# Pixie8888/R3DFSSeg

Hardware: AMD Instinct MI355X
Metric: episodes/sec S3DIS 2-way 5-shot 2048-pt (MPTI+attention, train step: forward+backward+grad all-reduce+Adam) (higher is better)
Workload: dtype f32 (index-free GEMMs -- self-attention, 1x1 convolutions, weight gradients, the EdgeConv backward's edge GEMMs -- as bf16x3 split products on the bf16 MFMA with fp32 accumulate; every index-deciding result: fp32)

## Files before the change

include/r3d.h:

```cpp
#ifndef R3D_H
#define R3D_H
#include <stdint.h>

#ifdef __cplusplus
extern "C" {
#endif

const char* r3d_last_error_string(void);
int r3d_abi_version(void);
int r3d_debug_poison_lds(unsigned pattern, unsigned* sink , void* stream);
int r3d_debug_set_cg_spmv_lds_min_blocks(int min_blocks);
int r3d_set_matrix_arith(int mode);
int r3d_get_matrix_arith(void);
int r3d_debug_set_gemm_bx3(int mask);

int r3d_cm_to_pm(const float* in , int B, int C, int N, float* out , long ld, void* stream);
int r3d_pm_to_cm(const float* in , long ld, int B, int C, int N, float* out , void* stream);
int r3d_pm_to_cm_pitched(const float* in, long ld, int B, int C, int N, float* out , long pitch, void* stream);
long r3d_cm_pitch(int N);
int r3d_copy_cols(const float* src, long ld_src, float* dst, long ld_dst, long M, int C, void* stream);

int r3d_sqnorm(const float* x, long ldx, long rows, int C, float* out, void* stream);
long r3d_knn_norm_ws_words(int B, int N);
int r3d_knn_topk(const float* x, long ldx, const float* x_cm, int B, int N, int C, int k, int mode,
                 const int32_t* n_valid_dev, float* norm_ws, float* cm_ws, int32_t* idx_out, float* score_out,
                 int32_t* status, void* stream);
long r3d_knn_ws_words(int B, int N, int C, int k, int flags);
int r3d_knn_topk_batched(const float* x, long ldx, const float* x_cm, int B, int N, int C, int k, int mode,
                         const int32_t* n_valid_dev, int n_valid_stride, float* ws, long ws_words, int32_t* idx_out,
                         float* score_out, int32_t* status, void* stream);
int r3d_debug_set_knn_bf16_threshold(int on);
int r3d_debug_set_knn_bf16_filter(int on);
int r3d_set_wpack_in_capture(int on);

int r3d_pointwise_conv(const float* X, long ldx, const float* W , long M, int K, int Co,
                       const float* scale, const float* shift, int act, float* Out, long ldo, void* stream);

int r3d_edgeconv_fwd(const float* PQ, const int32_t* idx, const float* W2, const float* s2, const float* t2,
                     float* out, long ldo, int B, int N, int K, int32_t* argmax_out, void* stream);

long r3d_attention_ws_words(int B, int N);
int r3d_attention_fwd(const float* qkv, long ld, int B, int N, float* out, long ldo, float* lse_out, float* ws,
                      void* stream);

int r3d_head_desc_words(void);
int r3d_head_max_k(void);
int r3d_fps_sample_count_table(int k, int n_max, int32_t* out, void* stream);
long r3d_head_proto_ws_words(int n_way, int k_shot, int N);
int r3d_head_proto_ws_offsets(int n_way, int k_shot, int N, long* out6 );
#define R3D_HEAD_FPS_ONE_LAUNCH 1
int r3d_head_prototypes(const int32_t* support_y , const int32_t* shot_keep ,
                        const float* feat , long ldf, const float* featT ,
                        const float* qfeat , long ldq, int n_way, int k_shot, int N, int D,
                        int n_query_pts, int k, float* nodes, long ldn, float* node_labels ,
                        int32_t* desc, int32_t* assign_out , int32_t* cluster_count ,
                        int32_t* ws, long ws_words, int flags, void* stream);

int r3d_head_prototypes_batched(int n_ep, int fps_group, const int32_t* support_y, long sy_stride, const int32_t* shot_keep,
                                long keep_stride, const float* feat, long ldf, long feat_ep_rows, const float* qfeat, long ldq,
                                long qfeat_ep_rows, int n_way, int k_shot, int N, int D, int n_query_pts, int k, float* nodes,
                                long ldn, long nodes_ep_rows, float* node_labels, int32_t* desc, long desc_stride,
                                int32_t* assign_out, long assign_stride, int32_t* cluster_count, long ccount_stride,
                                int32_t* ws, long ws_words, long ws_stride, int flags, void* stream);

long r3d_lp_ws_words(int n_cap, int kp1);
int r3d_lp_ws_offsets(int n_cap, int kp1, long* out6);
int r3d_label_propagate(const float* nodes, long ldn, int D, const int32_t* nbr, int kp1, const float* Y,
                        const int32_t* n_dev, const int32_t* n_proto_dev, int n_cap, float sigma, float alpha,
                        int max_iter, float tol, float* Z, int32_t* ws, long ws_words, int32_t* stats_out, void* stream);

int r3d_label_propagate_batched(int n_ep, const float* nodes, long ldn, int D, const int32_t* nbr, int kp1, const float* Y,
                                const int32_t* n_dev, const int32_t* n_proto_dev, long desc_stride, int n_cap, float sigma,
                                float alpha, int max_iter, float tol, float* Z, int32_t* ws, long ws_words, long ws_stride,
                                int32_t* stats_out, long stats_stride, void* stream);
long r3d_graph_weights_verify_words(int n_cap, int kp1);
int r3d_graph_weights_verify(int n_ep, const float* nodes, long ldn, int D, const int32_t* n_dev, long desc_stride, int n_cap,
                             int kp1, float sigma, int32_t* ws, long ws_words, long ws_stride, float* scratch,
                             int32_t* mismatch_out, void* stream);

int r3d_label_propagate_solve_batched(int n_ep, const float* Y, const int32_t* n_dev, long desc_stride, int n_cap, int kp1,
                                      float alpha, int max_iter, float tol, float* Z, int32_t* ws, long ws_words,
                                      long ws_stride, int32_t* stats_out, long stats_stride, void* stream);

int r3d_graph_set_lp_budget(void* graph, void* graph_exec, int budget, int* n_cg);

int r3d_query_logits_ce(const float* Z, const int32_t* n_proto_dev, int n_q, int N, int n_classes,
                        const int64_t* labels , float* logits ,
                        float* loss_out , int32_t* pred_out , void* stream);

int r3d_query_logits_ce_batched(int n_ep, const float* Z, long z_ep_rows, const int32_t* n_proto_dev, long desc_stride, int n_q,
                                int N, int n_classes, const int64_t* labels, float* logits, float* loss_out, int32_t* pred_out,
                                void* stream);

int r3d_pointwise_conv_acc(const float* X, long ldx, const float* W, long M, int K, int Co, const float* scale,
                           const float* shift, int act, float* Out, long ldo, void* stream);
long r3d_pointwise_conv_stats_ws_words(long M, int Co);
int r3d_pointwise_conv_stats(const float* X, long ldx, const float* W, long M, int K, int Co, float* Out, long ldo,
                             float* sums_out , float* ws, void* stream);
int r3d_pointwise_conv_stats2(const float* X, long ldx, const float* W, long M, int K, int Co, float* Out, long ldo,
                              long M_first, float* sums_a , float* sums_b , float* ws, void* stream);
int r3d_pointwise_conv_stats_seg(const float* X, long ldx, const float* W, long M, int K, int Co, float* Out, long ldo,
                                 long rows_a, long rows_b, float* sums_out, float* ws, void* stream);
int r3d_colreduce(const float* part , int chunks, int C, float* sums_out , void* stream);
int r3d_colreduce_seg(const float* part, int count_a, int count_b, int n_seg, int C, float* sums_out , void* stream);
long r3d_colstats_ws_words(long M, int C);
int r3d_colstats(const float* X, long ldx, const float* DY, long lddy, long M, int C, int mode, const float* scale,
                 const float* shift, const float* mean, const float* invstd, int act, float* sums_out ,
                 float* ws, void* stream);
int r3d_bn_fold(const float* sums, double count, int C, const float* gamma, const float* beta, float eps,
                float momentum, float* running_mean , float* running_var , float* mean, float* invstd,
                float* scale, float* shift, float* rec , const int32_t* rec_index_dev , long rec_stride,
                void* stream);
long r3d_colstats_seg_ws_words(long M, int C, long rows_a, long rows_b);
int r3d_colstats_seg(const float* X, long ldx, const float* DY, long lddy, long M, int C, long rows_a, long rows_b, int mode,
                     const float* scale, const float* shift, const float* mean, const float* invstd, long bn_stride, int act,
                     float* sums_out , float* ws, void* stream);
int r3d_bn_fold_seg(const float* sums , int n_seg, double count_a, double count_b, int C, const float* gamma,
                    const float* beta, float eps, float momentum, float* running_mean , float* running_var ,
                    float* mean, float* invstd, float* scale, float* shift, long bn_stride, float* rec ,
                    const int32_t* rec_index_dev , long rec_stride, void* stream);
int r3d_affine_act_seg(const float* Z, long ldz, long M, int C, long rows_a, long rows_b, const float* scale, const float* shift,
                       long bn_stride, int act, float* Y, long ldy, void* stream);
int r3d_bn_bwd_apply_seg(const float* Z, long ldz, const float* DY, long lddy, long M, int C, long rows_a, long rows_b,
                         const float* scale, const float* shift, const float* mean, const float* invstd, long bn_stride, int act,
                         const float* sums , double count_a, double count_b, float* DZ, long lddz, void* stream);
int r3d_bn_running_update(const float* rec, int n_records, long rec_stride, int C, float momentum,
                          const float* bias , float* running_mean,
                          float* running_var, void* stream);
int r3d_affine_act(const float* Z, long ldz, long M, int C, const float* scale, const float* shift, int act, float* Y,
                   long ldy, void* stream);
int r3d_bn_bwd_apply(const float* Z, long ldz, const float* DY, long lddy, long M, int C, const float* scale,
                     const float* shift, const float* mean, const float* invstd, int act, const float* sums,
                     double count, float* DZ, long lddz, void* stream);
long r3d_gemm_tn_ws_words(long M, int Ca, int Cb);
int r3d_gemm_tn(const float* A, long lda, const float* B, long ldb, long M, int Ca, int Cb, float alpha, float* out,
                int accumulate, float* ws, void* stream);
int r3d_add_cols(const float* src, long ld_src, float* dst, long ld_dst, long M, int C, void* stream);

long r3d_edgeconv_train_ws_words(int B, int N);
int r3d_edge_stats1(const float* PQ, const int32_t* idx, int B, int N, int K, int clouds_a, int clouds_b,
                    float* sums_out , float* esum , float* ws,
                    void* stream);
int r3d_edgeconv_train_fwd_minmax(const float* PQ, const int32_t* idx, const float* s1, const float* t1, long bn_stride,
                                  const float* W2, int B, int N, int K, int clouds_a, int clouds_b, float* zmax, float* zmin,
                                  int32_t* argmax, int32_t* argmin, float* sums_out , float* ws, void* stream);
int r3d_edge_select(float* zmax , const float* zmin, int32_t* argmax ,
                    const int32_t* argmin, const float* s2, const float* t2, long bn_stride, long M, long rows_a, long rows_b,
                    float* out, long ldo, void* stream);
long r3d_edge_reverse_ws_words(int B, int N, int K);
int r3d_edge_reverse(const int32_t* idx, int B, int N, int K, int32_t* rev_ws, long ws_words, void* stream);
int r3d_edgeconv_bwd(const float* PQ, const int32_t* idx, const float* s1, const float* t1, const float* mean1,
                     const float* invstd1, const float* W2, const float* s2, const float* t2, const float* mean2,
                     const float* invstd2, long bn_stride, const float* bn2_sums, const float* dout, long lddo,
                     const int32_t* argmax, const float* zwin , const float* esum , int B, int N, int K,
                     int clouds_a, int clouds_b, float* DY1 , float* BE ,
                     const int32_t* rev_ws , float* dW2, float* bn1_sums, float* dPQ,
                     float* ws, void* stream);

int r3d_attention_fwd_train(const float* qkv, long ld, int B, int N, float* out, long ldo, float* lse_out, float p_drop,
                            unsigned seed, const unsigned* seed_dev, float* ws , void* stream);
int r3d_attention_bwd(const float* qkv, long ld, int B, int N, const float* O, long ldo, const float* dO, long lddo,
                      const float* lse, float p_drop, unsigned seed, const unsigned* seed_dev, float q_scale, float* dqkv,
                      long ldd, float* ws , void* stream);
int r3d_attention_bwd_ws(const float* qkv, long ld, int B, int N, const float* O, long ldo, const float* dO, long lddo,
                         const float* lse, float p_drop, unsigned seed, const unsigned* seed_dev, float q_scale,
                         float* dqkv, long ldd, float* ws, int ws_holds_packed_qkv, void* stream);

long r3d_attention_ws_words_ep(int B, int N, int seed_group);
int r3d_attention_fwd_train_ep(const float* qkv, long ld, int B, int N, float* out, long ldo, float* lse_out, float p_drop,
                               unsigned seed, const unsigned* seed_dev, int seed_group, float* ws, void* stream);
int r3d_attention_bwd_ep(const float* qkv, long ld, int B, int N, const float* O, long ldo, const float* dO, long lddo,
                         const float* lse, float p_drop, unsigned seed, const unsigned* seed_dev, int seed_group, float q_scale,
                         float* dqkv, long ldd, float* ws, int ws_holds_packed_qkv, void* stream);

long r3d_attention_ws_words_ep_d(int B, int N, int seed_group, int D);
int r3d_attention_fwd_train_ep_d(const float* qkv, long ld, int B, int N, float* out, long ldo, float* lse_out, float p_drop,
                                 unsigned seed, const unsigned* seed_dev, int seed_group, int D, float* ws, void* stream);
int r3d_attention_bwd_ep_d(const float* qkv, long ld, int B, int N, const float* O, long ldo, const float* dO, long lddo,
                           const float* lse, float p_drop, unsigned seed, const unsigned* seed_dev, int seed_group, int D,
                           float q_scale, float* dqkv, long ldd, float* ws, int ws_holds_packed_qkv, void* stream);

int r3d_ce_grad(const float* Z, const int32_t* n_proto_dev, int n_cap, int n_query_pts, int n_classes,
                const int64_t* labels, const float* gscale_dev, float* G, void* stream);
int r3d_label_propagate_bwd(const float* nodes, long ldn, int D, int kp1, const float* Z, const float* G,
                            const int32_t* n_dev, int n_cap, float sigma, float alpha, int max_iter, float tol, float* lam,
                            float* dnodes, long ldd, int32_t* ws, long ws_words, int32_t* stats_out, void* stream);
int r3d_head_prototypes_bwd(const float* dnodes, long ldd, int n_way, int k_shot, int N, int D, int n_query_pts,
                            const int32_t* desc, const int32_t* assign, const int32_t* cluster_count, const int32_t* ws,
                            float* dsfeat, long lds_, float* dqfeat, long ldq, void* stream);

int r3d_ce_grad_batched(int n_ep, const float* Z, const int32_t* n_proto_dev, long desc_stride, int n_cap, int n_query_pts,
                        int n_classes, const int64_t* labels, const float* gscale_dev, float* G, void* stream);
int r3d_label_propagate_bwd_batched(int n_ep, const float* nodes, long ldn, int D, int kp1, const float* Z, const float* G,
                                    const int32_t* n_dev, long desc_stride, int n_cap, float sigma, float alpha, int max_iter,
                                    float tol, float* lam, float* dnodes, long ldd, int32_t* ws, long ws_words, long ws_stride,
                                    int32_t* stats_out, long stats_stride, void* stream);
int r3d_head_prototypes_bwd_batched(int n_ep, const float* dnodes, long ldd, long nodes_ep_rows, int n_way, int k_shot, int N,
                                    int D, int n_query_pts, const int32_t* desc, long desc_stride, const int32_t* assign,
                                    long assign_stride, const int32_t* cluster_count, long ccount_stride, const int32_t* ws,
                                    long ws_stride, float* dsfeat, long lds_, long dsfeat_ep_rows, float* dqfeat, long ldq,
                                    long dqfeat_ep_rows, void* stream);

long r3d_contrast_ws_words(int n_way, int k_shot, int N);
int r3d_contrast_fwd(const float* feat, long ldf, int D, const int32_t* support_y, const int32_t* support_flag, int n_way,
                     int k_shot, int N, const float* W, const float* bias, float temp, float* loss_out, float* ws,
                     long ws_words, void* stream);
int r3d_contrast_bwd(int D, int n_way, int k_shot, int N, const float* gscale_dev, float* dfeat, long ldd, float* dW,
                     float* db, float* ws, void* stream);
int r3d_contrast_fwd_batched(int n_ep, const float* feat, long ldf, long feat_ep_rows, int D, const int32_t* support_y,
                             const int32_t* support_flag, int n_way, int k_shot, int N, const float* W, const float* bias,
                             float temp, float* loss_out, float* ws, long ws_words, long ws_stride, void* stream);
int r3d_contrast_bwd_batched(int n_ep, int D, int n_way, int k_shot, int N, const float* gscale_dev, float* dfeat, long ldd,
                             long dfeat_ep_rows, float* dW, float* db, float* ws, long ws_stride, void* stream);
int r3d_train_metrics_batched(int n_ep, const int32_t* pred, const int64_t* query_y, const int64_t* gt_query_y, int n_query_pts,
                              const float* Z, long z_ep_rows, const int32_t* desc, long desc_stride, const int32_t* proto_ws,
                              long pws_stride, const int32_t* assign, long assign_stride, const int32_t* gt_support_y, int n_way,
                              int k_shot, int N, float* out4 , void* stream);
int r3d_train_metrics(const int32_t* pred, const int64_t* query_y, const int64_t* gt_query_y, int n_query_pts, const float* Z,
                      const int32_t* desc, const int32_t* proto_ws, const int32_t* assign, const int32_t* gt_support_y,
                      int n_way, int k_shot, int N, float* out4, void* stream);

long r3d_clean_ws_words(int n_way, int k_shot);
int r3d_clean_shot_detect(const float* feat , long ldf, int D, const float* support_x ,
                          int Cin, const int32_t* support_y, int n_way, int k_shot, int N, int32_t* shot_keep,
                          float* dbg_cos_sum , int32_t* ws, void* stream);

int r3d_clean_shot_detect_batched(int n_ep, const float* feat, long ldf, long feat_ep_rows, int D, const float* support_x,
                                  int Cin, const int32_t* support_y, int n_way, int k_shot, int N, int32_t* shot_keep,
                                  float* dbg_cos_sum, int32_t* ws, long ws_stride, void* stream);

int r3d_protonet_head(const float* sfeat, long ldf, const float* qfeat, long ldq, int D, const int32_t* support_y,
                      int n_way, int k_shot, int N, int n_query_pts, int method, float scaler, float* Z, float* ws,
                      void* stream);

long r3d_protonet_head_ws_words(int n_ep, int n_way, int k_shot);
int r3d_protonet_head_batched(int n_ep, const float* sfeat, long ldf, const float* qfeat, long ldq, long feat_ep_rows, int D,
                              const int32_t* support_y, int n_way, int k_shot, int N, int n_query_pts, int method,
                              float scaler, float* Z, float* ws, long ws_words, void* stream);
int r3d_count_correct_batched(int n_ep, const int32_t* pred, const int64_t* labels, long n_pts, int32_t* correct,
                              void* stream);

long r3d_protonet_head_train_ws_words(int n_ep, int n_way, int k_shot, int N, int n_query_pts, int D);
int r3d_protonet_head_train_fwd(int n_ep, const float* sfeat, long ldf, const float* qfeat, long ldq, long feat_ep_rows, int D,
                                const int32_t* support_y, int n_way, int k_shot, int N, int n_query_pts, int method,
                                float scaler, float* Z, float* ws, long ws_words, void* stream);
int r3d_protonet_head_bwd(int n_ep, const float* qfeat, long ldq, long feat_ep_rows, int D, const int32_t* support_y, int n_way,
                          int k_shot, int N, int n_query_pts, int method, float scaler, const float* dZ, float* dsfeat,
                          long ldds, float* dqfeat, long lddq, long dfeat_ep_rows, float* ws, long ws_words, void* stream);

int r3d_miou_accumulate(const int32_t* pred, const int64_t* gt, long n, const int32_t* lut, int n_lut, int n_classes,
                        uint64_t* hist, void* stream);

#ifdef __cplusplus
}
#endif
#endif
```

r3dfsseg_amd/_lib.py:

```python
import ctypes
import os
import re

_HERE = os.path.dirname(os.path.abspath(__file__))
LIB_PATH = os.environ.get("R3D_LIB") or os.path.join(_HERE, "libr3d_hip.so")
HEADER_PATH = os.path.join(os.path.dirname(_HERE), "include", "r3d.h")

c_f = ctypes.c_void_p
c_i = ctypes.c_int
c_l = ctypes.c_long
c_fl = ctypes.c_float
c_d = ctypes.c_double
c_u = ctypes.c_uint

_SIGS = {
    "r3d_last_error_string": (ctypes.c_char_p, []),
    "r3d_abi_version": (c_i, []),
    "r3d_cm_to_pm": (c_i, [c_f, c_i, c_i, c_i, c_f, c_l, c_f]),
    "r3d_pm_to_cm": (c_i, [c_f, c_l, c_i, c_i, c_i, c_f, c_f]),
    "r3d_pm_to_cm_pitched": (c_i, [c_f, c_l, c_i, c_i, c_i, c_f, c_l, c_f]),
    "r3d_cm_pitch": (c_l, [c_i]),
    "r3d_copy_cols": (c_i, [c_f, c_l, c_f, c_l, c_l, c_i, c_f]),
    "r3d_sqnorm": (c_i, [c_f, c_l, c_l, c_i, c_f, c_f]),
    "r3d_knn_topk": (c_i, [c_f, c_l, c_f, c_i, c_i, c_i, c_i, c_i, c_f, c_f, c_f, c_f, c_f, c_f, c_f]),
    "r3d_pointwise_conv": (c_i, [c_f, c_l, c_f, c_l, c_i, c_i, c_f, c_f, c_i, c_f, c_l, c_f]),
    "r3d_edgeconv_fwd": (c_i, [c_f, c_f, c_f, c_f, c_f, c_f, c_l, c_i, c_i, c_i, c_f, c_f]),
    "r3d_attention_ws_words": (c_l, [c_i, c_i]),
    "r3d_knn_norm_ws_words": (c_l, [c_i, c_i]),
    "r3d_attention_fwd": (c_i, [c_f, c_l, c_i, c_i, c_f, c_l, c_f, c_f, c_f]),
    "r3d_head_desc_words": (c_i, []),
    "r3d_debug_poison_lds": (c_i, [c_u, c_f, c_f]),
    "r3d_debug_set_cg_spmv_lds_min_blocks": (c_i, [c_i]),
    "r3d_debug_set_gemm_bx3": (c_i, [c_i]),
    "r3d_set_matrix_arith": (c_i, [c_i]),
    "r3d_get_matrix_arith": (c_i, []),
    "r3d_head_max_k": (c_i, []),
    "r3d_fps_sample_count_table": (c_i, [c_i, c_i, c_f, c_f]),
    "r3d_head_proto_ws_words": (c_l, [c_i, c_i, c_i]),
    "r3d_head_proto_ws_offsets": (c_i, [c_i, c_i, c_i, ctypes.POINTER(c_l)]),
    "r3d_head_prototypes": (c_i, [c_f, c_f, c_f, c_l, c_f, c_f, c_l, c_i, c_i, c_i, c_i, c_i, c_i, c_f, c_l,
                                  c_f, c_f, c_f, c_f, c_f, c_l, c_i, c_f]),
    "r3d_lp_ws_words": (c_l, [c_i, c_i]),
    "r3d_lp_ws_offsets": (c_i, [c_i, c_i, ctypes.POINTER(c_l)]),
    "r3d_label_propagate": (c_i, [c_f, c_l, c_i, c_f, c_i, c_f, c_f, c_f, c_i, c_fl, c_fl, c_i, c_fl, c_f, c_f,
                                  c_l, c_f, c_f]),
    "r3d_graph_set_lp_budget": (c_i, [c_f, c_f, c_i, ctypes.POINTER(c_i)]),
    "r3d_pointwise_conv_acc": (c_i, [c_f, c_l, c_f, c_l, c_i, c_i, c_f, c_f, c_i, c_f, c_l, c_f]),
    "r3d_edgeconv_train_fwd_minmax": (c_i, [c_f, c_f, c_f, c_f, c_l, c_f, c_i, c_i, c_i, c_i, c_i, c_f, c_f, c_f, c_f, c_f, c_f, c_f]),
    "r3d_edge_select": (c_i, [c_f, c_f, c_f, c_f, c_f, c_f, c_l, c_l, c_l, c_l, c_f, c_l, c_f]),
    "r3d_pointwise_conv_stats_ws_words": (c_l, [c_l, c_i]),
    "r3d_pointwise_conv_stats": (c_i, [c_f, c_l, c_f, c_l, c_i, c_i, c_f, c_l, c_f, c_f, c_f]),
    "r3d_pointwise_conv_stats2": (c_i, [c_f, c_l, c_f, c_l, c_i, c_i, c_f, c_l, c_l, c_f, c_f, c_f, c_f]),
    "r3d_colreduce": (c_i, [c_f, c_i, c_i, c_f, c_f]),
    "r3d_colstats_ws_words": (c_l, [c_l, c_i]),
    "r3d_colstats": (c_i, [c_f, c_l, c_f, c_l, c_l, c_i, c_i, c_f, c_f, c_f, c_f, c_i, c_f, c_f, c_f]),
    "r3d_bn_fold": (c_i, [c_f, c_d, c_i, c_f, c_f, c_fl, c_fl, c_f, c_f, c_f, c_f, c_f, c_f, c_f, c_f, c_l, c_f]),
    "r3d_bn_running_update": (c_i, [c_f, c_i, c_l, c_i, c_fl, c_f, c_f, c_f, c_f]),
    "r3d_affine_act": (c_i, [c_f, c_l, c_l, c_i, c_f, c_f, c_i, c_f, c_l, c_f]),
    "r3d_bn_bwd_apply": (c_i, [c_f, c_l, c_f, c_l, c_l, c_i, c_f, c_f, c_f, c_f, c_i, c_f, c_d, c_f, c_l, c_f]),
    "r3d_gemm_tn_ws_words": (c_l, [c_l, c_i, c_i]),
    "r3d_gemm_tn": (c_i, [c_f, c_l, c_f, c_l, c_l, c_i, c_i, c_fl, c_f, c_i, c_f, c_f]),
    "r3d_add_cols": (c_i, [c_f, c_l, c_f, c_l, c_l, c_i, c_f]),
    "r3d_edgeconv_train_ws_words": (c_l, [c_i, c_i]),
    "r3d_edge_stats1": (c_i, [c_f, c_f, c_i, c_i, c_i, c_i, c_i, c_f, c_f, c_f, c_f]),
    "r3d_edge_reverse_ws_words": (c_l, [c_i, c_i, c_i]),
    "r3d_edge_reverse": (c_i, [c_f, c_i, c_i, c_i, c_f, c_l, c_f]),
    "r3d_edgeconv_bwd": (c_i, [c_f] * 11 + [c_l, c_f, c_f, c_l, c_f, c_f, c_f, c_i, c_i, c_i, c_i, c_i, c_f, c_f, c_f, c_f, c_f, c_f, c_f, c_f]),
    "r3d_attention_fwd_train": (c_i, [c_f, c_l, c_i, c_i, c_f, c_l, c_f, c_fl, c_u, c_f, c_f, c_f]),
    "r3d_attention_bwd": (c_i, [c_f, c_l, c_i, c_i, c_f, c_l, c_f, c_l, c_f, c_fl, c_u, c_f, c_fl, c_f, c_l, c_f, c_f]),
    "r3d_attention_bwd_ws": (c_i, [c_f, c_l, c_i, c_i, c_f, c_l, c_f, c_l, c_f, c_fl, c_u, c_f, c_fl, c_f, c_l, c_f, c_i, c_f]),
    "r3d_ce_grad": (c_i, [c_f, c_f, c_i, c_i, c_i, c_f, c_f, c_f, c_f]),
    "r3d_label_propagate_bwd": (c_i, [c_f, c_l, c_i, c_i, c_f, c_f, c_f, c_i, c_fl, c_fl, c_i, c_fl, c_f, c_f, c_l, c_f, c_l, c_f, c_f]),
    "r3d_head_prototypes_bwd": (c_i, [c_f, c_l, c_i, c_i, c_i, c_i, c_i, c_f, c_f, c_f, c_f, c_f, c_l, c_f, c_l, c_f]),
    "r3d_contrast_ws_words": (c_l, [c_i, c_i, c_i]),
    "r3d_contrast_fwd": (c_i, [c_f, c_l, c_i, c_f, c_f, c_i, c_i, c_i, c_f, c_f, c_fl, c_f, c_f, c_l, c_f]),
    "r3d_contrast_bwd": (c_i, [c_i, c_i, c_i, c_i, c_f, c_f, c_l, c_f, c_f, c_f, c_f]),
    "r3d_train_metrics": (c_i, [c_f, c_f, c_f, c_i, c_f, c_f, c_f, c_f, c_f, c_i, c_i, c_i, c_f, c_f]),
    "r3d_clean_ws_words": (c_l, [c_i, c_i]),
    "r3d_clean_shot_detect": (c_i, [c_f, c_l, c_i, c_f, c_i, c_f, c_i, c_i, c_i, c_f, c_f, c_f, c_f]),
    "r3d_protonet_head": (c_i, [c_f, c_l, c_f, c_l, c_i, c_f, c_i, c_i, c_i, c_i, c_i, c_fl, c_f, c_f, c_f]),
    "r3d_protonet_head_ws_words": (c_l, [c_i, c_i, c_i]),
    "r3d_protonet_head_batched": (c_i, [c_i, c_f, c_l, c_f, c_l, c_l, c_i, c_f, c_i, c_i, c_i, c_i, c_i, c_fl, c_f, c_f, c_l, c_f]),
    "r3d_count_correct_batched": (c_i, [c_i, c_f, c_f, c_l, c_f, c_f]),
    "r3d_protonet_head_train_ws_words": (c_l, [c_i, c_i, c_i, c_i, c_i, c_i]),
    "r3d_protonet_head_train_fwd": (c_i, [c_i, c_f, c_l, c_f, c_l, c_l, c_i, c_f, c_i, c_i, c_i, c_i, c_i, c_fl, c_f, c_f, c_l, c_f]),
    "r3d_protonet_head_bwd": (c_i, [c_i, c_f, c_l, c_l, c_i, c_f, c_i, c_i, c_i, c_i, c_i, c_fl, c_f, c_f, c_l, c_f, c_l, c_l, c_f,
                                    c_l, c_f]),
    "r3d_miou_accumulate": (c_i, [c_f, c_f, c_l, c_f, c_i, c_i, c_f, c_f]),
    "r3d_query_logits_ce": (c_i, [c_f, c_f, c_i, c_i, c_i, c_f, c_f, c_f, c_f, c_f]),
    "r3d_knn_topk_batched": (c_i, [c_f, c_l, c_f, c_i, c_i, c_i, c_i, c_i, c_f, c_i, c_f, c_l, c_f, c_f, c_f, c_f]),
    "r3d_knn_ws_words": (c_l, [c_i, c_i, c_i, c_i, c_i]),
    "r3d_debug_set_knn_bf16_threshold": (c_i, [c_i]),
    "r3d_debug_set_knn_bf16_filter": (c_i, [c_i]),
    "r3d_set_wpack_in_capture": (c_i, [c_i]),
    "r3d_pointwise_conv_stats_seg": (c_i, [c_f, c_l, c_f, c_l, c_i, c_i, c_f, c_l, c_l, c_l, c_f, c_f, c_f]),
    "r3d_colreduce_seg": (c_i, [c_f, c_i, c_i, c_i, c_i, c_f, c_f]),
    "r3d_colstats_seg_ws_words": (c_l, [c_l, c_i, c_l, c_l]),
    "r3d_colstats_seg": (c_i, [c_f, c_l, c_f, c_l, c_l, c_i, c_l, c_l, c_i, c_f, c_f, c_f, c_f, c_l, c_i, c_f, c_f, c_f]),
    "r3d_bn_fold_seg": (c_i, [c_f, c_i, c_d, c_d, c_i, c_f, c_f, c_fl, c_fl, c_f, c_f, c_f, c_f, c_f, c_f, c_l, c_f, c_f, c_l, c_f]),
    "r3d_affine_act_seg": (c_i, [c_f, c_l, c_l, c_i, c_l, c_l, c_f, c_f, c_l, c_i, c_f, c_l, c_f]),
    "r3d_bn_bwd_apply_seg": (c_i, [c_f, c_l, c_f, c_l, c_l, c_i, c_l, c_l, c_f, c_f, c_f, c_f, c_l, c_i, c_f, c_d, c_d, c_f, c_l, c_f]),
    "r3d_attention_ws_words_ep": (c_l, [c_i, c_i, c_i]),
    "r3d_attention_fwd_train_ep": (c_i, [c_f, c_l, c_i, c_i, c_f, c_l, c_f, c_fl, c_u, c_f, c_i, c_f, c_f]),
    "r3d_attention_bwd_ep": (c_i, [c_f, c_l, c_i, c_i, c_f, c_l, c_f, c_l, c_f, c_fl, c_u, c_f, c_i, c_fl, c_f, c_l, c_f, c_i, c_f]),
    "r3d_attention_ws_words_ep_d": (c_l, [c_i, c_i, c_i, c_i]),
    "r3d_attention_fwd_train_ep_d": (c_i, [c_f, c_l, c_i, c_i, c_f, c_l, c_f, c_fl, c_u, c_f, c_i, c_i, c_f, c_f]),
    "r3d_attention_bwd_ep_d": (c_i, [c_f, c_l, c_i, c_i, c_f, c_l, c_f, c_l, c_f, c_fl, c_u, c_f, c_i, c_i, c_fl, c_f, c_l, c_f, c_i,
                                     c_f]),
    "r3d_head_prototypes_batched": (c_i, [c_i, c_i, c_f, c_l, c_f, c_l, c_f, c_l, c_l, c_f, c_l, c_l, c_i, c_i, c_i, c_i, c_i, c_i,
                                          c_f, c_l, c_l, c_f, c_f, c_l, c_f, c_l, c_f, c_l, c_f, c_l, c_l, c_i, c_f]),
    "r3d_head_prototypes_bwd_batched": (c_i, [c_i, c_f, c_l, c_l, c_i, c_i, c_i, c_i, c_i, c_f, c_l, c_f, c_l, c_f, c_l, c_f, c_l,
                                              c_f, c_l, c_l, c_f, c_l, c_l, c_f]),
    "r3d_graph_weights_verify_words": (c_l, [c_i, c_i]),
    "r3d_graph_weights_verify": (c_i, [c_i, c_f, c_l, c_i, c_f, c_l, c_i, c_i, c_fl, c_f, c_l, c_l, c_f, c_f, c_f]),
    "r3d_label_propagate_solve_batched": (c_i, [c_i, c_f, c_f, c_l, c_i, c_i, c_fl, c_i, c_fl, c_f, c_f, c_l, c_l, c_f, c_l, c_f]),
    "r3d_label_propagate_batched": (c_i, [c_i, c_f, c_l, c_i, c_f, c_i, c_f, c_f, c_f, c_l, c_i, c_fl, c_fl, c_i, c_fl, c_f, c_f,
                                          c_l, c_l, c_f, c_l, c_f]),
    "r3d_label_propagate_bwd_batched": (c_i, [c_i, c_f, c_l, c_i, c_i, c_f, c_f, c_f, c_l, c_i, c_fl, c_fl, c_i, c_fl, c_f, c_f,
                                              c_l, c_f, c_l, c_l, c_f, c_l, c_f]),
    "r3d_ce_grad_batched": (c_i, [c_i, c_f, c_f, c_l, c_i, c_i, c_i, c_f, c_f, c_f, c_f]),
    "r3d_query_logits_ce_batched": (c_i, [c_i, c_f, c_l, c_f, c_l, c_i, c_i, c_i, c_f, c_f, c_f, c_f, c_f]),
    "r3d_contrast_fwd_batched": (c_i, [c_i, c_f, c_l, c_l, c_i, c_f, c_f, c_i, c_i, c_i, c_f, c_f, c_fl, c_f, c_f, c_l, c_l, c_f]),
    "r3d_contrast_bwd_batched": (c_i, [c_i, c_i, c_i, c_i, c_i, c_f, c_f, c_l, c_l, c_f, c_f, c_f, c_l, c_f]),
    "r3d_train_metrics_batched": (c_i, [c_i, c_f, c_f, c_f, c_i, c_f, c_l, c_f, c_l, c_f, c_l, c_f, c_l, c_f, c_i, c_i, c_i, c_f, c_f]),
    "r3d_clean_shot_detect_batched": (c_i, [c_i, c_f, c_l, c_l, c_i, c_f, c_i, c_f, c_i, c_i, c_i, c_f, c_f, c_f, c_l, c_f]),
}

_lib = None


def header_symbols():
    txt = open(HEADER_PATH).read()
    txt = re.sub(r"/\*.*?\*/", "", txt, flags=re.S)
    return sorted(set(re.findall(r"\b(r3d_[a-z0-9_]+)\s*\(", txt)))


ABI_VERSION = 5


def load():
    global _lib
    if _lib is not None:
        return _lib
    import torch
    if not os.path.exists(LIB_PATH):
        raise RuntimeError(
            "r3dfsseg_amd: %s not found -- build it with `python -m r3dfsseg_amd.build` "
            "(hipcc, gfx950). There is no CPU fallback." % LIB_PATH)
    cdll = ctypes.CDLL(LIB_PATH)
    lib = _Bound()
    lib._cdll = cdll
    for name, (res, args) in _SIGS.items():
        try:
            fn = getattr(cdll, name)
        except AttributeError:
            raise RuntimeError("r3dfsseg_amd: symbol %s missing from %s" % (name, LIB_PATH))
        fn.restype = res
        fn.argtypes = args
        setattr(lib, name, fn)
    if lib.r3d_abi_version() != ABI_VERSION:
        raise RuntimeError("r3dfsseg_amd: %s has C ABI version %d, this package binds version %d -- rebuild it "
                           "(`python -m r3dfsseg_amd.build --force`)" % (LIB_PATH, lib.r3d_abi_version(), ABI_VERSION))
    _lib = lib
    mode = os.environ.get("R3D_MATRIX_ARITH")
    if mode is not None:
        if mode not in ("fp32", "bf16x3"):
            raise RuntimeError("R3D_MATRIX_ARITH=%r: expected fp32 or bf16x3" % mode)
        check(lib.r3d_set_matrix_arith(1 if mode == "bf16x3" else 0))
    mask = os.environ.get("R3D_GEMM_BX3")
    if mask is not None:
        check(lib.r3d_debug_set_gemm_bx3(int(mask)))
    return lib


class _Bound:
    """The bound entry points as plain attributes (one per symbol of include/r3d.h)."""


_call_log = None


def record_calls(on):
    lib = load()
    for name in _SIGS:
        raw = getattr(lib._cdll, name)
        if not on:
            setattr(lib, name, raw)
            continue

        def wrapper(*args, _raw=raw):
            rc = _raw(*args)
            if _call_log is not None:
                _call_log.append((_raw, args))
            return rc
        setattr(lib, name, wrapper)


def check(rc):
    if rc != 0:
        raise RuntimeError("r3d: " + load().r3d_last_error_string().decode())
```

r3dfsseg_amd/csrc/common.h:

```cpp
#pragma once
#include <hip/hip_runtime.h>
#include <stdint.h>
#include <stdio.h>

#define R3D_OK 0
#define R3D_ERR_ARG 1
#define R3D_ERR_LAUNCH 2
#define R3D_ERR_UNSUPPORTED 3

void r3d_set_error(const char* fmt, ...);

#define R3D_REQUIRE(cond, ...)          \
  do {                                  \
    if (!(cond)) {                      \
      r3d_set_error(__VA_ARGS__);       \
      return R3D_ERR_ARG;               \
    }                                   \
  } while (0)

#define R3D_LAUNCH_CHECK(name)                                              \
  do {                                                                      \
    hipError_t e_ = hipGetLastError();                                      \
    if (e_ != hipSuccess) {                                                 \
      r3d_set_error("%s: launch failed: %s", name, hipGetErrorString(e_));  \
      return R3D_ERR_LAUNCH;                                                \
    }                                                                       \
  } while (0)

typedef float f32x16 __attribute__((ext_vector_type(16)));
typedef float f32x4 __attribute__((ext_vector_type(4)));

#define R3D_WAVE 64

static __device__ __forceinline__ int r3d_lane() { return threadIdx.x & 63; }

static __device__ __forceinline__ int r3d_acc_row(int r, int lane) {
  return (r & 3) + 8 * (r >> 2) + 4 * (lane >> 5);
}

static __device__ __forceinline__ float r3d_readlane_f(float v, int src) {
  return __int_as_float(__builtin_amdgcn_readlane(__float_as_int(v), src));
}

static __device__ __forceinline__ float r3d_sum8_dpp(float v) {
  int x = __float_as_int(v);
  v += __int_as_float(__builtin_amdgcn_mov_dpp(x, 0xB1, 0xF, 0xF, true));
  x = __float_as_int(v);
  v += __int_as_float(__builtin_amdgcn_mov_dpp(x, 0x4E, 0xF, 0xF, true));
  x = __float_as_int(v);
  v += __int_as_float(__builtin_amdgcn_mov_dpp(x, 0x141, 0xF, 0xF, true));
  return v;
}

static __device__ __forceinline__ int r3d_wave_incl_scan(int v) {
  v += __builtin_amdgcn_update_dpp(0, v, 0x111, 0xF, 0xF, true);
  v += __builtin_amdgcn_update_dpp(0, v, 0x112, 0xF, 0xF, true);
  v += __builtin_amdgcn_update_dpp(0, v, 0x114, 0xF, 0xF, true);
  v += __builtin_amdgcn_update_dpp(0, v, 0x118, 0xF, 0xF, true);
  v += __builtin_amdgcn_update_dpp(0, v, 0x142, 0xA, 0xF, false);
  v += __builtin_amdgcn_update_dpp(0, v, 0x143, 0xC, 0xF, false);
  return v;
}

static __device__ __forceinline__ float r3d_wave_sum(float v) {
#pragma unroll
  for (int o = 32; o > 0; o >>= 1) v += __shfl_xor(v, o);
  return v;
}
static __device__ __forceinline__ float r3d_wave_max(float v) {
#pragma unroll
  for (int o = 32; o > 0; o >>= 1) v = fmaxf(v, __shfl_xor(v, o));
  return v;
}

static __device__ __forceinline__ float r3d_keep(float v, bool keep) {
  return __uint_as_float(__float_as_uint(v) & (keep ? 0xffffffffu : 0u));
}

typedef unsigned r3d_u32x4 __attribute__((ext_vector_type(4)));
typedef __bf16 r3d_bf16x8 __attribute__((ext_vector_type(8)));
extern int g_r3d_matrix_arith;

static __device__ __forceinline__ void r3d_bx3_split2(float x0, float x1, unsigned& h, unsigned& m, unsigned& l) {
  const unsigned u0 = __float_as_uint(x0), u1 = __float_as_uint(x1);
  const float r0 = x0 - __uint_as_float(u0 & 0xffff0000u), r1 = x1 - __uint_as_float(u1 & 0xffff0000u);
  const unsigned v0 = __float_as_uint(r0), v1 = __float_as_uint(r1);
  const float t0 = r0 - __uint_as_float(v0 & 0xffff0000u), t1 = r1 - __uint_as_float(v1 & 0xffff0000u);
  h = __builtin_amdgcn_perm(u1, u0, 0x07060302u);
  m = __builtin_amdgcn_perm(v1, v0, 0x07060302u);
  l = __builtin_amdgcn_perm(__float_as_uint(t1), __float_as_uint(t0), 0x07060302u);
}
struct r3d_bx3 {
  r3d_u32x4 h, m, l;
};
static __device__ __forceinline__ r3d_bx3 r3d_bx3_split8(const float* x) {
  r3d_bx3 f;
#pragma unroll
  for (int i = 0; i < 4; ++i) {
    unsigned h, m, l;
    r3d_bx3_split2(x[2 * i], x[2 * i + 1], h, m, l);
    f.h[i] = h; f.m[i] = m; f.l[i] = l;
  }
  return f;
}
static __device__ __forceinline__ f32x16 r3d_mfma_bf16(r3d_u32x4 a, r3d_u32x4 b, f32x16 c) {
#if defined(ATT_ABL) && (ATT_ABL & 4)
  c[0] += __uint_as_float(a[0] ^ b[1]);
  return c;
#endif
  return __builtin_amdgcn_mfma_f32_32x32x16_bf16(__builtin_bit_cast(r3d_bf16x8, a), __builtin_bit_cast(r3d_bf16x8, b), c, 0,
                                                 0, 0);
}
static __device__ __forceinline__ f32x16 r3d_bx3_mma(const r3d_bx3& a, const r3d_bx3& b, f32x16 c) {
  c = r3d_mfma_bf16(a.l, b.h, c);
  c = r3d_mfma_bf16(a.h, b.l, c);
  c = r3d_mfma_bf16(a.m, b.m, c);
  c = r3d_mfma_bf16(a.m, b.h, c);
  c = r3d_mfma_bf16(a.h, b.m, c);
  c = r3d_mfma_bf16(a.h, b.h, c);
  return c;
}

extern int g_r3d_gemm_bx3;

static inline int r3d_cdiv(long a, long b) { return (int)((a + b - 1) / b); }

static __device__ __forceinline__ int r3d_xcd_swizzle(int id, int n) {
  const int q = n >> 3, r = n & 7, x = id & 7;
  return (x < r ? x * (q + 1) : r * (q + 1) + (x - r) * q) + (id >> 3);
}

struct r3d_segmap {
  long a, b;
  __host__ __device__ bool odd(int seg) const { return b > 0 && (seg & 1); }
  __host__ __device__ long seg_rows(int seg) const { return odd(seg) ? b : a; }
  __host__ __device__ long seg_row0(int seg) const {
    return b > 0 ? (long)(seg >> 1) * (a + b) + (odd(seg) ? a : 0) : (long)seg * a;
  }
  __host__ __device__ int seg_of_row(long r) const {
    if (b == 0) return (int)(r / a);
    const long p = r / (a + b);
    return (int)(2 * p + ((r - p * (a + b)) >= a ? 1 : 0));
  }
  __device__ int seg_of_row32(int r) const {
    const int A = (int)a, B = (int)b;
    if (B == 0) return r / A;
    const int p = r / (A + B);
    return 2 * p + ((r - p * (A + B)) >= A ? 1 : 0);
  }
  __host__ __device__ int n_seg(long total) const { return (int)(b > 0 ? 2 * (total / (a + b)) : total / a); }
  __host__ __device__ bool covers(long total) const {
    return a > 0 && b >= 0 && total > 0 && total < 0x7fffffffL && total % (a + b) == 0;
  }
};

static __global__ void r3d_fill_words_kernel(unsigned* __restrict__ p, unsigned v, long n) {
  for (long i = (long)blockIdx.x * blockDim.x + threadIdx.x; i < n; i += (long)gridDim.x * blockDim.x) p[i] = v;
}
static __global__ void r3d_copy_words_kernel(unsigned* __restrict__ dst, const unsigned* __restrict__ src, long n) {
  for (long i = (long)blockIdx.x * blockDim.x + threadIdx.x; i < n; i += (long)gridDim.x * blockDim.x) dst[i] = src[i];
}
static __global__ void r3d_fill_words_ep_kernel(unsigned* __restrict__ p, unsigned v, long n, long stride_words) {
  p += (long)blockIdx.y * stride_words;
  for (long i = (long)blockIdx.x * blockDim.x + threadIdx.x; i < n; i += (long)gridDim.x * blockDim.x) p[i] = v;
}
static inline void r3d_fill_words_ep(void* p, unsigned v, long n_words, int n_ep, long stride_words, hipStream_t st) {
  const int g = (int)(n_words < 256L * 2048 ? (n_words + 255) / 256 : 2048);
  hipLaunchKernelGGL(r3d_fill_words_ep_kernel, dim3(g > 0 ? g : 1, n_ep), dim3(256), 0, st, (unsigned*)p, v, n_words, stride_words);
}
static inline void r3d_zero_words(void* p, long n_words, hipStream_t st) {
  const int g = (int)(n_words < 256L * 2048 ? (n_words + 255) / 256 : 2048);
  hipLaunchKernelGGL(r3d_fill_words_kernel, dim3(g > 0 ? g : 1), dim3(256), 0, st, (unsigned*)p, 0u, n_words);
}
static inline void r3d_copy_words(void* dst, const void* src, long n_words, hipStream_t st) {
  const int g = (int)(n_words < 256L * 2048 ? (n_words + 255) / 256 : 2048);
  hipLaunchKernelGGL(r3d_copy_words_kernel, dim3(g > 0 ? g : 1), dim3(256), 0, st, (unsigned*)dst, (const unsigned*)src,
                     n_words);
}
```

r3dfsseg_amd/csrc/edgeconv_train.hip:

```cpp
#include <stdlib.h>
#include "edge_tile.h"

#define ET_LD 65
#define ET_MAXBLK 1024
#define EC_CHUNK 32

static __device__ __forceinline__ float lrelu(float v) { return v > 0.f ? v : 0.2f * v; }

struct EcGeom {
  int N, cpc;
  __host__ __device__ static EcGeom make(int N) { return EcGeom{N, (N + EC_CHUNK - 1) / EC_CHUNK}; }
  __device__ void range(int chunk, int& cloud, int& p0, int& p1) const {
    cloud = __builtin_amdgcn_readfirstlane(chunk / cpc);
    p0 = __builtin_amdgcn_readfirstlane(cloud * N + (chunk - cloud * cpc) * EC_CHUNK);
    p1 = __builtin_amdgcn_readfirstlane(min(p0 + EC_CHUNK, (cloud + 1) * N));
  }
};
static __device__ __forceinline__ int ec_seg(const r3d_segmap& cs, int cloud) {
  return __builtin_amdgcn_readfirstlane(cs.seg_of_row32(cloud));
}

template <int RT>
__global__ __launch_bounds__(256) void r3d_edge_stats1_kernel(const float* __restrict__ PQ, const int* __restrict__ idx,
                                                              EcGeom gm, int n_chunks, float* __restrict__ part,
// ... 343 lines not shown
  for (int o = 32; o > 0; o >>= 1) my_below += __shfl_xor(my_below, o);
  if (lane == 0) atomicAdd(&below_s, my_below);
  __syncthreads();
  if (tid < RV_RANGE) {
    const int v = tid < nr ? cnt[tid] : 0;
    int x = v;
#pragma unroll
    for (int o = 1; o < 64; o <<= 1) {
      const int y = __shfl_up(x, o);
      if (lane >= o) x += y;
    }
    if (lane == 63) wsum[w] = x;
    cur[tid] = x - v;
  }
  __syncthreads();
  if (tid < RV_RANGE) {
    int wb = 0;
    for (int q = 0; q < w; ++q) wb += wsum[q];
    off[tid] = cur[tid] + wb;
  }
  if (tid == 0) {
    int t = 0;
    for (int q = 0; q < RV_RANGE / 64; ++q) t += wsum[q];
    off[RV_RANGE] = t;
  }
  __syncthreads();
  const long seg0 = gbase + below_s;
  if (tid < nr) rev_ptr[(long)cloud * N + r0 + tid] = (int)(seg0 + off[tid]);
  if (cloud == n_clouds - 1 && r0 + nr == N && tid == 0) rev_ptr[(long)n_clouds * N] = (int)((long)n_clouds * E);
  int a = 0;
  while (a < nr) {
    if (tid == 0) {
      int b = nr;
      if (off[nr] - off[a] > RV_CAP) {
        int lo = a, hi = nr;
        while (lo < hi) {
          const int mid = (lo + hi + 1) >> 1;
          if (off[mid] - off[a] <= RV_CAP) lo = mid; else hi = mid - 1;
        }
        b = lo;
      }
      b_s = b;
    }
    __syncthreads();
    const int b = b_s;
    if (b == a) {
      long outp = seg0 + off[a];
      for (long e0 = 0; e0 < E; e0 += 1024) {
        const long e = e0 + tid;
        const bool hit = e < E && min(max(lst[min(e, E - 1)], 0), N - 1) - r0 == a;
        const unsigned long long m = __ballot(hit);
        if (lane == 0) wsum[w] = __popcll(m);
        __syncthreads();
        int before = 0, total = 0;
        for (int q = 0; q < 16; ++q) { before += q < w ? wsum[q] : 0; total += wsum[q]; }
        if (hit) rev[outp + before + __popcll(m & ((1ull << lane) - 1ull))] = (int)(gbase + e);
        outp += total;
        __syncthreads();
      }
      a += 1;
      continue;
    }
    if (tid < RV_RANGE) cur[tid] = (tid >= a && tid < b) ? off[tid] - off[a] : 0;
    __syncthreads();
    for (long e0 = tid; e0 < E; e0 += 8 * 1024) {
      int jv[8];
#pragma unroll
      for (int u = 0; u < 8; ++u) jv[u] = lst[min(e0 + 1024 * u, E - 1)];
#pragma unroll
      for (int u = 0; u < 8; ++u) {
        const int j = min(max(jv[u], 0), N - 1) - r0;
        if (e0 + 1024 * u < E && j >= a && j < b)
          buf[atomicAdd(&cur[j], 1)] = (int)(e0 + 1024 * u);
      }
    }
    __syncthreads();
    for (int j = a + w; j < b; j += 16) {
      const int s0 = off[j] - off[a], c = cnt[j];
      const long out0 = seg0 + off[j];
      for (int m0 = 0; m0 < c; m0 += 64) {
        const int mine = m0 + lane < c ? buf[s0 + m0 + lane] : 0x7fffffff;
        int rank = 0;
        for (int t0 = 0; t0 < c; t0 += 16) {
          int ov[16];
#pragma unroll
          for (int t = 0; t < 16; ++t) ov[t] = buf[s0 + min(t0 + t, c - 1)];
#pragma unroll
          for (int t = 0; t < 16; ++t) rank += (t0 + t < c && ov[t] < mine) ? 1 : 0;
        }
        if (m0 + lane < c) rev[out0 + rank] = (int)(gbase + mine);
      }
    }
    __syncthreads();
    a = b;
  }
}

#define RO_WAVES 8
__global__ __launch_bounds__(64 * RO_WAVES) void r3d_edge_reverse_ordered_kernel(const int* __restrict__ idx, int N, int K,
                                                                                 int n_clouds, int* __restrict__ rev_ptr,
                                                                                 int* __restrict__ rev) {
  extern __shared__ int ro_hist[];
  __shared__ int ro_wsum[RO_WAVES];
  const int tid = threadIdx.x, lane = tid & 63, w = __builtin_amdgcn_readfirstlane(tid >> 6);
  const int cloud = blockIdx.x;
  const int E = N * K;
  const long gbase = (long)cloud * E;
  const int* lst = idx + gbase;
  const int per = ((E + RO_WAVES - 1) / RO_WAVES + 63) & ~63;
  const int e_beg = min(w * per, E), e_end = min(e_beg + per, E);
  int* mine = ro_hist + w * N;
  for (int i = tid; i < RO_WAVES * N; i += 64 * RO_WAVES) ro_hist[i] = 0;
  __syncthreads();
  for (int e0 = e_beg + lane; e0 < e_end; e0 += 8 * 64) {
    int jv[8];
#pragma unroll
    for (int u = 0; u < 8; ++u) jv[u] = lst[min(e0 + 64 * u, E - 1)];
#pragma unroll
    for (int u = 0; u < 8; ++u)
      if (e0 + 64 * u < e_end) atomicAdd(&mine[min(max(jv[u], 0), N - 1)], 1);
  }
  __syncthreads();
  const int TPT = (N + 64 * RO_WAVES - 1) / (64 * RO_WAVES);
  const int j0 = tid * TPT;
  int tot = 0;
  for (int j = j0; j < min(j0 + TPT, N); ++j)
#pragma unroll
    for (int q = 0; q < RO_WAVES; ++q) tot += ro_hist[q * N + j];
  int incl = tot;
#pragma unroll
  for (int o = 1; o < 64; o <<= 1) {
    const int y = __shfl_up(incl, o);
    if (lane >= o) incl += y;
  }
  if (lane == 63) ro_wsum[w] = incl;
  __syncthreads();
  int run = incl - tot;
  for (int q = 0; q < w; ++q) run += ro_wsum[q];
  for (int j = j0; j < min(j0 + TPT, N); ++j) {
    rev_ptr[(long)cloud * N + j] = (int)(gbase + run);
#pragma unroll
    for (int q = 0; q < RO_WAVES; ++q) {
      const int c = ro_hist[q * N + j];
      ro_hist[q * N + j] = run;
      run += c;
    }
  }
  if (cloud == n_clouds - 1 && tid == 0) rev_ptr[(long)n_clouds * N] = (int)((long)n_clouds * E);
  __syncthreads();
  for (int e0 = e_beg; e0 < e_end; e0 += 64) {
    const int e = e0 + lane;
    const bool ok = e < e_end;
    const int j = min(max(lst[min(e, E - 1)], 0), N - 1);
    const int src = e / K;
    const int src0 = __builtin_amdgcn_readfirstlane(e0 / K);
    const int src1 = __builtin_amdgcn_readfirstlane(min(e0 + 63, e_end - 1) / K);
    int pos = 0;
    for (int g = src0; g <= src1; ++g)
      if (ok && src == g) pos = atomicAdd(&mine[j], 1);
    if (ok) rev[gbase + pos] = (int)(gbase + e);
  }
}

template <int RT>
__global__ __launch_bounds__(256) void r3d_edgeconv_bwd2_kernel(
    const float* __restrict__ PQ, const float* __restrict__ s1, const float* __restrict__ mean1,
    const float* __restrict__ invstd1, long bn_stride, const float* __restrict__ bn1_sums ,
    const float* __restrict__ DY1, const float* __restrict__ BE, const float* __restrict__ esum ,
    const int* __restrict__ rev_ptr, const int* __restrict__ rev,
    int e_off, EcGeom gm, r3d_segmap cs , int n_chunks, float* __restrict__ dPQ ) {
  constexpr int K = 4 * RT;
  const int lane = threadIdx.x & 63, w = threadIdx.x >> 6;
  for (int item = blockIdx.x; item < n_chunks; item += gridDim.x) {
    const int chunk = r3d_xcd_swizzle(item, n_chunks);
    int cloud, p0, p1;
    gm.range(chunk, cloud, p0, p1);
    const int seg = ec_seg(cs, cloud);
    const long bo = (long)seg * bn_stride;
    const double E = (double)cs.seg_rows(seg) * gm.N * K;
    const float sc1 = s1[bo + lane], mu1 = mean1[bo + lane], is1 = invstd1[bo + lane];
    const float n1 = (float)((double)bn1_sums[(long)seg * 128 + lane] / E), n2 = (float)((double)bn1_sums[(long)seg * 128 + 64 + lane] / E);
    for (int pt_ = p0 + w; pt_ < p1; pt_ += 4) {
      const long pt = pt_;
      const int rb = rev_ptr[pt], re = rev_ptr[pt + 1];
      const float pj = PQ[pt * 128 + lane];
      const float bs = BE[pt * 128 + lane];
      const float es = esum ? (esum[pt * 64 + lane] - (float)K * mu1) * is1 : BE[pt * 128 + 64 + lane];
      float asum = 0.f, gsum = 0.f;
      for (int e0 = rb; e0 < re; e0 += 16) {
        const int my_e = rev[min(e0 + min(lane, 15), re - 1)];
        float dv[16], qv[16];
#pragma unroll
        for (int t = 0; t < 16; ++t) {
          const int e = __builtin_amdgcn_readlane(my_e, t) - e_off;
          dv[t] = DY1[(long)e * 64 + lane];
          qv[t] = PQ[(long)(e / K) * 128 + 64 + lane];
        }
#pragma unroll
        for (int t = 0; t < 16; ++t) {
          const bool ok = e0 + t < re;
          asum += r3d_keep(dv[t], ok);
          gsum += r3d_keep(qv[t], ok);
        }
      }
      const float cj = (float)(re - rb);
      dPQ[pt * 128 + lane] = sc1 * (asum - cj * n1 - n2 * (is1 * (cj * (pj - mu1) + gsum)));
      dPQ[pt * 128 + 64 + lane] = sc1 * (bs - (float)K * n1 - n2 * es);
    }
  }
}

static int et_check(const char* fn, int B, int N, int K, int clouds_a, int clouds_b) {
  if (B <= 0 || N <= 0 || N % E2_PTS != 0 || K < 4 || K > 32 || K % 4 != 0) {
    r3d_set_error("%s: unsupported shape B=%d N=%d K=%d (N %% 4 == 0, K %% 4 == 0, 4..32)", fn, B, N, K);
    return R3D_ERR_ARG;
  }
  const r3d_segmap cs{clouds_a, clouds_b};
  if (!cs.covers(B)) {
    r3d_set_error("%s: %d clouds are not whole segments of %d + %d clouds", fn, B, clouds_a, clouds_b);
    return R3D_ERR_ARG;
  }
  if ((long)B * N * K >= 0x7fffffffL) {
    r3d_set_error("%s: B*N*K = %ld edges exceed the 31-bit edge ids", fn, (long)B * N * K);
    return R3D_ERR_ARG;
  }
  return 0;
}
static int et_chunks(int B, int N) { return B * EcGeom::make(N).cpc; }
static int et_grid8(int n_chunks, int cap) { return n_chunks <= cap ? n_chunks : (cap >= 8 ? cap & ~7 : cap); }

extern "C" long r3d_edgeconv_train_ws_words(int B, int N) { return (long)ET_MAXBLK * 4096 + (long)et_chunks(B, N) * 128 + 64; }

static void et_reduce_chunks(const float* part, int N, int clouds_a, int clouds_b, int n_seg, float* out, hipStream_t st) {
  const int cpc = EcGeom::make(N).cpc;
  hipLaunchKernelGGL(r3d_part_reduce_kernel, dim3(128 / 64, n_seg), dim3(1024), 0, st, part, clouds_a * cpc, clouds_b * cpc, 128,
                     out, 128L, 128, (float*)nullptr, 0L);
}

extern "C" int r3d_edge_stats1(const float* PQ, const int32_t* idx, int B, int N, int K, int clouds_a, int clouds_b,
                               float* sums_out, float* esum, float* ws, void* stream) {
  R3D_REQUIRE(PQ && idx && sums_out && ws, "r3d_edge_stats1: null pointer");
  int rc = et_check("r3d_edge_stats1", B, N, K, clouds_a, clouds_b);
  if (rc) return rc;
  hipStream_t st = (hipStream_t)stream;
  const EcGeom gm = EcGeom::make(N);
  const int n_chunks = et_chunks(B, N);
  const int grid = et_grid8(n_chunks, 2048);
#define E2_CASE(RT) \
  case RT: hipLaunchKernelGGL(r3d_edge_stats1_kernel<RT>, dim3(grid), dim3(256), 0, st, PQ, idx, gm, n_chunks, ws, esum); break
  switch (K / 4) {
    E2_CASE(1); E2_CASE(2); E2_CASE(3); E2_CASE(4); E2_CASE(5); E2_CASE(6); E2_CASE(7); E2_CASE(8);
  }
#undef E2_CASE
  et_reduce_chunks(ws, N, clouds_a, clouds_b, r3d_segmap{clouds_a, clouds_b}.n_seg(B), sums_out, st);
  R3D_LAUNCH_CHECK("r3d_edge_stats1");
  return R3D_OK;
}

template <int RT>
static int fwd2_launch_rt(int n_chunks, hipStream_t st, const float* PQ, const int32_t* idx, const float* s1, const float* t1,
                          long bn_stride, const float* W2, EcGeom gm, r3d_segmap cs, int32_t* argmax, float* zmax, float* zmin,
                          int32_t* argmin, float* ws) {
  const size_t lds = sizeof(float) * ((size_t)2 * 16 * RT * E2_LD);
  static int resident = 0;
  if (!resident) {
    resident = e2_resident_blocks(r3d_edgeconv_train_fwd2_kernel<RT>, lds, ET_MAXBLK);
    R3D_REQUIRE(resident > 0, "r3d_edgeconv_train_fwd_minmax: cannot reserve %zu B of LDS", lds);
  }
  const int grid = et_grid8(n_chunks, resident);
  hipLaunchKernelGGL(r3d_edgeconv_train_fwd2_kernel<RT>, dim3(grid), dim3(256), lds, st, PQ, idx, s1, t1, bn_stride, W2, gm, cs,
                     n_chunks, argmax, zmax, zmin, argmin, ws);
  return R3D_OK;
}

extern "C" int r3d_edgeconv_train_fwd_minmax(const float* PQ, const int32_t* idx, const float* s1, const float* t1,
                                             long bn_stride, const float* W2, int B, int N, int K, int clouds_a, int clouds_b,
                                             float* zmax, float* zmin, int32_t* argmax, int32_t* argmin, float* sums_out,
                                             float* ws, void* stream) {
  R3D_REQUIRE(PQ && idx && s1 && t1 && W2 && zmax && zmin && argmax && argmin && sums_out && ws,
              "r3d_edgeconv_train_fwd_minmax: null pointer");
  int rc = et_check("r3d_edgeconv_train_fwd_minmax", B, N, K, clouds_a, clouds_b);
  if (rc) return rc;
  hipStream_t st = (hipStream_t)stream;
  const EcGeom gm = EcGeom::make(N);
  const r3d_segmap cs{clouds_a, clouds_b};
  const int n_chunks = et_chunks(B, N);
#define E2_CASE(RT)                                                                                                    \
  case RT:                                                                                                             \
    rc = fwd2_launch_rt<RT>(n_chunks, st, PQ, idx, s1, t1, bn_stride, W2, gm, cs, argmax, zmax, zmin, argmin, ws);      \
    break
  switch (K / 4) {
    E2_CASE(1); E2_CASE(2); E2_CASE(3); E2_CASE(4); E2_CASE(5); E2_CASE(6); E2_CASE(7); E2_CASE(8);
  }
#undef E2_CASE
  if (rc) return rc;
  et_reduce_chunks(ws, N, clouds_a, clouds_b, cs.n_seg(B), sums_out, st);
  R3D_LAUNCH_CHECK("r3d_edgeconv_train_fwd_minmax");
  return R3D_OK;
}

__global__ void r3d_edge_select_kernel(float* __restrict__ zmax, const float* __restrict__ zmin, int* __restrict__ argmax,
                                       const int* __restrict__ argmin, const float* __restrict__ s2,
                                       const float* __restrict__ t2, long bn_stride, r3d_segmap sm , long M,
                                       float* __restrict__ out, long ldo) {
  const long i = (long)blockIdx.x * blockDim.x + threadIdx.x;
  if (i >= M * 64) return;
  const int c = (int)(i & 63);
  const long m = (long)__builtin_amdgcn_readfirstlane((int)(i >> 6));
  const long bo = (long)__builtin_amdgcn_readfirstlane(sm.seg_of_row32((int)m)) * bn_stride + c;
  const float sc = s2[bo];
  const bool up = sc >= 0.f;
  const float z = up ? zmax[i] : zmin[i];
  if (!up) { zmax[i] = z; argmax[i] = argmin[i]; }
  out[m * ldo + c] = lrelu(sc * z + t2[bo]);
}
extern "C" int r3d_edge_select(float* zmax, const float* zmin, int32_t* argmax, const int32_t* argmin, const float* s2,
                               const float* t2, long bn_stride, long M, long rows_a, long rows_b, float* out, long ldo,
                               void* stream) {
  R3D_REQUIRE(zmax && zmin && argmax && argmin && s2 && t2 && out && M > 0 && ldo >= 64, "r3d_edge_select: bad arguments");
  const r3d_segmap sm{rows_a, rows_b};
  R3D_REQUIRE(sm.covers(M), "r3d_edge_select: %ld rows are not whole segments of %ld + %ld rows", M, rows_a, rows_b);
  hipLaunchKernelGGL(r3d_edge_select_kernel, dim3(r3d_cdiv(M * 64, 256)), dim3(256), 0, (hipStream_t)stream, zmax, zmin,
                     argmax, argmin, s2, t2, bn_stride, sm, M, out, ldo);
  R3D_LAUNCH_CHECK("r3d_edge_select");
  return R3D_OK;
}

template <int RT>
static int bwd1_launch_rt(int n_chunks, hipStream_t st, const float* PQ, const int32_t* idx, EcBn bn, const float* W2,
                          const float* bn2_sums, const float* dout, long lddo, const int32_t* argmax, EcGeom gm, r3d_segmap cs,
                          float* DY1, float* BE, float* part_dw, float* part_bn, int* grid_out) {
  const size_t lds = sizeof(float) * ((size_t)2 * 16 * RT * E2_LD + 2 * E2_PTS * 64 + 6 * 64);
  static int resident = 0;
  if (!resident) {
    resident = e2_resident_blocks(r3d_edgeconv_bwd1_kernel<RT>, lds, ET_MAXBLK);
    R3D_REQUIRE(resident > 0, "r3d_edgeconv_bwd: cannot reserve %zu B of LDS", lds);
  }
  const int grid = et_grid8(n_chunks, resident);
  hipLaunchKernelGGL(r3d_edgeconv_bwd1_kernel<RT>, dim3(grid), dim3(256), lds, st, PQ, idx, bn, W2, bn2_sums, dout, lddo, argmax,
                     gm, cs, n_chunks, DY1, BE, part_dw, part_bn);
  *grid_out = grid;
  return R3D_OK;
}

template <int RT>
static int bwd1_bx3_launch_rt(int n_chunks, hipStream_t st, const float* PQ, const int32_t* idx, EcBn bn, const float* W2,
                              const float* bn2_sums, const float* dout, long lddo, const int32_t* argmax, const float* zwin,
                              EcGeom gm, r3d_segmap cs, float* DY1, float* BE, float* part_dw, float* part_bn, int* grid_out) {
  static int resident = 0;
  if (!resident) {
    resident = e2_resident_blocks(r3d_edgeconv_bwd1_bx3_kernel<RT>, EB_LDS_BYTES, ET_MAXBLK / 2);
    R3D_REQUIRE(resident > 0, "r3d_edgeconv_bwd: cannot reserve %d B of LDS", (int)EB_LDS_BYTES);
  }
  const int grid = et_grid8(n_chunks, resident);
  hipLaunchKernelGGL(r3d_edgeconv_bwd1_bx3_kernel<RT>, dim3(grid), dim3(256), EB_LDS_BYTES, st, PQ, idx, bn, W2, bn2_sums, dout,
                     lddo, argmax, zwin, gm, cs, n_chunks, DY1, BE, part_dw, part_bn);
  *grid_out = grid;
  return R3D_OK;
}

extern "C" long r3d_edge_reverse_ws_words(int B, int N, int K) { return (long)B * N + 1 + (long)B * N * K + 16; }
extern "C" int r3d_edge_reverse(const int32_t* idx, int B, int N, int K, int32_t* rev_ws, long ws_words, void* stream) {
  R3D_REQUIRE(idx && rev_ws, "r3d_edge_reverse: null pointer");
  R3D_REQUIRE(B > 0 && B <= 65535 && N > 0 && K > 0 && (long)B * N * K < 0x7fffffffL, "r3d_edge_reverse: bad shape B=%d N=%d K=%d",
              B, N, K);
  R3D_REQUIRE(ws_words >= r3d_edge_reverse_ws_words(B, N, K), "r3d_edge_reverse: workspace of %ld words is shorter than "
              "r3d_edge_reverse_ws_words(%d, %d, %d)", ws_words, B, N, K);
  const size_t ro_lds = sizeof(int) * (size_t)RO_WAVES * N;
  static const bool ro_off = getenv("R3D_EDGE_REVERSE_SORT") != nullptr;
  if (!ro_off && ro_lds <= 144 * 1024 && (long)N * K >= 64 * RO_WAVES) {
    static size_t attr = 0;
    if (ro_lds > attr) {
      R3D_REQUIRE(hipFuncSetAttribute((const void*)r3d_edge_reverse_ordered_kernel, hipFuncAttributeMaxDynamicSharedMemorySize,
                                      (int)ro_lds) == hipSuccess, "r3d_edge_reverse: cannot reserve %zu B of LDS", ro_lds);
      attr = ro_lds;
    }
    hipLaunchKernelGGL(r3d_edge_reverse_ordered_kernel, dim3(B), dim3(64 * RO_WAVES), ro_lds, (hipStream_t)stream, idx, N, K, B,
                       rev_ws, rev_ws + (long)B * N + 1);
  } else {
    hipLaunchKernelGGL(r3d_edge_reverse_kernel, dim3(r3d_cdiv(N, RV_RANGE), B), dim3(1024), 0, (hipStream_t)stream, idx, N, K, B,
                       rev_ws, rev_ws + (long)B * N + 1);
  }
  R3D_LAUNCH_CHECK("r3d_edge_reverse");
  return R3D_OK;
}

extern "C" int r3d_edgeconv_bwd(const float* PQ, const int32_t* idx, const float* s1, const float* t1, const float* mean1,
                                const float* invstd1, const float* W2, const float* s2, const float* t2, const float* mean2,
                                const float* invstd2, long bn_stride, const float* bn2_sums, const float* dout, long lddo,
                                const int32_t* argmax, const float* zwin, const float* esum, int B, int N, int K, int clouds_a,
                                int clouds_b, float* DY1, float* BE, const int32_t* rev_ws, float* dW2, float* bn1_sums,
                                float* dPQ, float* ws, void* stream) {
  R3D_REQUIRE(PQ && idx && s1 && t1 && mean1 && invstd1 && W2 && s2 && t2 && mean2 && invstd2 && bn2_sums && dout &&
                  argmax && DY1 && BE && rev_ws && dW2 && bn1_sums && dPQ && ws,
              "r3d_edgeconv_bwd: null pointer");
  int rc = et_check("r3d_edgeconv_bwd", B, N, K, clouds_a, clouds_b);
  if (rc) return rc;
  const EcGeom gm = EcGeom::make(N);
  const r3d_segmap cs{clouds_a, clouds_b};
  const int n_chunks = et_chunks(B, N);
  const int n_seg = cs.n_seg(B);
  hipStream_t st = (hipStream_t)stream;
  float* part_dw = ws;
  float* part_bn = ws + (long)ET_MAXBLK * 4096;
  const EcBn bn{s1, t1, mean1, invstd1, s2, t2, mean2, invstd2, bn_stride};
  int grid = 0;
  const bool bx3 = g_r3d_matrix_arith == 1 && zwin && esum && N % EB_PTS == 0 && (lddo & 3) == 0 && ((uintptr_t)dout & 15) == 0;
#define E2_CASE(RT)                                                                                                        \
  case RT:                                                                                                                 \
    rc = bx3 ? bwd1_bx3_launch_rt<RT>(n_chunks, st, PQ, idx, bn, W2, bn2_sums, dout, lddo, argmax, zwin, gm, cs, DY1, BE,  \
                                      part_dw, part_bn, &grid)                                                             \
             : bwd1_launch_rt<RT>(n_chunks, st, PQ, idx, bn, W2, bn2_sums, dout, lddo, argmax, gm, cs, DY1, BE, part_dw,   \
                                  part_bn, &grid);                                                                         \
    break
  switch (K / 4) {
    E2_CASE(1); E2_CASE(2); E2_CASE(3); E2_CASE(4); E2_CASE(5); E2_CASE(6); E2_CASE(7); E2_CASE(8);
  }
#undef E2_CASE
  if (rc) return rc;
  hipLaunchKernelGGL(r3d_part_reduce_kernel, dim3(4096 / 64, 1), dim3(1024), 0, st, part_dw, bx3 ? 2 * grid : grid, 0, 4096, dW2,
                     0L, 4096, (float*)nullptr, 0L);
  et_reduce_chunks(part_bn, N, clouds_a, clouds_b, n_seg, bn1_sums, st);
  const int32_t* rev_ptr = rev_ws;
  const int32_t* rev = rev_ws + (long)B * N + 1;
  const int grid2 = et_grid8(n_chunks, 4096);
#define E2_CASE(RT)                                                                                                       \
  case RT:                                                                                                                \
    hipLaunchKernelGGL(r3d_edgeconv_bwd2_kernel<RT>, dim3(grid2), dim3(256), 0, st, PQ, s1, mean1, invstd1, bn_stride, bn1_sums, \
                       DY1, BE, bx3 ? esum : (const float*)nullptr, rev_ptr, rev, 0, gm, cs, n_chunks, dPQ);              \
    break
  switch (K / 4) {
    E2_CASE(1); E2_CASE(2); E2_CASE(3); E2_CASE(4); E2_CASE(5); E2_CASE(6); E2_CASE(7); E2_CASE(8);
  }
#undef E2_CASE
  R3D_LAUNCH_CHECK("r3d_edgeconv_bwd");
  return R3D_OK;
}
```

r3dfsseg_amd/csrc/head_graph.hip:

```cpp
#include "common.h"

#define HG_NC 4
typedef unsigned short hg_col_t;
#define HG_ROWS_PER_BLOCK_MIN 4
#define HG_MAX_PART 2048

struct HgEp {
  long nodes, nbr, y, z, g, lam, dn;
  long desc;
  long ws;
  long stats;
  long labels, logits, loss, pred;
};
#define HG_WS(p) p = (decltype(p))((const char*)(p) + (long)ep * st.ws * 4)
#define HG_AT(p, stride) p += (long)ep * (stride)

__global__ __launch_bounds__(256) void r3d_graph_bits_kernel(const int* __restrict__ nbr, int kp1, const int* __restrict__ n_dev,
                                                             int n_cap, int words, unsigned* __restrict__ outb, HgEp st) {
  __shared__ unsigned bm[4][1024];
  const int ep = blockIdx.y;
  nbr += (long)ep * st.nbr * kp1; HG_AT(n_dev, st.desc); HG_WS(outb);
  const int n = min(*n_dev, n_cap);
  const int w = threadIdx.x >> 6, lane = threadIdx.x & 63;
  const int i = blockIdx.x * 4 + w;
  unsigned* b = bm[w];
  for (int wd = lane; wd < words; wd += 64) b[wd] = 0u;
  __syncthreads();
  if (i < n) {
    const int k = kp1 - 1;
    for (int t = lane; t < k; t += 64) {
      const int j = nbr[(long)i * kp1 + 1 + t];
      if (j < 0 || j >= n || j == i) continue;
      atomicOr(&b[j >> 5], 1u << (j & 31));
    }
  }
  __syncthreads();
  if (i < n_cap)
    for (int wd = lane; wd < words; wd += 64) outb[(long)i * words + wd] = b[wd];
}

#define BT_ROWS 1024
#define BT_CW 8
__global__ __launch_bounds__(256) void r3d_graph_transpose_kernel(const unsigned* __restrict__ outb, int words, int n_cap,
                                                                  unsigned* __restrict__ inb ,
                                                                  HgEp st) {
  __shared__ unsigned tile[BT_CW * 32][BT_ROWS / 32 + 1];
  const int ep = blockIdx.z;
  HG_WS(outb); HG_WS(inb);
  const int c0w = blockIdx.x * BT_CW, r0 = blockIdx.y * BT_ROWS;
  const int w = threadIdx.x >> 6, lane = threadIdx.x & 63;
  for (int sb = w; sb < BT_ROWS / 64; sb += 4) {
    const int r = r0 + sb * 64 + lane;
    unsigned v[BT_CW];
#pragma unroll
    for (int cw = 0; cw < BT_CW; ++cw) v[cw] = (r < n_cap && c0w + cw < words) ? outb[(long)r * words + c0w + cw] : 0u;
#pragma unroll
    for (int cw = 0; cw < BT_CW; ++cw) {
#pragma unroll
      for (int b = 0; b < 32; ++b) {
        const unsigned long long m = __ballot((v[cw] >> b) & 1u);
        if (lane == b) {
          tile[cw * 32 + b][2 * sb] = (unsigned)m;
          tile[cw * 32 + b][2 * sb + 1] = (unsigned)(m >> 32);
        }
      }
    }
  }
  __syncthreads();
  for (int e = threadIdx.x; e < BT_CW * 32 * (BT_ROWS / 32); e += 256) {
    const int c = e >> 5, wd = e & 31;
    const int col = c0w * 32 + c, ow = r0 / 32 + wd;
    if (col < n_cap && ow < words) inb[(long)col * words + ow] = tile[c][wd];
  }
}

__global__ void r3d_graph_rowlen_kernel(unsigned* __restrict__ sym ,
                                        const unsigned* __restrict__ outb, int words,
                                        const int* __restrict__ n_dev, int n_cap, int* __restrict__ row_len, HgEp st) {
  const int ep = blockIdx.y;
  HG_WS(sym); HG_WS(outb); HG_AT(n_dev, st.desc); HG_WS(row_len);
  const int n = min(*n_dev, n_cap);
  const int row = blockIdx.x * (blockDim.x >> 6) + (threadIdx.x >> 6);
  const int lane = threadIdx.x & 63;
  if (row >= n_cap) return;
  int c = 0;
  if (row < n)
    for (int wd = lane; wd < words; wd += 64) {
      const unsigned v = sym[(long)row * words + wd] | outb[(long)row * words + wd];
      sym[(long)row * words + wd] = v;
      c += __popc(v);
    }
#pragma unroll
  for (int o = 32; o > 0; o >>= 1) c += __shfl_xor(c, o);
  if (lane == 0) row_len[row] = c;
}

__global__ __launch_bounds__(1024) void r3d_scan_kernel(const int* __restrict__ in, int n, int* __restrict__ out, HgEp st) {
  const int ep = blockIdx.x;
  HG_WS(in); HG_WS(out);
  __shared__ int wave_tot[16];
  __shared__ int carry_s;
  const int tid = threadIdx.x, lane = tid & 63, w = tid >> 6;
  if (tid == 0) carry_s = 0;
  __syncthreads();
  for (int t0 = 0; t0 < n; t0 += 1024) {
    const int i = t0 + tid;
    const int v = i < n ? in[i] : 0;
    int x = v;
#pragma unroll
    for (int o = 1; o < 64; o <<= 1) {
      const int y = __shfl_up(x, o);
      if (lane >= o) x += y;
    }
    if (lane == 63) wave_tot[w] = x;
    __syncthreads();
    int wbase = 0, tot = 0;
    for (int q = 0; q < 16; ++q) {
      const int tv = wave_tot[q];
      if (q < w) wbase += tv;
      tot += tv;
    }
    const int carry = carry_s;
    if (i < n) out[i] = carry + wbase + x - v;
    __syncthreads();
    if (tid == 0) carry_s = carry + tot;
    __syncthreads();
  }
  if (tid == 0) out[n] = carry_s;
}

__global__ __launch_bounds__(256) void r3d_graph_cols_kernel(const unsigned* __restrict__ sym, int words,
                                                             const int* __restrict__ n_dev, int n_cap,
                                                             const int* __restrict__ row_ptr, hg_col_t* __restrict__ col,
                                                             HgEp st) {
  const int ep = blockIdx.y;
  HG_WS(sym); HG_AT(n_dev, st.desc); HG_WS(row_ptr); HG_WS(col);
  const int n = min(*n_dev, n_cap);
  const int i = blockIdx.x * 4 + (threadIdx.x >> 6);
  const int lane = threadIdx.x & 63;
  if (i >= n) return;
  const int wpl = (words + 63) / 64;
  const int w0 = lane * wpl;
  int mycount = 0;
  for (int t = 0; t < wpl; ++t) {
    const int wd = w0 + t;
    if (wd < words) mycount += __popc(sym[(long)i * words + wd]);
  }
  int incl = mycount;
#pragma unroll
  for (int o = 1; o < 64; o <<= 1) {
    const int y = __shfl_up(incl, o);
    if (lane >= o) incl += y;
  }
  int wpos = row_ptr[i] + incl - mycount;
  for (int t = 0; t < wpl; ++t) {
    const int wd = w0 + t;
    if (wd >= words) break;
    unsigned bits = sym[(long)i * words + wd];
    while (bits) {
      const int b = __ffs((int)bits) - 1;
      bits &= bits - 1;
      col[wpos++] = (hg_col_t)(wd * 32 + b);
    }
  }
}

__global__ __launch_bounds__(256) void r3d_graph_weights_kernel(
    const float* __restrict__ nodes, long ldn, int D, const unsigned* __restrict__ outb, int words,
    const int* __restrict__ n_dev, int n_cap, const int* __restrict__ row_ptr, const hg_col_t* __restrict__ col,
    float sigma, float* __restrict__ val, float* __restrict__ dinv, float* __restrict__ wdir , HgEp st) {
  __shared__ __attribute__((aligned(16))) float xs[256];
  __shared__ float wsum[4];
  const int ep = blockIdx.y;
  nodes += (long)ep * st.nodes * ldn; HG_WS(outb); HG_AT(n_dev, st.desc); HG_WS(row_ptr); HG_WS(col); HG_WS(val); HG_WS(dinv);
  HG_WS(wdir);
  const int n = min(*n_dev, n_cap);
  const int w = threadIdx.x >> 6;
  const int i = blockIdx.x;
  const int lane = threadIdx.x & 63;
  if (i >= n) return;
  const float* xi = nodes + (long)i * ldn;
  xs[threadIdx.x] = (int)threadIdx.x < D ? xi[threadIdx.x] : 0.f;
  __syncthreads();
  const int beg = row_ptr[i], end = row_ptr[i + 1];
  const int D4 = D >> 2;
  const int part = lane & 7, slot = lane >> 3;
  float dsum = 0.f;
  for (int e0 = beg + 8 * w; e0 < end; e0 += 32) {
    const int e = e0 + slot;
    const bool ok = e < end;
    const int j = col[min(e, end - 1)];
    const float* xj = nodes + (long)j * ldn;
    float a = 0.f, b = 0.f;
    auto step = [&](const float4 y, int c4) {
      const float4 x = *reinterpret_cast<const float4*>(&xs[4 * c4]);
      float d1, d2;
      d1 = (x.x - y.x) + 1e-6f; d2 = (y.x - x.x) + 1e-6f; a = __builtin_fmaf(d1, d1, a); b = __builtin_fmaf(d2, d2, b);
      d1 = (x.y - y.y) + 1e-6f; d2 = (y.y - x.y) + 1e-6f; a = __builtin_fmaf(d1, d1, a); b = __builtin_fmaf(d2, d2, b);
      d1 = (x.z - y.z) + 1e-6f; d2 = (y.z - x.z) + 1e-6f; a = __builtin_fmaf(d1, d1, a); b = __builtin_fmaf(d2, d2, b);
      d1 = (x.w - y.w) + 1e-6f; d2 = (y.w - x.w) + 1e-6f; a = __builtin_fmaf(d1, d1, a); b = __builtin_fmaf(d2, d2, b);
    };
    int c4 = part;
    for (; c4 + 40 < D4; c4 += 48) {
      float4 y[6];
#pragma unroll
      for (int u = 0; u < 6; ++u) y[u] = *reinterpret_cast<const float4*>(xj + 4 * (c4 + 8 * u));
#pragma unroll
      for (int u = 0; u < 6; ++u) step(y[u], c4 + 8 * u);
    }
    for (; c4 < D4; c4 += 8) step(*reinterpret_cast<const float4*>(xj + 4 * c4), c4);
    if (part == 0) {
      for (int c = 4 * D4; c < D; ++c) {
        const float y = xj[c], x = xs[c];
        const float d1 = (x - y) + 1e-6f, d2 = (y - x) + 1e-6f;
        a = __builtin_fmaf(d1, d1, a);
        b = __builtin_fmaf(d2, d2, b);
      }
    }
    a = r3d_sum8_dpp(a);
    b = r3d_sum8_dpp(b);
    const bool out_ij = (outb[(long)i * words + (j >> 5)] >> (j & 31)) & 1u;
    const bool out_ji = (outb[(long)j * words + (i >> 5)] >> (i & 31)) & 1u;
    float wij = 0.f, wji = 0.f;
    if (out_ij) { const float d = sqrtf(a) / sigma; wij = expf(-0.5f * (d * d)); }
    if (out_ji) { const float d = sqrtf(b) / sigma; wji = expf(-0.5f * (d * d)); }
    const float wgt = wij + wji;
    if (ok && part == 0) {
      val[e] = wgt;
      *reinterpret_cast<float2*>(wdir + 2L * e) = make_float2(wij, wji);
      dsum += wgt;
    }
  }
  dsum = r3d_wave_sum(dsum);
  if (lane == 0) wsum[w] = dsum;
  __syncthreads();
  if (threadIdx.x == 0)
    dinv[i] = sqrtf(1.0f / ((((wsum[0] + wsum[1]) + wsum[2]) + wsum[3]) + 2.220446049250313e-16f));
}

__global__ void r3d_graph_normalize_kernel(const int* __restrict__ row_ptr, const hg_col_t* __restrict__ col,
                                           const float* __restrict__ dinv, const int* __restrict__ n_dev,
                                           int n_cap, float* __restrict__ val, HgEp st) {
  const int ep = blockIdx.y;
  HG_WS(row_ptr); HG_WS(col); HG_WS(dinv); HG_AT(n_dev, st.desc); HG_WS(val);
  const int n = min(*n_dev, n_cap);
  const int i = blockIdx.x * 4 + (threadIdx.x >> 6);
  const int lane = threadIdx.x & 63;
  if (i >= n) return;
  const float di = dinv[i];
  for (int e = row_ptr[i] + lane; e < row_ptr[i + 1]; e += 64) val[e] = (di * val[e]) * dinv[col[e]];
}

#define HG_MAX_ITER 1022
#define HG_M 64
#define HG_UROWS 256
#define HG_EBLOCKS 16
#define HG_PART (4 + 2 * HG_M * HG_NC)
static_assert(HG_M == 64 && HG_M * HG_NC == 256, "the CG kernels map (aggregate, column) onto 256 threads, aggregate = lane");
struct CgState {
  int done;
  int iters;
  unsigned ticket;
  int pad_;
  float bb[HG_NC];
  float rz[HG_NC];
  float beta[HG_NC];
  float mu[HG_M * HG_NC];
};

static __device__ __forceinline__ float4 f4_zero() { return make_float4(0.f, 0.f, 0.f, 0.f); }

static __device__ __forceinline__ float4 block_sum4(float4 v, float4* sm ) {
  const int lane = threadIdx.x & 63, w = threadIdx.x >> 6;
#pragma unroll
  for (int o = 32; o > 0; o >>= 1) {
    v.x += __shfl_xor(v.x, o); v.y += __shfl_xor(v.y, o);
    v.z += __shfl_xor(v.z, o); v.w += __shfl_xor(v.w, o);
  }
  __syncthreads();
  if (lane == 0) sm[w] = v;
  __syncthreads();
  float4 r = sm[0];
  for (int q = 1; q < 4; ++q) { r.x += sm[q].x; r.y += sm[q].y; r.z += sm[q].z; r.w += sm[q].w; }
  return r;
}

static __device__ __forceinline__ float4 reduce_partials(const float4* part, int nblk, float4* sm) {
  float4 a = f4_zero();
  for (int q0 = threadIdx.x; q0 < nblk; q0 += 8 * 256) {
    float4 p[8];
#pragma unroll
    for (int u = 0; u < 8; ++u) {
      const int q = q0 + 256 * u;
      const bool ok = q < nblk;
      p[u] = part[min(q, nblk - 1)];
      p[u].x = r3d_keep(p[u].x, ok); p[u].y = r3d_keep(p[u].y, ok); p[u].z = r3d_keep(p[u].z, ok); p[u].w = r3d_keep(p[u].w, ok);
    }
#pragma unroll
    for (int u = 0; u < 8; ++u) { a.x += p[u].x; a.y += p[u].y; a.z += p[u].z; a.w += p[u].w; }
  }
  return block_sum4(a, sm);
}

static __device__ __forceinline__ float f4_get(const float4& v, int c) { return c == 0 ? v.x : c == 1 ? v.y : c == 2 ? v.z : v.w; }

#define HG_SEED_PITCH 257
__global__ __launch_bounds__(256) void r3d_cg_aggregate_kernel(const float* __restrict__ nodes, long ldn, int D,
                                                               const int* __restrict__ n_dev, const int* __restrict__ n_proto_dev,
                                                               int n_cap, int rows_per_wave, int* __restrict__ agg, HgEp st) {
  extern __shared__ float smem[];
  {
    const int ep = blockIdx.y;
    nodes += (long)ep * st.nodes * ldn; HG_AT(n_dev, st.desc); HG_AT(n_proto_dev, st.desc); HG_WS(agg);
  }
  const int pitch = D | 1;
  float* seeds = smem;
  float* xrow = smem + HG_M * pitch + (threadIdx.x >> 6) * D;
  const int n = min(*n_dev, n_cap);
  const int n_proto = max(1, min(*n_proto_dev, n));
  const int lane = threadIdx.x & 63, w = threadIdx.x >> 6;
  {
    const int D4 = D >> 2;
    for (int s0 = 0; s0 < HG_M; s0 += 16) {
      const int sd = s0 + (threadIdx.x >> 4), l16 = threadIdx.x & 15;
      const int src = (int)(((long)sd * (n_proto - 1)) / (HG_M - 1));
      const float4* row = reinterpret_cast<const float4*>(nodes + (long)src * ldn);
      float4 v[4];
#pragma unroll
      for (int u = 0; u < 4; ++u) v[u] = row[min(l16 + 16 * u, D4 - 1)];
#pragma unroll
      for (int u = 0; u < 4; ++u) {
        const int c4 = l16 + 16 * u;
        if (c4 < D4) {
          float* dst = seeds + sd * pitch + 4 * c4;
          dst[0] = v[u].x; dst[1] = v[u].y; dst[2] = v[u].z; dst[3] = v[u].w;
        }
      }
    }
  }
  const int row0 = (blockIdx.x * 4 + w) * rows_per_wave;
  float xr[4][4];
#pragma unroll
  for (int k = 0; k < 4; ++k)
#pragma unroll
    for (int u = 0; u < 4; ++u)
      xr[k][u] = nodes[(long)min(row0 + min(k, rows_per_wave - 1), n - 1) * ldn + min(lane + 64 * u, D - 1)];
  __syncthreads();
  for (int k = 0; k < rows_per_wave; ++k) {
    const int i = row0 + k;
    if (i >= n) break;
#pragma unroll
    for (int u = 0; u < 4; ++u)
      if (lane + 64 * u < D) xrow[lane + 64 * u] = k == 0 ? xr[0][u] : k == 1 ? xr[1][u] : k == 2 ? xr[2][u] : xr[3][u];
    float d2 = 0.f;
    const float* sp = seeds + lane * pitch;
    for (int c0 = 0; c0 < D; c0 += 16) {
      float xs_[16], ss_[16];
#pragma unroll
      for (int c = 0; c < 16; ++c) { xs_[c] = xrow[min(c0 + c, D - 1)]; ss_[c] = sp[min(c0 + c, D - 1)]; }
#pragma unroll
      for (int c = 0; c < 16; ++c) {
        const float df = c0 + c < D ? xs_[c] - ss_[c] : 0.f;
        d2 = __builtin_fmaf(df, df, d2);
      }
    }
    unsigned long long key = ((unsigned long long)__float_as_uint(d2) << 32) | (unsigned)lane;
#pragma unroll
    for (int o = 32; o > 0; o >>= 1) {
      const unsigned long long other = __shfl_xor(key, o);
      key = other < key ? other : key;
    }
    if (lane == 0) agg[i] = (int)(key & 63u);
    __builtin_amdgcn_wave_barrier();
  }
}

__global__ __launch_bounds__(256) void r3d_cg_mw_kernel(const int* __restrict__ row_ptr, const hg_col_t* __restrict__ col,
                                                        const float* __restrict__ val, const float* __restrict__ dinv,
                                                        const int* __restrict__ agg, const int* __restrict__ n_dev, int n_cap,
                                                        float alpha_lp, int rows_per_wave, float* __restrict__ MW, HgEp st) {
  __shared__ float2 pairs[4][256];
  {
    const int ep = blockIdx.y;
    HG_WS(row_ptr); HG_WS(col); HG_WS(val); HG_WS(dinv); HG_WS(agg); HG_AT(n_dev, st.desc); HG_WS(MW);
  }
  const int n = min(*n_dev, n_cap);
  const int lane = threadIdx.x & 63, w = threadIdx.x >> 6;
  const int row0 = (blockIdx.x * 4 + w) * rows_per_wave;
  for (int k = 0; k < rows_per_wave; ++k) {
    const int i = row0 + k;
    if (i >= n_cap) break;
    float acc = 0.f;
    if (i < n) {
      const int rb = row_ptr[i], re = row_ptr[i + 1];
      for (int e0 = rb; e0 < re; e0 += 256) {
        const int cnt = min(256, re - e0);
#pragma unroll
        for (int u = 0; u < 4; ++u) {
          const int t = lane + 64 * u;
          if (t < cnt) {
            const int j = col[e0 + t];
            pairs[w][t] = make_float2(__int_as_float(agg[j]), val[e0 + t] / dinv[j]);
          }
        }
        __builtin_amdgcn_wave_barrier();
        for (int t0 = 0; t0 < cnt; t0 += 16) {
          float2 pr[16];
#pragma unroll
          for (int t = 0; t < 16; ++t) pr[t] = pairs[w][t0 + t];
#pragma unroll
          for (int t = 0; t < 16; ++t) acc += (__float_as_int(pr[t].x) == lane && t0 + t < cnt) ? pr[t].y : 0.f;
        }
        __builtin_amdgcn_wave_barrier();
      }
      acc = (agg[i] == lane ? 1.f / dinv[i] : 0.f) - alpha_lp * acc;
    }
    MW[(long)i * HG_M + lane] = acc;
  }
}

__global__ __launch_bounds__(128) void r3d_cg_epart_kernel(const float* __restrict__ MW, const float* __restrict__ dinv,
                                                           const int* __restrict__ agg, const int* __restrict__ n_dev, int n_cap,
                                                           float* __restrict__ Epart , HgEp st) {
  __shared__ float Ew[2][HG_M][HG_M];
  {
    const int ep = blockIdx.y;
    HG_WS(MW); HG_WS(dinv); HG_WS(agg); HG_AT(n_dev, st.desc); HG_WS(Epart);
  }
  const int n = min(*n_dev, n_cap);
  const int lane = threadIdx.x & 63, w = threadIdx.x >> 6;
  for (int a = 0; a < HG_M; ++a) Ew[w][a][lane] = 0.f;
  const int stride = 2 * HG_EBLOCKS;
  for (int i0 = blockIdx.x * 2 + w; i0 < n; i0 += 8 * stride) {
    float m[8], u[8];
    int a[8];
#pragma unroll
    for (int t = 0; t < 8; ++t) {
      const int i = min(i0 + t * stride, n - 1);
      m[t] = MW[(long)i * HG_M + lane]; u[t] = 1.f / dinv[i]; a[t] = agg[i];
    }
#pragma unroll
    for (int t = 0; t < 8; ++t)
      if (i0 + t * stride < n) Ew[w][a[t]][lane] += m[t] * u[t];
  }
  __syncthreads();
  float* out = Epart + (long)blockIdx.x * HG_M * HG_M;
  for (int e = threadIdx.x; e < HG_M * HG_M; e += 128) {
    const int a = e >> 6, b = e & 63;
    out[e] = Ew[0][a][b] + Ew[1][a][b];
  }
}

__global__ __launch_bounds__(1024) void r3d_cg_einv_kernel(const float* __restrict__ Epart, float* __restrict__ Einv, HgEp st) {
  __shared__ double S0[HG_M][HG_M + 1];
  {
    const int ep = blockIdx.x;
    HG_WS(Epart); HG_WS(Einv);
  }
  __shared__ double prow[2][2 * HG_M];
  __shared__ double pcol[2][HG_M];
  const int tid = threadIdx.x;
  const int row = tid >> 4, cg = (tid & 15) * 4;
  double a[4], b[4];
  {
    float v[HG_EBLOCKS][4];
#pragma unroll
    for (int q = 0; q < HG_EBLOCKS; ++q) {
      const float4 t = *reinterpret_cast<const float4*>(Epart + (long)q * HG_M * HG_M + row * HG_M + cg);
      v[q][0] = t.x; v[q][1] = t.y; v[q][2] = t.z; v[q][3] = t.w;
    }
#pragma unroll
    for (int c = 0; c < 4; ++c) {
      double s = 0.0;
#pragma unroll
      for (int q = 0; q < HG_EBLOCKS; ++q) s += (double)v[q][c];
      S0[row][cg + c] = s;
    }
  }
  __syncthreads();
#pragma unroll
  for (int c = 0; c < 4; ++c) {
    double v = 0.5 * (S0[row][cg + c] + S0[cg + c][row]);
    if (row == cg + c && !(v > 0.0)) v = 1.0;
    a[c] = v;
    b[c] = row == cg + c ? 1.0 : 0.0;
  }
  auto publish = [&](int k, int buf) {
    const int kc = k & 3;
    const double sel = kc == 0 ? a[0] : kc == 1 ? a[1] : kc == 2 ? a[2] : a[3];
    if (row == k) {
      const double piv = 1.0 / __shfl(sel, (k * 16 + (k >> 2)) & 63, 64);
#pragma unroll
      for (int c = 0; c < 4; ++c) { prow[buf][cg + c] = a[c] * piv; prow[buf][HG_M + cg + c] = b[c] * piv; }
    }
    if (cg == (k & ~3)) pcol[buf][row] = sel;
  };
  publish(0, 0);
  __syncthreads();
  for (int k = 0; k < HG_M; ++k) {
    const int buf = k & 1;
    double pa[4], pb[4];
#pragma unroll
    for (int c = 0; c < 4; ++c) { pa[c] = prow[buf][cg + c]; pb[c] = prow[buf][HG_M + cg + c]; }
    if (row == k) {
#pragma unroll
      for (int c = 0; c < 4; ++c) { a[c] = pa[c]; b[c] = pb[c]; }
    } else {
      const double f = pcol[buf][row];
#pragma unroll
      for (int c = 0; c < 4; ++c) { a[c] -= f * pa[c]; b[c] -= f * pb[c]; }
    }
    if (k + 1 < HG_M) publish(k + 1, buf ^ 1);
    __syncthreads();
  }
  __syncthreads();
#pragma unroll
  for (int c = 0; c < 4; ++c) S0[row][cg + c] = b[c];
  __syncthreads();
#pragma unroll
  for (int c = 0; c < 4; ++c) Einv[row * HG_M + cg + c] = (float)(0.5 * (S0[row][cg + c] + S0[cg + c][row]));
}

static __device__ __forceinline__ void cg_store_sc1(float* p, float v) {
  __hip_atomic_store(reinterpret_cast<unsigned*>(p), __float_as_uint(v), __ATOMIC_RELAXED, __HIP_MEMORY_SCOPE_AGENT);
}

static __device__ __forceinline__ float cg_load_sc1(const float* p) {
  return __uint_as_float(__hip_atomic_load(reinterpret_cast<const unsigned*>(p), __ATOMIC_RELAXED, __HIP_MEMORY_SCOPE_AGENT));
}

static __device__ __forceinline__ void cg_load_mw_column(const float* __restrict__ MW, int row0, int n_cap, float (&m)[64]) {
  const int a = threadIdx.x & 63, w = threadIdx.x >> 6;
#pragma unroll
  for (int k = 0; k < 64; ++k) m[k] = MW[(long)min(row0 + 64 * w + k, n_cap - 1) * HG_M + a];
}

static __device__ __forceinline__ void cg_block_partials(const float4* rs, const float* us, const int* ag, int row0, int n,
                                                         const float (&m)[64], bool with_t2, float* __restrict__ part,
                                                         float4* sm, float4* wpart ) {
  const int a = threadIdx.x & 63, w = threadIdx.x >> 6;
  float4 t = f4_zero(), t2 = f4_zero();
#pragma unroll 16
  for (int k = 0; k < 64; ++k) {
    const float4 rv = rs[64 * w + k];
    const float uw = ag[64 * w + k] == a ? us[64 * w + k] : 0.f;
    t.x = __builtin_fmaf(uw, rv.x, t.x); t.y = __builtin_fmaf(uw, rv.y, t.y);
    t.z = __builtin_fmaf(uw, rv.z, t.z); t.w = __builtin_fmaf(uw, rv.w, t.w);
    if (with_t2) {
      t2.x = __builtin_fmaf(m[k], rv.x, t2.x); t2.y = __builtin_fmaf(m[k], rv.y, t2.y);
      t2.z = __builtin_fmaf(m[k], rv.z, t2.z); t2.w = __builtin_fmaf(m[k], rv.w, t2.w);
    }
  }
  wpart[w * HG_M + a] = t;
  wpart[4 * HG_M + w * HG_M + a] = t2;
  float4 sq = f4_zero();
  if ((int)threadIdx.x < n - row0) {
    const float4 v = rs[threadIdx.x];
    sq = make_float4(v.x * v.x, v.y * v.y, v.z * v.z, v.w * v.w);
  }
  sq = block_sum4(sq, sm);
  if (threadIdx.x < 4) cg_store_sc1(part + threadIdx.x, f4_get(sq, threadIdx.x));
  {
    const int c = w;
    float st = 0.f, st2 = 0.f;
#pragma unroll
    for (int q = 0; q < 4; ++q) {
      st += f4_get(wpart[q * HG_M + a], c);
      st2 += f4_get(wpart[4 * HG_M + q * HG_M + a], c);
    }
    cg_store_sc1(part + 4 + a * HG_NC + c, st);
    cg_store_sc1(part + 4 + HG_M * HG_NC + a * HG_NC + c, st2);
  }
}

static __device__ __forceinline__ void cg_reduce_step(const float* __restrict__ part, int nblk, const float* __restrict__ Einv,
                                                      int phase, int it, float tol2, CgState* __restrict__ cg, double* d_s,
                                                      float* t_s, float* rr_s) {
  const int a = threadIdx.x & 63, c = threadIdx.x >> 6;
  float ev[HG_M];
#pragma unroll
  for (int b = 0; b < HG_M; ++b) ev[b] = Einv[b * HG_M + a];
  const float rz_old = cg->rz[c];
  const float bbv = cg->bb[threadIdx.x & 3];
  float t = 0.f, t2 = 0.f, rrp = 0.f;
  const float* pa = part + 4 + a * HG_NC + c;
  for (int b0 = 0; b0 < nblk; b0 += 32) {
    float tv[32], t2v[32], rv[32];
#pragma unroll
    for (int u = 0; u < 32; ++u) {
      const long b = min(b0 + u, nblk - 1);
      const bool ok = b0 + u < nblk;
      tv[u] = r3d_keep(cg_load_sc1(pa + b * HG_PART), ok);
      t2v[u] = r3d_keep(cg_load_sc1(pa + b * HG_PART + HG_M * HG_NC), ok);
      rv[u] = r3d_keep(cg_load_sc1(part + b * HG_PART + (threadIdx.x & 3)), ok);
    }
#pragma unroll
    for (int u = 0; u < 32; ++u) { t += tv[u]; t2 += t2v[u]; rrp += rv[u]; }
  }
  if (threadIdx.x < HG_NC) rr_s[threadIdx.x] = rrp;
  d_s[a * HG_NC + c] = phase == 0 ? (double)t : (double)t - (double)t2;
  t_s[a * HG_NC + c] = t;
  __syncthreads();
  if (phase == 1) {
    const bool conv = rr_s[0] <= tol2 * __shfl(bbv, 0) && rr_s[1] <= tol2 * __shfl(bbv, 1) &&
                      rr_s[2] <= tol2 * __shfl(bbv, 2) && rr_s[3] <= tol2 * __shfl(bbv, 3);
    if (conv) {
      if (threadIdx.x == 0) { cg->done = 1; cg->iters = it; }
      return;
    }
  }
  double m4[4] = {0.0, 0.0, 0.0, 0.0};
#pragma unroll
  for (int b = 0; b < HG_M; b += 4) {
#pragma unroll
    for (int e = 0; e < 4; ++e) m4[e] += (double)ev[b + e] * d_s[(b + e) * HG_NC + c];
  }
  const float mu = (float)((m4[0] + m4[1]) + (m4[2] + m4[3]));
  float tm = t_s[a * HG_NC + c] * mu;
  tm = r3d_wave_sum(tm);
  cg->mu[a * HG_NC + c] = mu;
  if (a == 0) {
    if (phase == 0) {
      cg->bb[c] = rr_s[c];
    } else {
      const float rz = rr_s[c] + tm;
      cg->beta[c] = (it > 0 && rz_old > 0.f) ? rz / rz_old : 0.f;
      cg->rz[c] = rz;
    }
  }
  if (threadIdx.x == 0) {
    if (phase == 0) { cg->done = 0; cg->iters = 0; }
    else cg->iters = it;
  }
}

static __device__ __forceinline__ bool cg_delivered_last(CgState* __restrict__ cg, int nblk, int* flag) {
  asm volatile("s_waitcnt vmcnt(0)" ::: "memory");
  __syncthreads();
  if (threadIdx.x == 0) {
    const unsigned t = __hip_atomic_fetch_add(&cg->ticket, 1u, __ATOMIC_RELAXED, __HIP_MEMORY_SCOPE_AGENT);
    *flag = (t + 1u) % (unsigned)nblk == 0u;
    __builtin_amdgcn_fence(__ATOMIC_ACQUIRE, "wavefront");
  }
  __syncthreads();
  return *flag != 0;
}

__global__ __launch_bounds__(256) void r3d_cg_init_kernel(const float4* __restrict__ B, const float* __restrict__ dinv,
                                                          const int* __restrict__ agg, const float* __restrict__ MW,
                                                          const int* __restrict__ n_dev, int n_cap, int mode,
                                                          float4* __restrict__ x, float4* __restrict__ r,
                                                          float4* __restrict__ p, float4* __restrict__ q,
                                                          float* __restrict__ part, const float* __restrict__ Einv, float tol2,
                                                          CgState* __restrict__ cg, HgEp st, long b_stride, long x_stride) {
  {
    const int ep = blockIdx.y;
    HG_AT(B, b_stride); HG_WS(dinv); HG_WS(agg); HG_WS(MW); HG_AT(n_dev, st.desc); HG_AT(x, x_stride); HG_WS(r); HG_WS(p); HG_WS(q);
    HG_WS(part); HG_WS(Einv); HG_WS(cg);
  }
  __shared__ float4 sm[4];
  __shared__ float4 rs[HG_UROWS];
  __shared__ float us[HG_UROWS];
  __shared__ int ag[HG_UROWS];
  __shared__ __attribute__((aligned(16))) float mu_s[HG_M * HG_NC];
  __shared__ float4 wpart[2 * 4 * HG_M];
  __shared__ double d_s[HG_M * HG_NC];
  __shared__ float t_s[HG_M * HG_NC];
  __shared__ float rr_s[HG_NC];
  __shared__ int last_s;
  __shared__ float tile_s[4 * 32 * 65];
  __shared__ float4 dot_s[HG_UROWS];
  const int row0 = blockIdx.x * HG_UROWS;
  float m[64];
  if (mode == 1) cg_load_mw_column(MW, row0, n_cap, m);
  const int n = min(*n_dev, n_cap);
  if (mode == 1) mu_s[threadIdx.x] = cg->mu[threadIdx.x];
  __syncthreads();
  if (mode == 1) {
    const int lane = threadIdx.x & 63, w = threadIdx.x >> 6;
    float* tl = tile_s + w * (32 * 65);
#pragma unroll
    for (int h = 0; h < 2; ++h) {
#pragma unroll
      for (int k = 0; k < 32; ++k) tl[k * 65 + lane] = m[32 * h + k];
      __builtin_amdgcn_wave_barrier();
      const int rk = lane & 31, a0 = 32 * (lane >> 5);
      float4 acc = f4_zero();
#pragma unroll 8
      for (int a = 0; a < 32; ++a) {
        const float mv = tl[rk * 65 + a0 + a];
        const float4 cv = *reinterpret_cast<const float4*>(&mu_s[(a0 + a) * HG_NC]);
// ... 187 lines not shown
          float4 rj[6];
#pragma unroll
          for (int u = 0; u < 6; ++u) rj[u] = rs[jv[u]];
#pragma unroll
          for (int u = 0; u < 6; ++u) {
            s.x = __builtin_fmaf(av[u], rj[u].x, s.x); s.y = __builtin_fmaf(av[u], rj[u].y, s.y);
            s.z = __builtin_fmaf(av[u], rj[u].z, s.z); s.w = __builtin_fmaf(av[u], rj[u].w, s.w);
          }
        }
        for (int e0 = rb + 384; e0 < re; e0 += 384) {
          int j2[6];
          float a2[6];
#pragma unroll
          for (int u = 0; u < 6; ++u) {
            const int e = e0 + lane + 64 * u;
            const int ec = min(e, re - 1);
            j2[u] = col[ec];
            a2[u] = r3d_keep(val[ec], e < re);
          }
#pragma unroll
          for (int u = 0; u < 6; ++u) {
            const float4 rj = rs[j2[u]];
            s.x = __builtin_fmaf(a2[u], rj.x, s.x); s.y = __builtin_fmaf(a2[u], rj.y, s.y);
            s.z = __builtin_fmaf(a2[u], rj.z, s.z); s.w = __builtin_fmaf(a2[u], rj.w, s.w);
          }
        }
        s.x = __builtin_fmaf(mw, mul.x, -alpha_lp * s.x); s.y = __builtin_fmaf(mw, mul.y, -alpha_lp * s.y);
        s.z = __builtin_fmaf(mw, mul.z, -alpha_lp * s.z); s.w = __builtin_fmaf(mw, mul.w, -alpha_lp * s.w);
        acc[kk] = s;
#pragma unroll
        for (int u = 0; u < 6; ++u) { jv[u] = jn[u]; av[u] = an[u]; }
        mw = mwn;
      }
    }
    float4 a4[4], a2[2], a1;
    {
      const bool hi = (lane & 32) != 0;
#pragma unroll
      for (int t = 0; t < 4; ++t) {
        const float4 keepv = hi ? acc[4 + t] : acc[t], sendv = hi ? acc[t] : acc[4 + t];
        a4[t].x = keepv.x + __shfl_xor(sendv.x, 32); a4[t].y = keepv.y + __shfl_xor(sendv.y, 32);
        a4[t].z = keepv.z + __shfl_xor(sendv.z, 32); a4[t].w = keepv.w + __shfl_xor(sendv.w, 32);
      }
    }
    {
      const bool hi = (lane & 16) != 0;
#pragma unroll
      for (int t = 0; t < 2; ++t) {
        const float4 keepv = hi ? a4[2 + t] : a4[t], sendv = hi ? a4[t] : a4[2 + t];
        a2[t].x = keepv.x + __shfl_xor(sendv.x, 16); a2[t].y = keepv.y + __shfl_xor(sendv.y, 16);
        a2[t].z = keepv.z + __shfl_xor(sendv.z, 16); a2[t].w = keepv.w + __shfl_xor(sendv.w, 16);
      }
    }
    {
      const bool hi = (lane & 8) != 0;
      const float4 keepv = hi ? a2[1] : a2[0], sendv = hi ? a2[0] : a2[1];
      a1.x = keepv.x + __shfl_xor(sendv.x, 8); a1.y = keepv.y + __shfl_xor(sendv.y, 8);
      a1.z = keepv.z + __shfl_xor(sendv.z, 8); a1.w = keepv.w + __shfl_xor(sendv.w, 8);
    }
#pragma unroll
    for (int o = 4; o > 0; o >>= 1) {
      a1.x += __shfl_xor(a1.x, o); a1.y += __shfl_xor(a1.y, o);
      a1.z += __shfl_xor(a1.z, o); a1.w += __shfl_xor(a1.w, o);
    }
    tot[h] = a1;
  }
  float4 acc_pq = f4_zero();
  const int trow = 8 * (lane & 7) + (lane >> 3);
  if ((lane & 7) < 2 && trow < nrows) {
    const float4 keep = (lane & 1) ? tot[1] : tot[0];
    const int i = row_of(trow);
    const float4 ri = rs[i], pi = p[i], qi = q[i];
    const float u = 1.f / dinv[i];
    const float4 m = mu_s[agg[i]];
    const float4 pn = make_float4((ri.x + u * m.x) + beta.x * pi.x, (ri.y + u * m.y) + beta.y * pi.y,
                                  (ri.z + u * m.z) + beta.z * pi.z, (ri.w + u * m.w) + beta.w * pi.w);
    const float4 qn = make_float4((ri.x + keep.x) + beta.x * qi.x, (ri.y + keep.y) + beta.y * qi.y,
                                  (ri.z + keep.z) + beta.z * qi.z, (ri.w + keep.w) + beta.w * qi.w);
    p[i] = pn;
    q[i] = qn;
    acc_pq = make_float4(pn.x * qn.x, pn.y * qn.y, pn.z * qn.z, pn.w * qn.w);
  }
  if ((lane & 7) < 2) pq_s[SL_WAVES * trow + w] = acc_pq;
  __syncthreads();
  if (tid < SL_ROWS / 4) {
    const float4 a = pq_s[4 * tid], b2 = pq_s[4 * tid + 1], c2 = pq_s[4 * tid + 2], d2 = pq_s[4 * tid + 3];
    const float4 t = make_float4(((a.x + b2.x) + c2.x) + d2.x, ((a.y + b2.y) + c2.y) + d2.y, ((a.z + b2.z) + c2.z) + d2.z,
                                 ((a.w + b2.w) + c2.w) + d2.w);
    const int gidx = tid * n_wg + bx;
    if (gidx < n_part) part_pq[gidx] = t;
  }
}

#ifdef CG_STAMPS
__device__ unsigned long long g_cg_dbg[32];
#define CSTAMP(i) do { if (it == 3 && threadIdx.x == 0 && blockIdx.x == 0) g_cg_dbg[i] = __builtin_amdgcn_s_memtime(); } while (0)
#define CSTAMP_LAST(i) do { if (it == 3 && threadIdx.x == 0) g_cg_dbg[16 + i] = __builtin_amdgcn_s_memtime(); } while (0)
extern "C" int r3d_cg_debug_read(unsigned long long* out32) {
  return hipMemcpyFromSymbol(out32, HIP_SYMBOL(g_cg_dbg), sizeof(g_cg_dbg)) == hipSuccess ? 0 : 1;
}
#else
#define CSTAMP(i)
#define CSTAMP_LAST(i)
#endif

__global__ __launch_bounds__(256) void r3d_cg_update_kernel(
    const int* __restrict__ n_dev, int n_cap, int it, int nblk_pq, const float* __restrict__ dinv, const int* __restrict__ agg,
    const float* __restrict__ MW, const float4* __restrict__ p, const float4* __restrict__ q, float4* __restrict__ x,
    float4* __restrict__ r, const float4* __restrict__ part_pq, float* __restrict__ part, const float* __restrict__ Einv,
    float tol2, CgState* __restrict__ cg, HgEp st, long x_stride) {
  __shared__ float4 sm[4];
  __shared__ float4 rs[HG_UROWS];
  __shared__ float us[HG_UROWS];
  __shared__ int ag[HG_UROWS];
  __shared__ float4 wpart[2 * 4 * HG_M];
  __shared__ double d_s[HG_M * HG_NC];
  __shared__ float t_s[HG_M * HG_NC];
  __shared__ float rr_s[HG_NC];
  __shared__ int last_s;
  {
    const int ep = blockIdx.y;
    HG_AT(n_dev, st.desc); HG_WS(dinv); HG_WS(agg); HG_WS(MW); HG_WS(p); HG_WS(q); HG_AT(x, x_stride); HG_WS(r); HG_WS(part_pq);
    HG_WS(part); HG_WS(Einv); HG_WS(cg);
  }
  const int row0 = blockIdx.x * HG_UROWS;
  const int i = row0 + threadIdx.x;
  const int ic = min(i, n_cap - 1);
  float m[64];
  CSTAMP(0);
  cg_load_mw_column(MW, row0, n_cap, m);
  const float4 pi = p[ic], qi = q[ic];
  float4 xi = x[ic], ri = r[ic];
  const float dv = dinv[ic];
  const int av = agg[ic];
  const int done = cg->done;
  const float4 rz = *reinterpret_cast<const float4*>(cg->rz);
  const int n = min(*n_dev, n_cap);
  const float4 pq = reduce_partials(part_pq, nblk_pq, sm);
  CSTAMP(1);
  if (done) return;
  float4 al;
  al.x = pq.x > 0.f ? rz.x / pq.x : 0.f;
  al.y = pq.y > 0.f ? rz.y / pq.y : 0.f;
  al.z = pq.z > 0.f ? rz.z / pq.z : 0.f;
  al.w = pq.w > 0.f ? rz.w / pq.w : 0.f;
  float u = 0.f;
  int a = 0;
  if (i < n) {
    xi.x += al.x * pi.x; xi.y += al.y * pi.y; xi.z += al.z * pi.z; xi.w += al.w * pi.w;
    ri.x -= al.x * qi.x; ri.y -= al.y * qi.y; ri.z -= al.z * qi.z; ri.w -= al.w * qi.w;
    x[i] = xi; r[i] = ri;
    u = 1.f / dv;
    a = av;
  } else {
    ri = f4_zero();
  }
  rs[threadIdx.x] = ri; us[threadIdx.x] = u; ag[threadIdx.x] = a;
  __syncthreads();
  CSTAMP(2);
  cg_block_partials(rs, us, ag, row0, n, m, true, part + (long)blockIdx.x * HG_PART, sm, wpart);
  CSTAMP(3);
  const bool last = cg_delivered_last(cg, gridDim.x, &last_s);
  CSTAMP(4);
  if (last) {
    CSTAMP_LAST(0);
    cg_reduce_step(part, gridDim.x, Einv, 1, it + 1, tol2, cg, d_s, t_s, rr_s);
    CSTAMP_LAST(1);
  }
}

__global__ __launch_bounds__(1024) void r3d_logits_ce_kernel(const float4* __restrict__ Z, const float4* __restrict__ Z2,
                                                             const int* __restrict__ desc_nproto, int n_q, int N, int n_classes,
                                                             const long long* __restrict__ labels,
                                                             float* __restrict__ logits ,
                                                             float* __restrict__ loss_out, int* __restrict__ pred_out, HgEp st) {
  __shared__ float red[16];
  {
    const int ep = blockIdx.x;
    HG_AT(Z, st.z); HG_AT(desc_nproto, st.desc); HG_AT(logits, st.logits);
    if (Z2) HG_AT(Z2, st.z);
    if (labels) HG_AT(labels, st.labels);
    if (loss_out) HG_AT(loss_out, st.loss);
    if (pred_out) HG_AT(pred_out, st.pred);
  }
  const int n_proto = *desc_nproto;
  float acc = 0.f;
  for (int e = threadIdx.x; e < n_q * N; e += blockDim.x) {
    const int qi = e / N, p = e - qi * N;
    const float4 z = Z[n_proto + e];
    const float4 z2 = Z2 ? Z2[n_proto + e] : f4_zero();
    const float zv[8] = {z.x, z.y, z.z, z.w, z2.x, z2.y, z2.z, z2.w};
    float mx = zv[0];
    int am = 0;
    for (int c = 1; c < n_classes; ++c) if (zv[c] > mx) { mx = zv[c]; am = c; }
    float se = 0.f;
    for (int c = 0; c < n_classes; ++c) {
      logits[((long)qi * n_classes + c) * N + p] = zv[c];
      se += expf(zv[c] - mx);
    }
    if (labels) {
      const int lab = (int)labels[e];
      acc += (mx + logf(se)) - zv[lab];
    }
    if (pred_out) pred_out[e] = am;
  }
  acc = r3d_wave_sum(acc);
  if ((threadIdx.x & 63) == 0) red[threadIdx.x >> 6] = acc;
  __syncthreads();
  if (threadIdx.x == 0) {
    float t = 0.f;
    for (int w = 0; w < (int)(blockDim.x >> 6); ++w) t += red[w];
    if (loss_out) *loss_out = t / (float)(n_q * N);
  }
}

struct LpWs {
  unsigned *outb, *sym;
  int *row_len, *row_ptr, *agg;
  hg_col_t* col;
  float *val, *dinv, *wdir, *MW, *Epart, *part;
  float* Einv;
  float4 *r, *p, *q, *part_pq;
  CgState* cg;
  long words, total;
};

static inline long hg_vblocks(int n_cap) { return r3d_cdiv(n_cap, HG_UROWS); }

static LpWs lp_carve(int32_t* ws, int n_cap, int kp1) {
  LpWs L;
  L.words = (n_cap + 31) / 32;
  const long nnz_cap = 2L * n_cap * (kp1 - 1);
  int32_t* wp = ws;
  auto align4 = [&]() { wp += (4 - ((wp - ws) & 3)) & 3; };
  L.outb = (unsigned*)wp; wp += n_cap * L.words;
  L.sym = (unsigned*)wp; wp += n_cap * L.words;
  L.row_len = wp; wp += n_cap + 8;
  L.row_ptr = wp; wp += n_cap + 8;
  L.col = (hg_col_t*)wp; wp += (nnz_cap + 1) / 2;
  L.val = (float*)wp; wp += nnz_cap;
  L.wdir = (float*)wp; wp += 2 * nnz_cap;
  L.dinv = (float*)wp; wp += n_cap;
  L.agg = wp; wp += n_cap;
  align4();
  L.MW = (float*)wp; wp += (long)n_cap * HG_M;
  L.Epart = (float*)wp; wp += (long)HG_EBLOCKS * HG_M * HG_M;
  align4();
  L.Einv = (float*)wp; wp += (long)HG_M * HG_M;
  L.part = (float*)wp; wp += hg_vblocks(n_cap) * HG_PART;
  align4();
  L.r = (float4*)wp; wp += 4L * n_cap;
  L.p = (float4*)wp; wp += 4L * n_cap;
  L.q = (float4*)wp; wp += 4L * n_cap;
  L.part_pq = (float4*)wp; wp += 4L * HG_MAX_PART;
  L.cg = (CgState*)wp; wp += (sizeof(CgState) + 3) / 4;
  L.total = (wp - ws) + 64;
  return L;
}

extern "C" long r3d_lp_ws_words(int n_cap, int kp1) { return lp_carve(nullptr, n_cap, kp1).total; }

extern "C" int r3d_lp_ws_offsets(int n_cap, int kp1, long* out6) {
  R3D_REQUIRE(out6 && n_cap > 0 && kp1 >= 2, "r3d_lp_ws_offsets: bad arguments");
  const LpWs L = lp_carve(nullptr, n_cap, kp1);
  const int32_t* base = nullptr;
  out6[0] = (const int32_t*)L.row_ptr - base; out6[1] = (const int32_t*)L.col - base; out6[2] = (const int32_t*)L.val - base;
  out6[3] = (const int32_t*)L.dinv - base; out6[4] = (const int32_t*)L.agg - base; out6[5] = (const int32_t*)L.cg - base;
  return R3D_OK;
}

__global__ void r3d_weights_compare_kernel(const int* __restrict__ row_ptr, const int* __restrict__ n_dev, int n_cap,
                                           const float* __restrict__ wdir, const float* __restrict__ wdir2, long scratch_stride,
                                           int* __restrict__ mismatch, HgEp st) {
  const int ep = blockIdx.y;
  HG_WS(row_ptr); HG_AT(n_dev, st.desc); HG_WS(wdir);
  wdir2 += (long)ep * scratch_stride;
  const int n = min(*n_dev, n_cap);
  const long nnz2 = 2L * row_ptr[n];
  int bad = 0;
  for (long e = (long)blockIdx.x * blockDim.x + threadIdx.x; e < nnz2; e += (long)gridDim.x * blockDim.x)
    bad += __float_as_uint(wdir[e]) != __float_as_uint(wdir2[e]) ? 1 : 0;
  bad = (int)r3d_wave_sum((float)bad);
  if ((threadIdx.x & 63) == 0 && bad) atomicAdd(mismatch, bad);
}
extern "C" long r3d_graph_weights_verify_words(int n_cap, int kp1) {
  const long nnz_cap = 2L * n_cap * (kp1 - 1);
  return 2 * nnz_cap + nnz_cap + n_cap + 64;
}
extern "C" int r3d_graph_weights_verify(int n_ep, const float* nodes, long ldn, int D, const int32_t* n_dev, long desc_stride,
                                        int n_cap, int kp1, float sigma, int32_t* ws, long ws_words, long ws_stride,
                                        float* scratch, int32_t* mismatch_out, void* stream) {
  R3D_REQUIRE(nodes && n_dev && ws && scratch && mismatch_out, "r3d_graph_weights_verify: null pointer");
  R3D_REQUIRE(n_cap > 0 && kp1 >= 2 && ws_words >= r3d_lp_ws_words(n_cap, kp1) && n_ep >= 1 &&
                  (n_ep == 1 || ((ws_stride & 3) == 0 && ws_stride >= ws_words)),
              "r3d_graph_weights_verify: bad arguments");
  hipStream_t st = (hipStream_t)stream;
  const LpWs L = lp_carve(ws, n_cap, kp1);
  const long nnz_cap = 2L * n_cap * (kp1 - 1), per = r3d_graph_weights_verify_words(n_cap, kp1);
  for (int e = 0; e < n_ep; ++e) {
    HgEp one{};
    float* base = scratch + (long)e * per;
    int32_t* wse = ws + (long)e * ws_stride;
    const LpWs Le = lp_carve(wse, n_cap, kp1);
    hipLaunchKernelGGL(r3d_graph_weights_kernel, dim3(n_cap, 1), dim3(256), 0, st, nodes + (long)e * n_cap * ldn, ldn, D, Le.outb,
                       (int)Le.words, n_dev + (long)e * desc_stride, n_cap, Le.row_ptr, Le.col, sigma, base + 2 * nnz_cap,
                       base + 3 * nnz_cap, base, one);
  }
  HgEp ep{};
  ep.desc = desc_stride; ep.ws = ws_stride;
  hipLaunchKernelGGL(r3d_weights_compare_kernel, dim3(256, n_ep), dim3(256), 0, st, L.row_ptr, n_dev, n_cap, L.wdir, scratch, per,
                     mismatch_out, ep);
  R3D_LAUNCH_CHECK("r3d_graph_weights_verify");
  return R3D_OK;
}

__global__ void r3d_cg_stats_kernel(const CgState* __restrict__ cg, int* __restrict__ stats_out, HgEp st) {
  const int ep = blockIdx.x;
  HG_WS(cg); HG_AT(stats_out, st.stats);
  if (threadIdx.x == 0) { stats_out[0] = cg->done; stats_out[1] = cg->iters; }
}

static int lp_coarse_space(const LpWs& L, const float* nodes, long ldn, int D, const int32_t* n_dev, const int32_t* n_proto_dev,
                           int n_cap, float alpha, int n_ep, const HgEp& ep, hipStream_t st) {
  const int agg_rpw = 4;
  const size_t agg_lds = ((size_t)HG_M * (D | 1) + 4 * D) * sizeof(float);
  static bool lds_opt_in = false;
  if (!lds_opt_in) {
    hipFuncSetAttribute((const void*)r3d_cg_aggregate_kernel, hipFuncAttributeMaxDynamicSharedMemorySize, 96 * 1024);
    lds_opt_in = true;
  }
  hipLaunchKernelGGL(r3d_cg_aggregate_kernel, dim3(r3d_cdiv(n_cap, 4 * agg_rpw), n_ep), dim3(256), agg_lds, st, nodes, ldn, D,
                     n_dev, n_proto_dev, n_cap, agg_rpw, L.agg, ep);
  hipLaunchKernelGGL(r3d_cg_mw_kernel, dim3(r3d_cdiv(n_cap, 4), n_ep), dim3(256), 0, st, L.row_ptr, L.col, L.val, L.dinv, L.agg,
                     n_dev, n_cap, alpha, 1, L.MW, ep);
  hipLaunchKernelGGL(r3d_cg_epart_kernel, dim3(HG_EBLOCKS, n_ep), dim3(128), 0, st, L.MW, L.dinv, L.agg, n_dev, n_cap, L.Epart,
                     ep);
  hipLaunchKernelGGL(r3d_cg_einv_kernel, dim3(n_ep), dim3(1024), 0, st, L.Epart, L.Einv, ep);
  return R3D_OK;
}

static int g_cg_lds_min_blocks = 256;
extern "C" int r3d_debug_set_cg_spmv_lds_min_blocks(int min_blocks) {
  const int old = g_cg_lds_min_blocks;
  g_cg_lds_min_blocks = min_blocks;
  return old;
}

static int lp_solve(const LpWs& L, const float* RHS, long rhs_stride, const int32_t* n_dev, int n_cap, float alpha, int max_iter,
                    float tol, float* X, long x_stride, int32_t* stats_out, int n_ep, const HgEp& ep, hipStream_t st) {
  const int nblk_v = (int)hg_vblocks(n_cap);
  int rpb = HG_ROWS_PER_BLOCK_MIN;
  while (r3d_cdiv(n_cap, rpb) > HG_MAX_PART) rpb += 4;
  const int nblk_s = r3d_cdiv(n_cap, rpb);
  R3D_REQUIRE(nblk_s <= HG_MAX_PART, "r3d_label_propagate: n_cap too large");
  float4* x = (float4*)X;
  const float tol2 = tol * tol;
  r3d_fill_words_ep(&L.cg->ticket, 0u, 1, n_ep, ep.ws, st);
  for (int mode = 0; mode < 2; ++mode)
    hipLaunchKernelGGL(r3d_cg_init_kernel, dim3(nblk_v, n_ep), dim3(256), 0, st, (const float4*)RHS, L.dinv, L.agg, L.MW, n_dev,
                       n_cap, mode, x, L.r, L.p, L.q, L.part, L.Einv, tol2, L.cg, ep, rhs_stride, x_stride);
  const size_t lds_r = (size_t)n_cap * sizeof(float4);
  const bool use_lds = lds_r <= SL_MAX_LDS && rpb == HG_ROWS_PER_BLOCK_MIN && (long)n_ep * r3d_cdiv(n_cap, SL_ROWS) >= g_cg_lds_min_blocks;
  if (use_lds) {
    static size_t attr = 0;
    if (lds_r > attr) {
      hipError_t e = hipFuncSetAttribute((const void*)r3d_cg_spmv_lds_kernel, hipFuncAttributeMaxDynamicSharedMemorySize, (int)lds_r);
      R3D_REQUIRE(e == hipSuccess, "r3d_label_propagate: cannot reserve %zu B of LDS: %s", lds_r, hipGetErrorString(e));
      attr = lds_r;
    }
  }
  const int nblk_l = r3d_cdiv(n_cap, SL_ROWS);
  const int nblk_pq = nblk_s;
  for (int it = 0; it < max_iter; ++it) {
    if (use_lds)
      hipLaunchKernelGGL(r3d_cg_spmv_lds_kernel, dim3(nblk_l, n_ep), dim3(64 * SL_WAVES), lds_r, st, L.row_ptr, L.col, L.val, L.dinv,
                         L.agg, L.MW, n_dev, n_cap, alpha, it, SL_ROWS, L.r, L.p, L.q, L.part_pq, L.cg, ep);
    else
      hipLaunchKernelGGL(r3d_cg_spmv_kernel, dim3(nblk_s, n_ep), dim3(256), 0, st, L.row_ptr, L.col, L.val, L.dinv, L.agg, L.MW,
                         n_dev, n_cap, alpha, it, rpb, L.r, L.p, L.q, L.part_pq, L.cg, ep);
    hipLaunchKernelGGL(r3d_cg_update_kernel, dim3(nblk_v, n_ep), dim3(256), 0, st, n_dev, n_cap, it, nblk_pq, L.dinv, L.agg, L.MW,
                       L.p, L.q, x, L.r, L.part_pq, L.part, L.Einv, tol2, L.cg, ep, x_stride);
  }
  if (stats_out) hipLaunchKernelGGL(r3d_cg_stats_kernel, dim3(n_ep), dim3(64), 0, st, L.cg, stats_out, ep);
  return R3D_OK;
}

static int label_propagate_impl(int n_ep, const HgEp& ep, const float* nodes, long ldn, int D, const int32_t* nbr, int kp1,
                                const float* Y, const int32_t* n_dev, const int32_t* n_proto_dev, int n_cap, float sigma,
                                float alpha, int max_iter, float tol, float* Z, int32_t* ws, long ws_words, int32_t* stats_out,
                                void* stream) {
  R3D_REQUIRE(nodes && nbr && Y && n_dev && n_proto_dev && Z && ws, "r3d_label_propagate: null pointer");
  R3D_REQUIRE(n_cap > 0 && kp1 >= 2 && ws_words >= r3d_lp_ws_words(n_cap, kp1),
              "r3d_label_propagate: workspace of %ld words, r3d_lp_ws_words(%d, %d) = %ld needed", ws_words, n_cap, kp1,
              n_cap > 0 && kp1 >= 2 ? r3d_lp_ws_words(n_cap, kp1) : -1L);
  R3D_REQUIRE((ldn & 3) == 0 && ((uintptr_t)nodes & 15) == 0,
              "r3d_label_propagate: node rows are read as float4: ldn must be a multiple of 4 and nodes 16-byte aligned");
  R3D_REQUIRE(n_cap > 0 && n_cap <= 32768 && D > 0 && D <= 256 && (D & 3) == 0 && kp1 >= 2,
              "r3d_label_propagate: unsupported n_cap=%d D=%d kp1=%d", n_cap, D, kp1);
  R3D_REQUIRE(max_iter > 0 && max_iter <= HG_MAX_ITER && sigma > 0.f, "r3d_label_propagate: bad solver parameters");
  R3D_REQUIRE(((uintptr_t)ws & 15) == 0 && ((uintptr_t)Y & 15) == 0 && ((uintptr_t)Z & 15) == 0,
              "r3d_label_propagate: ws, Y and Z must be 16-byte aligned");
  R3D_REQUIRE(n_ep >= 1 && n_ep <= 4096 && (n_ep == 1 || ((ep.ws & 3) == 0 && ep.ws >= ws_words)),
              "r3d_label_propagate: %d systems need a scratch stride that is a multiple of 4 words and >= the scratch size", n_ep);
  hipStream_t st = (hipStream_t)stream;
  const LpWs L = lp_carve(ws, n_cap, kp1);
  const long words = L.words;
  hipLaunchKernelGGL(r3d_graph_bits_kernel, dim3(r3d_cdiv(n_cap, 4), n_ep), dim3(256), 0, st, nbr, kp1, n_dev, n_cap,
                     (int)words, L.outb, ep);
  hipLaunchKernelGGL(r3d_graph_transpose_kernel, dim3(r3d_cdiv(words, BT_CW), r3d_cdiv(n_cap, BT_ROWS), n_ep), dim3(256), 0, st,
                     L.outb, (int)words, n_cap, L.sym, ep);
  hipLaunchKernelGGL(r3d_graph_rowlen_kernel, dim3(r3d_cdiv(n_cap, 4), n_ep), dim3(256), 0, st, L.sym, L.outb, (int)words,
                     n_dev, n_cap, L.row_len, ep);
  hipLaunchKernelGGL(r3d_scan_kernel, dim3(n_ep), dim3(1024), 0, st, L.row_len, n_cap, L.row_ptr, ep);
  hipLaunchKernelGGL(r3d_graph_cols_kernel, dim3(r3d_cdiv(n_cap, 4), n_ep), dim3(256), 0, st, L.sym, (int)words, n_dev,
                     n_cap, L.row_ptr, L.col, ep);
  hipLaunchKernelGGL(r3d_graph_weights_kernel, dim3(n_cap, n_ep), dim3(256), 0, st, nodes, ldn, D, L.outb,
                     (int)words, n_dev, n_cap, L.row_ptr, L.col, sigma, L.val, L.dinv, L.wdir, ep);
  hipLaunchKernelGGL(r3d_graph_normalize_kernel, dim3(r3d_cdiv(n_cap, 4), n_ep), dim3(256), 0, st, L.row_ptr, L.col, L.dinv,
                     n_dev, n_cap, L.val, ep);
  int rc = lp_coarse_space(L, nodes, ldn, D, n_dev, n_proto_dev, n_cap, alpha, n_ep, ep, st);
  if (rc) return rc;
  rc = lp_solve(L, Y, ep.y, n_dev, n_cap, alpha, max_iter, tol, Z, ep.z, stats_out, n_ep, ep, st);
  if (rc) return rc;
  R3D_LAUNCH_CHECK("r3d_label_propagate");
  return R3D_OK;
}

extern "C" int r3d_label_propagate(const float* nodes, long ldn, int D, const int32_t* nbr, int kp1,
                                   const float* Y, const int32_t* n_dev, const int32_t* n_proto_dev, int n_cap, float sigma,
                                   float alpha, int max_iter, float tol, float* Z, int32_t* ws, long ws_words,
                                   int32_t* stats_out, void* stream) {
  const HgEp one{};
  return label_propagate_impl(1, one, nodes, ldn, D, nbr, kp1, Y, n_dev, n_proto_dev, n_cap, sigma, alpha, max_iter, tol, Z, ws,
                              ws_words, stats_out, stream);
}

extern "C" int r3d_label_propagate_solve_batched(int n_ep, const float* Y, const int32_t* n_dev, long desc_stride, int n_cap,
                                                 int kp1, float alpha, int max_iter, float tol, float* Z, int32_t* ws,
                                                 long ws_words, long ws_stride, int32_t* stats_out, long stats_stride,
                                                 void* stream) {
  R3D_REQUIRE(Y && n_dev && Z && ws, "r3d_label_propagate_solve: null pointer");
  R3D_REQUIRE(n_cap > 0 && kp1 >= 2 && ws_words >= r3d_lp_ws_words(n_cap, kp1), "r3d_label_propagate_solve: workspace too short");
  R3D_REQUIRE(max_iter > 0 && max_iter <= HG_MAX_ITER, "r3d_label_propagate_solve: bad solver parameters");
  R3D_REQUIRE(((uintptr_t)ws & 15) == 0 && ((uintptr_t)Y & 15) == 0 && ((uintptr_t)Z & 15) == 0,
              "r3d_label_propagate_solve: ws, Y and Z must be 16-byte aligned");
  R3D_REQUIRE(n_ep >= 1 && n_ep <= 4096 && (n_ep == 1 || ((ws_stride & 3) == 0 && ws_stride >= ws_words)),
              "r3d_label_propagate_solve: bad scratch stride");
  HgEp ep{};
  ep.nodes = ep.nbr = ep.y = ep.z = n_cap;
  ep.desc = desc_stride; ep.ws = ws_stride; ep.stats = stats_stride;
  const LpWs L = lp_carve(ws, n_cap, kp1);
  const int rc = lp_solve(L, Y, ep.y, n_dev, n_cap, alpha, max_iter, tol, Z, ep.z, stats_out, n_ep, ep, (hipStream_t)stream);
  if (rc) return rc;
  R3D_LAUNCH_CHECK("r3d_label_propagate_solve");
  return R3D_OK;
}

extern "C" int r3d_label_propagate_batched(int n_ep, const float* nodes, long ldn, int D, const int32_t* nbr, int kp1,
                                           const float* Y, const int32_t* n_dev, const int32_t* n_proto_dev, long desc_stride,
                                           int n_cap, float sigma, float alpha, int max_iter, float tol, float* Z, int32_t* ws,
                                           long ws_words, long ws_stride, int32_t* stats_out, long stats_stride, void* stream) {
  HgEp ep{};
  ep.nodes = ep.nbr = ep.y = ep.z = n_cap;
  ep.desc = desc_stride; ep.ws = ws_stride; ep.stats = stats_stride;
  return label_propagate_impl(n_ep, ep, nodes, ldn, D, nbr, kp1, Y, n_dev, n_proto_dev, n_cap, sigma, alpha, max_iter, tol, Z, ws,
                              ws_words, stats_out, stream);
}

static __device__ __forceinline__ float dot4(float4 a, float4 b) { return a.x * b.x + a.y * b.y + a.z * b.z + a.w * b.w; }

__global__ __launch_bounds__(256) void r3d_lp_bwd_dd_kernel(const int* __restrict__ row_ptr, const hg_col_t* __restrict__ col,
                                                            const float* __restrict__ val, const float* __restrict__ dinv,
                                                            const int* __restrict__ n_dev, int n_cap, float alpha,
                                                            const float4* __restrict__ lam, const float4* __restrict__ Z,
                                                            float* __restrict__ dD, HgEp st) {
  const int ep = blockIdx.y;
  HG_WS(row_ptr); HG_WS(col); HG_WS(val); HG_WS(dinv); HG_AT(n_dev, st.desc); HG_AT(lam, st.lam); HG_AT(Z, st.z); HG_WS(dD);
  const int n = min(*n_dev, n_cap);
  const int i = blockIdx.x * 4 + (threadIdx.x >> 6);
  const int lane = threadIdx.x & 63;
  if (i >= n) return;
  const float4 li = lam[i], zi = Z[i];
  const float di = dinv[i];
  float g = 0.f;
  for (int e = row_ptr[i] + lane; e < row_ptr[i + 1]; e += 64) {
    const int j = col[e];
    const float ds = alpha * (dot4(li, Z[j]) + dot4(lam[j], zi));
    g += ds * (val[e] / di);
  }
  g = r3d_wave_sum(g);
  if (lane == 0) dD[i] = -0.5f * di * di * di * g;
}

__global__ __launch_bounds__(256) void r3d_lp_bwd_dx_kernel(
    const float* __restrict__ nodes, long ldn, int D, const float* __restrict__ wdir,
    const int* __restrict__ row_ptr, const hg_col_t* __restrict__ col, const float* __restrict__ dinv,
    const int* __restrict__ n_dev, int n_cap, float sigma, float alpha, const float4* __restrict__ lam,
    const float4* __restrict__ Z, const float* __restrict__ dD, float* __restrict__ dnodes, long ldd, HgEp st) {
  {
    const int ep = blockIdx.y;
    nodes += (long)ep * st.nodes * ldn; HG_WS(wdir); HG_WS(row_ptr); HG_WS(col); HG_WS(dinv); HG_AT(n_dev, st.desc);
    HG_AT(lam, st.lam); HG_AT(Z, st.z); HG_WS(dD); dnodes += (long)ep * st.dn * ldd;
  }
  __shared__ float acc_s[4][256];
  __shared__ float uv_s[4][2];
  const int n = min(*n_dev, n_cap);
  const int w = threadIdx.x >> 6;
  const int i = blockIdx.x;
  const int lane = threadIdx.x & 63;
  if (i >= n) return;
  const float* xi = nodes + (long)i * ldn;
  const float4 li = lam[i], zi = Z[i];
  const float di = dinv[i], ddi = dD[i];
  const int beg = row_ptr[i], end = row_ptr[i + 1];
  const float inv_s2 = 1.f / (sigma * sigma);
  const int c0 = min(lane, D - 1), c1 = min(lane + 64, D - 1), c2 = min(lane + 128, D - 1), c3 = min(lane + 192, D - 1);
  float U = 0.f, V = 0.f;
  float a0 = 0.f, a1 = 0.f, a2 = 0.f, a3 = 0.f;
  for (int e0 = beg + 64 * w; e0 < end; e0 += 256) {
    const int e = e0 + lane;
    const bool ok = e < end;
    const int ec = min(e, end - 1);
    const int j = col[ec];
    const float2 wd = *reinterpret_cast<const float2*>(wdir + 2L * ec);
    const float dj = dinv[j];
    const float T = alpha * (dot4(li, Z[j]) + dot4(lam[j], zi)) * di * dj + ddi + dD[j];
    const float cij = ok ? -T * wd.x * inv_s2 : 0.f;
    const float cji = ok ? -T * wd.y * inv_s2 : 0.f;
    const float u = cij + cji;
    U += u;
    V += cij - cji;
    const int cnt = min(64, end - e0);
    int t = 0;
    for (; t + 8 <= cnt; t += 8) {
      float x0[8], x1[8], x2[8], x3[8], ut[8];
#pragma unroll
      for (int q = 0; q < 8; ++q) {
        ut[q] = r3d_readlane_f(u, t + q);
        const float* xr = nodes + (long)__builtin_amdgcn_readlane(j, t + q) * ldn;
        x0[q] = xr[c0]; x1[q] = xr[c1]; x2[q] = xr[c2];
        x3[q] = D > 192 ? xr[c3] : 0.f;
      }
#pragma unroll
      for (int q = 0; q < 8; ++q) {
        a0 = __builtin_fmaf(ut[q], x0[q], a0); a1 = __builtin_fmaf(ut[q], x1[q], a1);
        a2 = __builtin_fmaf(ut[q], x2[q], a2); a3 = __builtin_fmaf(ut[q], x3[q], a3);
      }
    }
    for (; t < cnt; ++t) {
      const float ut = r3d_readlane_f(u, t);
      const float* xr = nodes + (long)__builtin_amdgcn_readlane(j, t) * ldn;
      a0 = __builtin_fmaf(ut, xr[c0], a0); a1 = __builtin_fmaf(ut, xr[c1], a1);
      a2 = __builtin_fmaf(ut, xr[c2], a2); a3 = __builtin_fmaf(ut, D > 192 ? xr[c3] : 0.f, a3);
    }
  }
  U = r3d_wave_sum(U);
  V = r3d_wave_sum(V);
  acc_s[w][lane] = a0; acc_s[w][64 + lane] = a1; acc_s[w][128 + lane] = a2; acc_s[w][192 + lane] = a3;
  if (lane == 0) { uv_s[w][0] = U; uv_s[w][1] = V; }
  __syncthreads();
  const int c = threadIdx.x;
  if (c < D) {
    const float At = ((acc_s[0][c] + acc_s[1][c]) + acc_s[2][c]) + acc_s[3][c];
    const float Ut = ((uv_s[0][0] + uv_s[1][0]) + uv_s[2][0]) + uv_s[3][0];
    const float Vt = ((uv_s[0][1] + uv_s[1][1]) + uv_s[2][1]) + uv_s[3][1];
    dnodes[(long)i * ldd + c] = xi[c] * Ut - At + 1e-6f * Vt;
  }
}

__global__ void r3d_ce_grad_kernel(const float4* __restrict__ Z, const int* __restrict__ n_proto_dev, int n_cap, int n_qpts,
                                   int n_classes, const long long* __restrict__ labels, const float* __restrict__ gscale,
                                   float4* __restrict__ G, const float4* __restrict__ Z2, float4* __restrict__ G2, HgEp st) {
  {
    const int ep = blockIdx.y;
    HG_AT(Z, st.z); HG_AT(n_proto_dev, st.desc); HG_AT(labels, st.labels); HG_AT(G, st.g);
    if (Z2) { HG_AT(Z2, st.z); HG_AT(G2, st.g); }
  }
  const int i = blockIdx.x * blockDim.x + threadIdx.x;
  if (i >= n_cap) return;
  const int n_proto = *n_proto_dev;
  const int q = i - n_proto;
  float g[8] = {0.f, 0.f, 0.f, 0.f, 0.f, 0.f, 0.f, 0.f};
  if (q >= 0 && q < n_qpts) {
    const float4 z = Z[i];
    const float4 z2 = Z2 ? Z2[i] : f4_zero();
    const float zv[8] = {z.x, z.y, z.z, z.w, z2.x, z2.y, z2.z, z2.w};
    float mx = zv[0];
    for (int c = 1; c < n_classes; ++c) mx = fmaxf(mx, zv[c]);
    float se = 0.f;
    for (int c = 0; c < n_classes; ++c) se += expf(zv[c] - mx);
    const int lab = (int)labels[q];
    const float sc = gscale[0] / (float)n_qpts;
    for (int c = 0; c < n_classes; ++c) g[c] = (expf(zv[c] - mx) / se - (c == lab ? 1.f : 0.f)) * sc;
  }
  G[i] = make_float4(g[0], g[1], g[2], g[3]);
  if (G2) G2[i] = make_float4(g[4], g[5], g[6], g[7]);
}

static int label_propagate_bwd_impl(int n_ep, const HgEp& ep, const float* nodes, long ldn, int D, int kp1, const float* Z,
                                    const float* G, const int32_t* n_dev, int n_cap, float sigma, float alpha, int max_iter,
                                    float tol, float* lam, float* dnodes, long ldd, int32_t* ws, long ws_words,
                                    int32_t* stats_out, void* stream) {
  R3D_REQUIRE(nodes && Z && G && n_dev && lam && dnodes && ws, "r3d_label_propagate_bwd: null pointer");
  R3D_REQUIRE(n_cap > 0 && kp1 >= 2 && ws_words >= r3d_lp_ws_words(n_cap, kp1),
              "r3d_label_propagate_bwd: workspace of %ld words is shorter than r3d_lp_ws_words(%d, %d)", ws_words, n_cap, kp1);
  R3D_REQUIRE((ldn & 3) == 0 && ((uintptr_t)nodes & 15) == 0 && ((uintptr_t)ws & 15) == 0 && ((uintptr_t)Z & 15) == 0 &&
                  ((uintptr_t)G & 15) == 0 && ((uintptr_t)lam & 15) == 0,
              "r3d_label_propagate_bwd: ldn must be a multiple of 4; nodes, ws, Z, G, lam 16-byte aligned");
  R3D_REQUIRE(n_cap > 0 && n_cap <= 32768 && D > 0 && D <= 256 && max_iter > 0 && max_iter <= HG_MAX_ITER,
              "r3d_label_propagate_bwd: bad arguments");
  R3D_REQUIRE(n_ep >= 1 && n_ep <= 4096 && (n_ep == 1 || ((ep.ws & 3) == 0 && ep.ws >= ws_words)),
              "r3d_label_propagate_bwd: %d systems need a scratch stride that is a multiple of 4 words and >= the scratch size", n_ep);
  hipStream_t st = (hipStream_t)stream;
  const LpWs L = lp_carve(ws, n_cap, kp1);
  int rc = lp_solve(L, G, ep.g, n_dev, n_cap, alpha, max_iter, tol, lam, ep.lam, stats_out, n_ep, ep, st);
  if (rc) return rc;
  float* dD = (float*)L.q;
  hipLaunchKernelGGL(r3d_lp_bwd_dd_kernel, dim3(r3d_cdiv(n_cap, 4), n_ep), dim3(256), 0, st, L.row_ptr, L.col, L.val, L.dinv, n_dev,
                     n_cap, alpha, (const float4*)lam, (const float4*)Z, dD, ep);
  hipLaunchKernelGGL(r3d_lp_bwd_dx_kernel, dim3(n_cap, n_ep), dim3(256), 0, st, nodes, ldn, D, L.wdir,
                     L.row_ptr, L.col, L.dinv, n_dev, n_cap, sigma, alpha, (const float4*)lam, (const float4*)Z, dD, dnodes,
                     ldd, ep);
  R3D_LAUNCH_CHECK("r3d_label_propagate_bwd");
  return R3D_OK;
}
extern "C" int r3d_label_propagate_bwd(const float* nodes, long ldn, int D, int kp1, const float* Z, const float* G,
                                       const int32_t* n_dev, int n_cap, float sigma, float alpha, int max_iter, float tol,
                                       float* lam, float* dnodes, long ldd, int32_t* ws, long ws_words, int32_t* stats_out,
                                       void* stream) {
  const HgEp one{};
  return label_propagate_bwd_impl(1, one, nodes, ldn, D, kp1, Z, G, n_dev, n_cap, sigma, alpha, max_iter, tol, lam, dnodes, ldd,
                                  ws, ws_words, stats_out, stream);
}
extern "C" int r3d_label_propagate_bwd_batched(int n_ep, const float* nodes, long ldn, int D, int kp1, const float* Z,
                                               const float* G, const int32_t* n_dev, long desc_stride, int n_cap, float sigma,
                                               float alpha, int max_iter, float tol, float* lam, float* dnodes, long ldd,
                                               int32_t* ws, long ws_words, long ws_stride, int32_t* stats_out,
                                               long stats_stride, void* stream) {
  HgEp ep{};
  ep.nodes = ep.z = ep.g = ep.lam = ep.dn = n_cap;
  ep.desc = desc_stride; ep.ws = ws_stride; ep.stats = stats_stride;
  return label_propagate_bwd_impl(n_ep, ep, nodes, ldn, D, kp1, Z, G, n_dev, n_cap, sigma, alpha, max_iter, tol, lam, dnodes, ldd,
                                  ws, ws_words, stats_out, stream);
}

extern "C" int r3d_ce_grad_batched(int n_ep, const float* Z, const int32_t* n_proto_dev, long desc_stride, int n_cap,
                                   int n_query_pts, int n_classes, const int64_t* labels, const float* gscale_dev, float* G,
                                   void* stream) {
  R3D_REQUIRE(Z && n_proto_dev && labels && gscale_dev && G && n_ep >= 1 && n_ep <= 65535, "r3d_ce_grad: bad arguments");
  R3D_REQUIRE(n_classes >= 2 && n_classes <= 2 * HG_NC, "r3d_ce_grad: %d classes (2..%d)", n_classes, 2 * HG_NC);
  HgEp ep{};
  ep.z = ep.g = n_cap; ep.desc = desc_stride; ep.labels = n_query_pts;
  const long plane = (long)n_ep * n_cap;
  const float4* Z2 = n_classes > HG_NC ? (const float4*)Z + plane : nullptr;
  float4* G2 = n_classes > HG_NC ? (float4*)G + plane : nullptr;
  hipLaunchKernelGGL(r3d_ce_grad_kernel, dim3(r3d_cdiv(n_cap, 256), n_ep), dim3(256), 0, (hipStream_t)stream, (const float4*)Z,
                     n_proto_dev, n_cap, n_query_pts, n_classes, (const long long*)labels, gscale_dev, (float4*)G, Z2, G2, ep);
  R3D_LAUNCH_CHECK("r3d_ce_grad");
  return R3D_OK;
}
extern "C" int r3d_ce_grad(const float* Z, const int32_t* n_proto_dev, int n_cap, int n_query_pts, int n_classes,
                           const int64_t* labels, const float* gscale_dev, float* G, void* stream) {
  return r3d_ce_grad_batched(1, Z, n_proto_dev, 0, n_cap, n_query_pts, n_classes, labels, gscale_dev, G, stream);
}

extern "C" int r3d_query_logits_ce_batched(int n_ep, const float* Z, long z_ep_rows, const int32_t* n_proto_dev, long desc_stride,
                                           int n_q, int N, int n_classes, const int64_t* labels, float* logits, float* loss_out,
                                           int32_t* pred_out, void* stream) {
  R3D_REQUIRE(Z && n_proto_dev && logits, "r3d_query_logits_ce: null pointer");
  R3D_REQUIRE(n_q > 0 && N > 0 && n_classes >= 2 && n_classes <= 2 * HG_NC && n_ep >= 1, "r3d_query_logits_ce: bad shape");
  R3D_REQUIRE(n_classes <= HG_NC || z_ep_rows > 0, "r3d_query_logits_ce: more than %d classes need the batched form "
              "(Z as two planes (2, n_ep * z_ep_rows, 4))", HG_NC);
  HgEp ep{};
  ep.z = z_ep_rows; ep.desc = desc_stride; ep.labels = (long)n_q * N; ep.logits = (long)n_q * n_classes * N; ep.loss = 1;
  ep.pred = (long)n_q * N;
  const float4* Z2 = n_classes > HG_NC ? (const float4*)Z + (long)n_ep * z_ep_rows : nullptr;
  hipLaunchKernelGGL(r3d_logits_ce_kernel, dim3(n_ep), dim3(1024), 0, (hipStream_t)stream, (const float4*)Z, Z2,
                     n_proto_dev, n_q, N, n_classes, (const long long*)labels, logits, loss_out, pred_out, ep);
  R3D_LAUNCH_CHECK("r3d_query_logits_ce");
  return R3D_OK;
}
extern "C" int r3d_query_logits_ce(const float* Z, const int32_t* n_proto_dev, int n_q, int N, int n_classes,
                                   const int64_t* labels, float* logits, float* loss_out, int32_t* pred_out,
                                   void* stream) {
  return r3d_query_logits_ce_batched(1, Z, 0, n_proto_dev, 0, n_q, N, n_classes, labels, logits, loss_out, pred_out, stream);
}

extern "C" int r3d_graph_set_lp_budget(void* graph, void* graph_exec, int budget, int* n_cg) {
  R3D_REQUIRE(graph && graph_exec && budget > 0, "r3d_graph_set_lp_budget: bad arguments");
  hipGraph_t g = (hipGraph_t)graph;
  hipGraphExec_t ge = (hipGraphExec_t)graph_exec;
  size_t n = 0;
  R3D_REQUIRE(hipGraphGetNodes(g, nullptr, &n) == hipSuccess, "r3d_graph_set_lp_budget: hipGraphGetNodes failed");
  hipGraphNode_t* nodes = (hipGraphNode_t*)malloc(sizeof(hipGraphNode_t) * (n ? n : 1));
  R3D_REQUIRE(nodes, "r3d_graph_set_lp_budget: out of memory");
  int found = 0, rc = R3D_OK;
  if (hipGraphGetNodes(g, nodes, &n) != hipSuccess) rc = R3D_ERR_LAUNCH;
  for (size_t i = 0; rc == R3D_OK && i < n; ++i) {
    hipGraphNodeType ty;
    if (hipGraphNodeGetType(nodes[i], &ty) != hipSuccess) { rc = R3D_ERR_LAUNCH; break; }
    if (ty != hipGraphNodeTypeKernel) continue;
    hipKernelNodeParams kp;
    if (hipGraphKernelNodeGetParams(nodes[i], &kp) != hipSuccess) { rc = R3D_ERR_LAUNCH; break; }
    int it, on;
    if (kp.func == (void*)r3d_cg_spmv_kernel || kp.func == (void*)r3d_cg_spmv_lds_kernel) { it = *(const int*)kp.kernelParams[9]; on = it < budget; }
    else if (kp.func == (void*)r3d_cg_update_kernel) { it = *(const int*)kp.kernelParams[2]; on = it < budget; }
    else continue;
    ++found;
    if (hipGraphNodeSetEnabled(ge, nodes[i], on ? 1u : 0u) != hipSuccess) { rc = R3D_ERR_LAUNCH; break; }
  }
  free(nodes);
  if (rc != R3D_OK) {
    r3d_set_error("r3d_graph_set_lp_budget: HIP graph call failed: %s", hipGetErrorString(hipGetLastError()));
    return rc;
  }
  if (n_cg) *n_cg = found;
  return R3D_OK;
}
```

r3dfsseg_amd/train_ops.py:

```python
import ctypes
from types import SimpleNamespace

import torch

from . import _lib, ops
from .ops import SegLayout, _p, _rows, _st, _timed

BN_EPS, BN_MOM = 1e-5, 0.1
update_running_stats = True


class BNRecorder:

    def __init__(self, max_episodes, device):
        self.max_records = 2 * max_episodes
        self.device = device
        self.tables = {}
        self.index_dev = None

    def slot_for(self, bnmod, bias):
        if bnmod not in self.tables:
            rec = torch.zeros(self.max_records, 2, bnmod.num_features, device=self.device, dtype=torch.float32)
            self.tables[bnmod] = (rec, bias.detach() if bias is not None else None)
        return self.tables[bnmod][0]

    def apply(self, n_episodes):
        lib = _lib.load()
        assert 2 * n_episodes <= self.max_records
        with torch.no_grad():
            for bnmod, (rec, bias) in self.tables.items():
                C = bnmod.num_features
                _lib.check(lib.r3d_bn_running_update(_p(rec), 2 * n_episodes, 2 * C, C, BN_MOM, _p(bias),
                                                     _p(bnmod.running_mean), _p(bnmod.running_var), _st()))
                bnmod.num_batches_tracked += 2 * n_episodes


bn_recorder = None


class deferred_running_stats:

    def __init__(self, model):
        self.model = model

    def __enter__(self):
        global bn_recorder
        rec = self.model.__dict__.get("_bn_rec1")
        if rec is None:
            rec = self.model.__dict__["_bn_rec1"] = BNRecorder(1, next(self.model.parameters()).device)
        self.saved, bn_recorder = bn_recorder, rec
        return rec

    def __exit__(self, *exc):
        global bn_recorder
        bn_recorder = self.saved
        return False


def _f(n, dev):
    return torch.empty(n, device=dev, dtype=torch.float32)


class BNVec:

    def __init__(self, n_seg, C, dev):
        self.t = torch.empty(n_seg, 4, C, device=dev, dtype=torch.float32)
        self.stride = 4 * C

    @property
    def scale(self): return self.t[:, 0]
    @property
    def shift(self): return self.t[:, 1]
    @property
    def mean(self): return self.t[:, 2]
    @property
    def invstd(self): return self.t[:, 3]

    def ptrs(self):
        return _p(self.t[0, 0]), _p(self.t[0, 1]), _p(self.t[0, 2]), _p(self.t[0, 3])


def colstats(X, C, seg, mode=0, DY=None, bn=None, act=0):
    M, ldx = _rows(X)
    dev = X.device
    lib = _lib.load()
    sums = _f(seg.n_seg * 2 * C, dev).view(seg.n_seg, 2, C)
    ws = _f(lib.r3d_colstats_seg_ws_words(M, C, seg.rows_a, seg.rows_b), dev)
    lddy = DY.stride(0) if DY is not None else 0
    sc, sh, mu, is_ = bn.ptrs() if bn is not None else (None, None, None, None)
    with _timed("bn_stats"):
        _lib.check(lib.r3d_colstats_seg(_p(X), ldx, _p(DY), lddy, M, C, seg.rows_a, seg.rows_b, mode, sc, sh, mu, is_,
                                        bn.stride if bn is not None else 0, act, _p(sums), _p(ws), _st()))
    return sums


def bn_fold(sums, counts, bnmod, bias=None):
    n_seg, _, C = sums.shape
    dev = sums.device
    lib = _lib.load()
    bn = BNVec(n_seg, C, dev)
    rec = bn_recorder
    if rec is not None:
        table, idx_dev = rec.slot_for(bnmod, bias), rec.index_dev
    elif update_running_stats:
        table, idx_dev = torch.empty(n_seg, 2, C, device=dev, dtype=torch.float32), None
    else:
        table, idx_dev = None, None
    sc, sh, mu, is_ = bn.ptrs()
    _lib.check(lib.r3d_bn_fold_seg(_p(sums), n_seg, counts[0], counts[1], C, _p(bnmod.weight), _p(bnmod.bias), BN_EPS, BN_MOM,
                                   None, None, mu, is_, sc, sh, bn.stride, _p(table), _p(idx_dev), 2 * C, _st()))
    if rec is None and table is not None:
        with torch.no_grad():
            _lib.check(lib.r3d_bn_running_update(_p(table), n_seg, 2 * C, C, BN_MOM, _p(bias.detach()) if bias is not None else None,
                                                 _p(bnmod.running_mean), _p(bnmod.running_var), _st()))
            bnmod.num_batches_tracked += n_seg
    return bn


def affine_act(Z, bn, act, seg, out=None):
    M, ldz = _rows(Z)
    C = Z.shape[1]
    if out is None:
        out = torch.empty(M, C, device=Z.device, dtype=torch.float32)
    sc, sh, _, _ = bn.ptrs()
    _lib.check(_lib.load().r3d_affine_act_seg(_p(Z), ldz, M, C, seg.rows_a, seg.rows_b, sc, sh, bn.stride, act, _p(out),
                                              out.stride(0), _st()))
    return out


def bn_bwd_apply(Z, DY, bn, act, sums, counts, seg, out=None):
    M, ldz = _rows(Z)
    C = Z.shape[1]
    DZ = torch.empty(M, C, device=Z.device, dtype=torch.float32) if out is None else out
    sc, sh, mu, is_ = bn.ptrs()
    _lib.check(_lib.load().r3d_bn_bwd_apply_seg(_p(Z), ldz, _p(DY), DY.stride(0), M, C, seg.rows_a, seg.rows_b, sc, sh, mu, is_,
                                                bn.stride, act, _p(sums), counts[0], counts[1], _p(DZ), DZ.stride(0), _st()))
    return DZ


def gemm_tn(A, B):
    M, lda = _rows(A)
    M2, ldb = _rows(B)
    assert M == M2
    Ca, Cb = A.shape[1], B.shape[1]
    lib = _lib.load()
    out = torch.empty(Ca, Cb, device=A.device, dtype=torch.float32)
    ws = _f(lib.r3d_gemm_tn_ws_words(M, Ca, Cb), A.device)
    with _timed("gemm_tn"):
        _lib.check(lib.r3d_gemm_tn(_p(A), lda, _p(B), ldb, M, Ca, Cb, 1.0, _p(out), 0, _p(ws), _st()))
    return out


def conv_acc(X, W, out):
    M, ldx = _rows(X)
    with _timed("pointwise_conv"):
        _lib.check(_lib.load().r3d_pointwise_conv_acc(_p(X), ldx, _p(W), M, X.shape[1], W.shape[0], None, None, 0, _p(out),
                                                      out.stride(0), _st()))


def add_cols(src, dst):
    M, lds = _rows(src)
    _lib.check(_lib.load().r3d_add_cols(_p(src), lds, _p(dst), dst.stride(0), M, src.shape[1], _st()))


def _one_segment(M):
    return SegLayout(1, 1, 0, M)


def conv_bn_fwd(X, W2d, bnmod, act, bias=None, out=None, seg=None):
    M, ldx = _rows(X)
    C = W2d.shape[0]
    lib = _lib.load()
    seg = _one_segment(M) if seg is None else seg
    assert seg.M == M
    z = torch.empty(M, C, device=X.device, dtype=torch.float32)
    if seg.aligned(64):
        sums = _f(seg.n_seg * 2 * C, X.device).view(seg.n_seg, 2, C)
        ws = _f(lib.r3d_pointwise_conv_stats_ws_words(M, C), X.device)
        with _timed("pointwise_conv"):
            _lib.check(lib.r3d_pointwise_conv_stats_seg(_p(X), ldx, _p(W2d), M, X.shape[1], C, _p(z), C, seg.rows_a, seg.rows_b,
                                                        _p(sums), _p(ws), _st()))
    else:
        ops.pointwise_conv(X, W2d, out=z)
        sums = colstats(z, C, seg, mode=0)
    bn = bn_fold(sums, seg.counts(), bnmod, bias)
    y = affine_act(z, bn, act, seg, out=out)
    return y, (X, W2d, z, bn, act, seg)


def conv_bn_bwd(saved, dY, want_dx=True, dx_acc=None):
    X, W2d, z, bn, act, seg = saved
    C = W2d.shape[0]
    M = z.shape[0]
    sums = colstats(z, C, seg, mode=1, DY=dY, bn=bn, act=act)
    dz = bn_bwd_apply(z, dY, bn, act, sums, seg.counts(), seg)
    dW = gemm_tn(dz, X)
    tot = sums.sum(0) if seg.n_seg > 1 else sums[0]
    dbias = torch.zeros(C, device=z.device, dtype=torch.float32)
    dX = None
    if want_dx:
        Wt = W2d.t().contiguous()
        if dx_acc is not None:
            conv_acc(dz, Wt, dx_acc)
        else:
            dX = ops.pointwise_conv(dz, Wt)
    return dW, tot[1], tot[0], dbias, dX


def edgeconv_train_fwd(inp, idx, ec, B, N, out, seg=None):
    lib = _lib.load()
    dev = inp.device
    seg = SegLayout(1, B, 0, N) if seg is None else seg
    assert seg.B == B and seg.N == N
    W1 = ec.layer[0].weight.reshape(64, -1)
    C = W1.shape[1] // 2
    Wpq = torch.cat((W1[:, :C], W1[:, C:] - W1[:, :C]), 0).contiguous()
    PQ = ops.pointwise_conv(inp, Wpq)
    K = idx.shape[-1]
    ws = _f(lib.r3d_edgeconv_train_ws_words(B, N), dev)
    W2 = ec.layer[3].weight.reshape(64, 64).contiguous()
    M = B * N
    argmax = torch.empty(M, 64, device=dev, dtype=torch.int32)
    argmin = torch.empty(M, 64, device=dev, dtype=torch.int32)
    zmax = torch.empty(M, 64, device=dev, dtype=torch.float32)
    zmin = torch.empty(M, 64, device=dev, dtype=torch.float32)
    idx3 = idx.view(B, N, K)
    sums1 = _f(seg.n_seg * 128, dev).view(seg.n_seg, 2, 64)
    sums2 = _f(seg.n_seg * 128, dev).view(seg.n_seg, 2, 64)
    counts = seg.counts(per_row=K)
    esum = torch.empty(M, 64, device=dev, dtype=torch.float32)
    with _timed("edgeconv"):
        _lib.check(lib.r3d_edge_stats1(_p(PQ), _p(idx3), B, N, K, seg.S, seg.Q, _p(sums1), _p(esum), _p(ws), _st()))
    bn1 = bn_fold(sums1, counts, ec.layer[1])
    sc1, sh1, _, _ = bn1.ptrs()
    with _timed("edgeconv"):
        _lib.check(lib.r3d_edgeconv_train_fwd_minmax(_p(PQ), _p(idx3), sc1, sh1, bn1.stride, _p(W2), B, N, K, seg.S, seg.Q,
                                                     _p(zmax), _p(zmin), _p(argmax), _p(argmin), _p(sums2), _p(ws), _st()))
    bn2 = bn_fold(sums2, counts, ec.layer[4])
    sc2, sh2, _, _ = bn2.ptrs()
    with _timed("edgeconv"):
        _lib.check(lib.r3d_edge_select(_p(zmax), _p(zmin), _p(argmax), _p(argmin), sc2, sh2, bn2.stride, M, seg.rows_a,
                                       seg.rows_b, _p(out), out.stride(0), _st()))
    return (inp, idx3, Wpq, PQ, W2, bn1, bn2, argmax, zmax, C, seg, esum)


def edgeconv_train_bwd(saved, dout, B, N, dx_acc):
    inp, idx3, Wpq, PQ, W2, bn1, bn2, argmax, zmax, C, seg, esum = saved
    lib = _lib.load()
    dev = PQ.device
    K = idx3.shape[-1]
    M = B * N
    dPQ = _f(M * 128, dev).view(M, 128)
    ws = _f(lib.r3d_edgeconv_train_ws_words(B, N), dev)
    rev = torch.empty(lib.r3d_edge_reverse_ws_words(B, N, K), device=dev, dtype=torch.int32)
    with _timed("edgeconv_bwd"):
        _lib.check(lib.r3d_edge_reverse(_p(idx3), B, N, K, _p(rev), rev.numel(), _st()))
    bn2_sums = colstats(zmax, 64, seg, mode=1, DY=dout, bn=bn2, act=ops.ACT_LRELU)
    DY1, BE = _f(M * K * 64, dev), _f(M * 128, dev)
    dW2, bn1_sums = _f(64 * 64, dev), _f(seg.n_seg * 128, dev).view(seg.n_seg, 2, 64)
    s1, t1, m1, i1 = bn1.ptrs()
    s2, t2, m2, i2 = bn2.ptrs()
    with _timed("edgeconv_bwd"):
        _lib.check(lib.r3d_edgeconv_bwd(_p(PQ), _p(idx3), s1, t1, m1, i1, _p(W2), s2, t2, m2, i2, bn1.stride, _p(bn2_sums),
                                        _p(dout), dout.stride(0), _p(argmax), _p(zmax), _p(esum), B, N, K, seg.S, seg.Q, _p(DY1),
                                        _p(BE), _p(rev),
                                        _p(dW2), _p(bn1_sums), _p(dPQ), _p(ws), _st()))
    t1s = bn1_sums.sum(0) if seg.n_seg > 1 else bn1_sums[0]
    t2s = bn2_sums.sum(0) if seg.n_seg > 1 else bn2_sums[0]
    dWpq = gemm_tn(dPQ, inp)
    dW1 = torch.cat((dWpq[:64] - dWpq[64:], dWpq[64:]), 1).reshape(64, 2 * C, 1, 1)
    if dx_acc is not None:
        conv_acc(dPQ, Wpq.t().contiguous(), dx_acc)
    return dW1, t1s[1], t1s[0], dW2.view(64, 64, 1, 1), t2s[1], t2s[0]


class EncoderTrainFn(torch.autograd.Function):

    @staticmethod
    def forward(ctx, x, model, seed, *params):
        enc, base, att = model.encoder, model.base_learner, model.att_learner
        lib = _lib.load()
        B, _, N = x.shape
        M = B * N
        dev = x.device
        seg = getattr(ctx, "seg", None)
        if seg is None:
            seg = SegLayout(1, B, 0, N)
        assert seg.B == B and seg.N == N
        x_pm, x_cm = ops.input_layouts(x)
        cat = torch.empty(M, 64 * enc.n_edgeconv, device=dev, dtype=torch.float32)
        inp, ec_saved = x_pm, []
        for l in range(enc.n_edgeconv):
            idx = ops.knn(inp, B, N, enc.k, x_cm=x_cm if l == 0 else None)
            if enc.idx_patch is not None:
                idx = enc.idx_patch(l, idx.view(B, N, enc.k)).view(idx.shape)
            out = cat[:, 64 * l:64 * (l + 1)]
            ec_saved.append(edgeconv_train_fwd(inp, idx, enc.edge_convs[l], B, N, out, seg))
            inp = out
        h, mlp_saved = cat, []
        for jn in range(len(enc.conv.layer_dims)):
            W = enc.conv.layer[3 * jn].weight
            h, sv = conv_bn_fwd(h, W.reshape(W.shape[0], -1).contiguous(), enc.conv.layer[3 * jn + 1], ops.ACT_LRELU, seg=seg)
            mlp_saved.append(sv)
        level2 = h
        feat = torch.empty(M, model.feat_dim, device=dev, dtype=torch.float32)
        od = att.out_channel
        ops.copy_cols(cat[:, :64], feat[:, :64])
        hb, base_saved = level2, []
        for i, seq in enumerate(base.convs):
            last = i == base.num_convs - 1
            W = seq[0].weight
            hb, sv = conv_bn_fwd(hb, W.reshape(W.shape[0], -1).contiguous(), seq[1], ops.ACT_NONE if last else ops.ACT_RELU,
                                 bias=seq[0].bias, out=feat[:, 64 + od:] if last else None, seg=seg)
            base_saved.append(sv)
        Wqkv, qscale = att._fold()
        qkv = ops.pointwise_conv(level2, Wqkv, qscale, None, ops.ACT_NONE)
        lse = torch.empty(M, device=dev, dtype=torch.float32)
        p_drop = float(att.dropout.p)
        aws = _f(lib.r3d_attention_ws_words_ep_d(B, N, seg.clouds, od), dev)
        with _timed("attention"):
            _lib.check(lib.r3d_attention_fwd_train_ep_d(_p(qkv), 3 * od, B, N, _p(feat[:, 64:64 + od]), feat.stride(0), _p(lse),
                                                        p_drop, ctypes.c_uint(seed & 0xffffffff), _p(model._slot.seed_dev),
                                                        seg.clouds, od, _p(aws), _st()))
        ctx.model, ctx.dims, ctx.seed_dev, ctx.seg = model, (B, N, seed, p_drop), model._slot.seed_dev, seg
        model._dbg_idx = [sv[1] for sv in ec_saved]
        if getattr(model, "_trace", None) is not None:
            for e in range(seg.E):
                for b0, Bs in ((e * seg.clouds, seg.S), (e * seg.clouds + seg.S, seg.Q)):
                    if Bs:
                        model._trace.setdefault("idx", []).append([sv[1][b0:b0 + Bs] for sv in ec_saved])
                        model._trace.setdefault("argmax", []).append([sv[7][b0 * N:(b0 + Bs) * N] for sv in ec_saved])
        ctx.saved = (ec_saved, mlp_saved, base_saved, cat, level2, Wqkv, qkv, lse, feat, aws)
        return feat

    @staticmethod
    def backward(ctx, dfeat):
        model = ctx.model
        enc, base, att = model.encoder, model.base_learner, model.att_learner
        B, N, seed, p_drop = ctx.dims
        seg = ctx.seg
        ec_saved, mlp_saved, base_saved, cat, level2, Wqkv, qkv, lse, feat, aws = ctx.saved
        lib = _lib.load()
        dev = dfeat.device
        M = B * N
        dfeat = dfeat.contiguous()
        class _G(dict):
            def __setitem__(self, k, v):
                dict.__setitem__(self, id(k), v)
        g = _G()
        dlevel2 = torch.zeros(M, level2.shape[1], device=dev, dtype=torch.float32)
        od = att.out_channel
        d = dfeat[:, 64 + od:]
        for i in reversed(range(base.num_convs)):
            seq = base.convs[i]
            dW, dg, db, dbias, dX = conv_bn_bwd(base_saved[i], d, want_dx=True, dx_acc=dlevel2 if i == 0 else None)
            g[seq[0].weight] = dW.view_as(seq[0].weight)
            g[seq[0].bias] = dbias
            g[seq[1].weight], g[seq[1].bias] = dg, db
            d = dX
        dqkv = torch.empty(M, 3 * od, device=dev, dtype=torch.float32)
        with _timed("attention_bwd"):
            _lib.check(lib.r3d_attention_bwd_ep_d(_p(qkv), 3 * od, B, N, _p(feat[:, 64:64 + od]), feat.stride(0),
                                                  _p(dfeat[:, 64:64 + od]), dfeat.stride(0), _p(lse), p_drop,
                                                  ctypes.c_uint(seed & 0xffffffff), _p(ctx.seed_dev), seg.clouds, od,
                                                  1.0 / att.temperature, _p(dqkv), 3 * od, _p(aws), 1, _st()))
        dWqkv = gemm_tn(dqkv, level2)
        for k, m in enumerate((att.q_map, att.k_map, att.v_map)):
            g[m.weight] = dWqkv[od * k:od * (k + 1)].reshape(m.weight.shape)
        Wraw = torch.cat([m.weight.reshape(od, -1) for m in (att.q_map, att.k_map, att.v_map)], 0)
        conv_acc(dqkv, Wraw.t().contiguous(), dlevel2)
        dcat = torch.zeros(M, cat.shape[1], device=dev, dtype=torch.float32)
        add_cols(dfeat[:, :64], dcat[:, :64])
        d = dlevel2
        for jn in reversed(range(len(mlp_saved))):
            conv, bnm = enc.conv.layer[3 * jn], enc.conv.layer[3 * jn + 1]
            dW, dg, db, _, dX = conv_bn_bwd(mlp_saved[jn], d, want_dx=True, dx_acc=dcat if jn == 0 else None)
            g[conv.weight] = dW.view_as(conv.weight)
            g[bnm.weight], g[bnm.bias] = dg, db
            d = dX
        for l in reversed(range(enc.n_edgeconv)):
            ec = enc.edge_convs[l]
            dx_acc = dcat[:, 64 * (l - 1):64 * l] if l > 0 else None
            dW1, dg1, db1, dW2, dg2, db2 = edgeconv_train_bwd(ec_saved[l], dcat[:, 64 * l:64 * (l + 1)], B, N, dx_acc)
            g[ec.layer[0].weight], g[ec.layer[1].weight], g[ec.layer[1].bias] = dW1, dg1, db1
            g[ec.layer[3].weight], g[ec.layer[4].weight], g[ec.layer[4].bias] = dW2, dg2, db2
        ctx.saved = None
        return (None, None, None) + tuple(g.get(id(p)) for p in ctx.param_list)


def encoder_params(model):
    ps = list(model.encoder.parameters()) + list(model.base_learner.parameters()) + list(model.att_learner.parameters())
    return ps


def _adjacent_rows(a, b):
    base = a._base
    if base is None or base is not b._base or base.dim() != 2 or not base.is_contiguous():
        return None
    if not (a.is_contiguous() and b.is_contiguous() and a.dim() == 2 and b.dim() == 2 and a.shape[1] == b.shape[1] == base.shape[1]):
        return None
    if base.shape[0] != a.shape[0] + b.shape[0] or a.data_ptr() != base.data_ptr():
        return None
    if b.data_ptr() != base.data_ptr() + a.numel() * a.element_size():
        return None
    return base


def next_dropout_seed(model):
    slot = model._slot
    if slot.seed_dev is not None:
        slot.seed_dev.add_(2)
        return 0
    model._drop_seed = getattr(model, "_drop_seed", 0) + 2
    return model._drop_seed


def next_dropout_seeds(model, E):
    slot = model._slot
    if slot.seed_dev is not None:
        slot.seed_dev.add_(2 * E)
        return 2 - 2 * E
    seed = getattr(model, "_drop_seed", 0) + 2
    model._drop_seed = seed + 2 * (E - 1)
    return seed


def get_features_train(model, x, seed, seg=None):
    params = encoder_params(model)

    class _Fn(EncoderTrainFn):
        @staticmethod
        def forward(ctx, x, *ps):
            ctx.param_list = params
            ctx.seg = seg
            feat = EncoderTrainFn.forward(ctx, x, model, seed, *ps)
            if seg is None or seg.Q == 0:
                return feat
            assert seg.E == 1
            rows = seg.rows_a
            ctx.seg_shapes = ((rows, feat.shape[1]), (feat.shape[0] - rows, feat.shape[1]))
            return feat[:rows], feat[rows:]

        @staticmethod
        def backward(ctx, *dfeats):
            if len(dfeats) == 2:
                dfeats = [d if d is not None else torch.zeros(sh, device=ctx.saved[3].device, dtype=torch.float32)
                          for d, sh in zip(dfeats, ctx.seg_shapes)]
                dfeat = _adjacent_rows(*dfeats)
                if dfeat is None:
                    dfeat = torch.cat(dfeats, 0)
            else:
                dfeat = dfeats[0]
            out = EncoderTrainFn.backward(ctx, dfeat)
            return (None,) + out[3:]

    return _Fn.apply(x, *params)


def explicit_encoder_step(model, batch, grad_sink, head):
    E = batch.E
    S, N = model.n_way * model.k_shot, model.n_points
    Q = batch.query_x.shape[1]
    with torch.no_grad():
        seed = next_dropout_seeds(model, E)
        params = encoder_params(model)
        ctx = SimpleNamespace(param_list=params, seg=SegLayout(E, S, Q, N))
        feat = EncoderTrainFn.forward(ctx, batch.x_all.view(E * (S + Q), model.in_channels, N), model, seed)
        outputs, dfeat, extra = head(feat, ctx.seg)
        assert dfeat.shape[0] == feat.shape[0]
        grads = EncoderTrainFn.backward(ctx, dfeat)[3:]
        index = {id(p): i for i, p in enumerate(q for q in model.parameters() if q.requires_grad)}
        dst, src = [], []
        for p, g in list(zip(params, grads)) + extra:
            if g is not None:
                dst.append(grad_sink[index[id(p)]])
                src.append(g.reshape(p.shape))
        torch._foreach_add_(dst, src)
    return outputs


def mpti_train_forward(model, support_x, support_y, query_x, query_y, gt_support_y, gt_query_y, logger, support_flag):
    from . import head_train
    return head_train.mpti_train_forward(model, support_x, support_y, query_x, query_y, gt_support_y, gt_query_y, logger,
                                         support_flag)
```

Baseline: 393.6.

## Remap label-propagation grids across XCDs and drop redundant zero-fills and copies

Label-propagation and graph kernels now run on a 1D grid whose block-to-episode mapping interleaves eight episodes across consecutive block IDs. Blocks are dispatched round-robin to the XCDs, so this keeps each episode's blocks on one XCD and its L2. The edge-select kernel can also write a second output directly into the feature tensor, which removes a separate copy_cols. In the backward pass, the zero-initialised gradient buffers become uninitialised: the first conv writes into them instead of accumulating, and the add_cols moves after that write. This saves memsets and extra passes over memory, but correctness now depends on every column being written before it is read.

New measurement: 389.4. -1.1%, worse.

```diff
diff --git a/include/r3d.h b/include/r3d.h
--- a/include/r3d.h
+++ b/include/r3d.h
@@ -10,6 +10,9 @@
 int r3d_abi_version(void);
 int r3d_debug_poison_lds(unsigned pattern, unsigned* sink , void* stream);
 int r3d_debug_set_cg_spmv_lds_min_blocks(int min_blocks);
+int r3d_debug_set_lp_xcd_map(int on);
+int r3d_lp_xcd_grid(int n_blk, int n_ep);
+int r3d_lp_xcd_block(int id, int n_blk, int n_ep, int32_t* sys_blk );
 int r3d_set_matrix_arith(int mode);
 int r3d_get_matrix_arith(void);
 int r3d_debug_set_gemm_bx3(int mask);
@@ -147,6 +150,9 @@
 int r3d_edge_select(float* zmax , const float* zmin, int32_t* argmax ,
                     const int32_t* argmin, const float* s2, const float* t2, long bn_stride, long M, long rows_a, long rows_b,
                     float* out, long ldo, void* stream);
+int r3d_edge_select2(float* zmax, const float* zmin, int32_t* argmax, const int32_t* argmin, const float* s2,
+                     const float* t2, long bn_stride, long M, long rows_a, long rows_b, float* out, long ldo, float* out2,
+                     long ldo2, void* stream);
 long r3d_edge_reverse_ws_words(int B, int N, int K);
 int r3d_edge_reverse(const int32_t* idx, int B, int N, int K, int32_t* rev_ws, long ws_words, void* stream);
 int r3d_edgeconv_bwd(const float* PQ, const int32_t* idx, const float* s1, const float* t1, const float* mean1,
diff --git a/r3dfsseg_amd/_lib.py b/r3dfsseg_amd/_lib.py
--- a/r3dfsseg_amd/_lib.py
+++ b/r3dfsseg_amd/_lib.py
@@ -32,6 +32,9 @@
     "r3d_debug_poison_lds": (c_i, [c_u, c_f, c_f]),
     "r3d_debug_set_cg_spmv_lds_min_blocks": (c_i, [c_i]),
     "r3d_debug_set_gemm_bx3": (c_i, [c_i]),
+    "r3d_debug_set_lp_xcd_map": (c_i, [c_i]),
+    "r3d_lp_xcd_grid": (c_i, [c_i, c_i]),
+    "r3d_lp_xcd_block": (c_i, [c_i, c_i, c_i, ctypes.POINTER(ctypes.c_int32)]),
     "r3d_set_matrix_arith": (c_i, [c_i]),
     "r3d_get_matrix_arith": (c_i, []),
     "r3d_head_max_k": (c_i, []),
@@ -48,6 +51,7 @@
     "r3d_pointwise_conv_acc": (c_i, [c_f, c_l, c_f, c_l, c_i, c_i, c_f, c_f, c_i, c_f, c_l, c_f]),
     "r3d_edgeconv_train_fwd_minmax": (c_i, [c_f, c_f, c_f, c_f, c_l, c_f, c_i, c_i, c_i, c_i, c_i, c_f, c_f, c_f, c_f, c_f, c_f, c_f]),
     "r3d_edge_select": (c_i, [c_f, c_f, c_f, c_f, c_f, c_f, c_l, c_l, c_l, c_l, c_f, c_l, c_f]),
+    "r3d_edge_select2": (c_i, [c_f, c_f, c_f, c_f, c_f, c_f, c_l, c_l, c_l, c_l, c_f, c_l, c_f, c_l, c_f]),
     "r3d_pointwise_conv_stats_ws_words": (c_l, [c_l, c_i]),
     "r3d_pointwise_conv_stats": (c_i, [c_f, c_l, c_f, c_l, c_i, c_i, c_f, c_l, c_f, c_f, c_f]),
     "r3d_pointwise_conv_stats2": (c_i, [c_f, c_l, c_f, c_l, c_i, c_i, c_f, c_l, c_l, c_f, c_f, c_f, c_f]),
diff --git a/r3dfsseg_amd/csrc/common.h b/r3dfsseg_amd/csrc/common.h
--- a/r3dfsseg_amd/csrc/common.h
+++ b/r3dfsseg_amd/csrc/common.h
@@ -130,6 +130,25 @@
   return (x < r ? x * (q + 1) : r * (q + 1) + (x - r) * q) + (id >> 3);
 }
 
+struct r3d_sysblk {
+  int sys, blk;
+};
+static __host__ __device__ __forceinline__ r3d_sysblk r3d_xcd_system_block(int id, int n_blk, int n_ep, int xcd) {
+  r3d_sysblk s;
+  if (!xcd || n_ep < 8) {
+    s.sys = id / n_blk;
+    s.blk = id - s.sys * n_blk;
+    return s;
+  }
+  const int g = id / (8 * n_blk), in = id - g * (8 * n_blk);
+  s.sys = 8 * g + (in & 7);
+  s.blk = in >> 3;
+  return s;
+}
+static inline int r3d_xcd_system_grid(int n_blk, int n_ep, int xcd) {
+  return (!xcd || n_ep < 8) ? n_blk * n_ep : ((n_ep + 7) / 8) * 8 * n_blk;
+}
+
 struct r3d_segmap {
   long a, b;
   __host__ __device__ bool odd(int seg) const { return b > 0 && (seg & 1); }
diff --git a/r3dfsseg_amd/csrc/edgeconv_train.hip b/r3dfsseg_amd/csrc/edgeconv_train.hip
--- a/r3dfsseg_amd/csrc/edgeconv_train.hip
+++ b/r3dfsseg_amd/csrc/edgeconv_train.hip
@@ -669,7 +669,7 @@
 __global__ void r3d_edge_select_kernel(float* __restrict__ zmax, const float* __restrict__ zmin, int* __restrict__ argmax,
                                        const int* __restrict__ argmin, const float* __restrict__ s2,
                                        const float* __restrict__ t2, long bn_stride, r3d_segmap sm , long M,
-                                       float* __restrict__ out, long ldo) {
+                                       float* __restrict__ out, long ldo, float* __restrict__ out2, long ldo2) {
   const long i = (long)blockIdx.x * blockDim.x + threadIdx.x;
   if (i >= M * 64) return;
   const int c = (int)(i & 63);
@@ -679,18 +679,26 @@
   const bool up = sc >= 0.f;
   const float z = up ? zmax[i] : zmin[i];
   if (!up) { zmax[i] = z; argmax[i] = argmin[i]; }
-  out[m * ldo + c] = lrelu(sc * z + t2[bo]);
+  const float y = lrelu(sc * z + t2[bo]);
+  out[m * ldo + c] = y;
+  if (out2) out2[m * ldo2 + c] = y;
+}
+extern "C" int r3d_edge_select2(float* zmax, const float* zmin, int32_t* argmax, const int32_t* argmin, const float* s2,
+                                const float* t2, long bn_stride, long M, long rows_a, long rows_b, float* out, long ldo,
+                                float* out2, long ldo2, void* stream) {
+  R3D_REQUIRE(zmax && zmin && argmax && argmin && s2 && t2 && out && M > 0 && ldo >= 64 && (!out2 || ldo2 >= 64),
+              "r3d_edge_select: bad arguments");
+  const r3d_segmap sm{rows_a, rows_b};
+  R3D_REQUIRE(sm.covers(M), "r3d_edge_select: %ld rows are not whole segments of %ld + %ld rows", M, rows_a, rows_b);
+  hipLaunchKernelGGL(r3d_edge_select_kernel, dim3(r3d_cdiv(M * 64, 256)), dim3(256), 0, (hipStream_t)stream, zmax, zmin,
+                     argmax, argmin, s2, t2, bn_stride, sm, M, out, ldo, out2, ldo2);
+  R3D_LAUNCH_CHECK("r3d_edge_select");
+  return R3D_OK;
 }
 extern "C" int r3d_edge_select(float* zmax, const float* zmin, int32_t* argmax, const int32_t* argmin, const float* s2,
                                const float* t2, long bn_stride, long M, long rows_a, long rows_b, float* out, long ldo,
                                void* stream) {
-  R3D_REQUIRE(zmax && zmin && argmax && argmin && s2 && t2 && out && M > 0 && ldo >= 64, "r3d_edge_select: bad arguments");
-  const r3d_segmap sm{rows_a, rows_b};
-  R3D_REQUIRE(sm.covers(M), "r3d_edge_select: %ld rows are not whole segments of %ld + %ld rows", M, rows_a, rows_b);
-  hipLaunchKernelGGL(r3d_edge_select_kernel, dim3(r3d_cdiv(M * 64, 256)), dim3(256), 0, (hipStream_t)stream, zmax, zmin,
-                     argmax, argmin, s2, t2, bn_stride, sm, M, out, ldo);
-  R3D_LAUNCH_CHECK("r3d_edge_select");
-  return R3D_OK;
+  return r3d_edge_select2(zmax, zmin, argmax, argmin, s2, t2, bn_stride, M, rows_a, rows_b, out, ldo, nullptr, 0, stream);
 }
 
 template <int RT>
diff --git a/r3dfsseg_amd/csrc/head_graph.hip b/r3dfsseg_amd/csrc/head_graph.hip
--- a/r3dfsseg_amd/csrc/head_graph.hip
+++ b/r3dfsseg_amd/csrc/head_graph.hip
@@ -13,6 +13,30 @@
   long labels, logits, loss, pred;
 };
 #define HG_WS(p) p = (decltype(p))((const char*)(p) + (long)ep * st.ws * 4)
+struct HgGrid {
+  int n_blk, n_ep, xcd;
+};
+#define HG_SYSBLK(gr)                                                                          \
+  const r3d_sysblk sb_ = r3d_xcd_system_block((int)blockIdx.x, gr.n_blk, gr.n_ep, gr.xcd);     \
+  if (sb_.sys >= gr.n_ep) return;                              \
+  const int ep = sb_.sys, blk = sb_.blk
+static int g_lp_xcd_map = 1;
+extern "C" int r3d_debug_set_lp_xcd_map(int on) {
+  const int old = g_lp_xcd_map;
+  g_lp_xcd_map = on ? 1 : 0;
+  return old;
+}
+static inline HgGrid hg_grid(int n_blk, int n_ep) { return HgGrid{n_blk, n_ep, g_lp_xcd_map}; }
+static inline dim3 hg_dim(const HgGrid& g) { return dim3((unsigned)r3d_xcd_system_grid(g.n_blk, g.n_ep, g.xcd)); }
+extern "C" int r3d_lp_xcd_grid(int n_blk, int n_ep) { return r3d_xcd_system_grid(n_blk, n_ep, g_lp_xcd_map); }
+extern "C" int r3d_lp_xcd_block(int id, int n_blk, int n_ep, int32_t* sys_blk) {
+  R3D_REQUIRE(sys_blk && n_blk > 0 && n_ep > 0 && id >= 0 && id < r3d_xcd_system_grid(n_blk, n_ep, g_lp_xcd_map),
+              "r3d_lp_xcd_block: bad arguments");
+  const r3d_sysblk s = r3d_xcd_system_block(id, n_blk, n_ep, g_lp_xcd_map);
+  sys_blk[0] = s.sys;
+  sys_blk[1] = s.blk;
+  return R3D_OK;
+}
 #define HG_AT(p, stride) p += (long)ep * (stride)
 
 __global__ __launch_bounds__(256) void r3d_graph_bits_kernel(const int* __restrict__ nbr, int kp1, const int* __restrict__ n_dev,
@@ -132,11 +156,11 @@
 __global__ __launch_bounds__(256) void r3d_graph_cols_kernel(const unsigned* __restrict__ sym, int words,
                                                              const int* __restrict__ n_dev, int n_cap,
                                                              const int* __restrict__ row_ptr, hg_col_t* __restrict__ col,
-                                                             HgEp st) {
-  const int ep = blockIdx.y;
+                                                             HgEp st, HgGrid gr) {
+  HG_SYSBLK(gr);
   HG_WS(sym); HG_AT(n_dev, st.desc); HG_WS(row_ptr); HG_WS(col);
   const int n = min(*n_dev, n_cap);
-  const int i = blockIdx.x * 4 + (threadIdx.x >> 6);
+  const int i = blk * 4 + (threadIdx.x >> 6);
   const int lane = threadIdx.x & 63;
   if (i >= n) return;
   const int wpl = (words + 63) / 64;
@@ -168,15 +192,16 @@
 __global__ __launch_bounds__(256) void r3d_graph_weights_kernel(
     const float* __restrict__ nodes, long ldn, int D, const unsigned* __restrict__ outb, int words,
     const int* __restrict__ n_dev, int n_cap, const int* __restrict__ row_ptr, const hg_col_t* __restrict__ col,
-    float sigma, float* __restrict__ val, float* __restrict__ dinv, float* __restrict__ wdir , HgEp st) {
+    float sigma, float* __restrict__ val, float* __restrict__ dinv, float* __restrict__ wdir , HgEp st,
+    HgGrid gr) {
   __shared__ __attribute__((aligned(16))) float xs[256];
   __shared__ float wsum[4];
-  const int ep = blockIdx.y;
+  HG_SYSBLK(gr);
   nodes += (long)ep * st.nodes * ldn; HG_WS(outb); HG_AT(n_dev, st.desc); HG_WS(row_ptr); HG_WS(col); HG_WS(val); HG_WS(dinv);
   HG_WS(wdir);
   const int n = min(*n_dev, n_cap);
   const int w = threadIdx.x >> 6;
-  const int i = blockIdx.x;
+  const int i = blk;
   const int lane = threadIdx.x & 63;
   if (i >= n) return;
   const float* xi = nodes + (long)i * ldn;
@@ -240,11 +265,11 @@
 
 __global__ void r3d_graph_normalize_kernel(const int* __restrict__ row_ptr, const hg_col_t* __restrict__ col,
                                            const float* __restrict__ dinv, const int* __restrict__ n_dev,
-                                           int n_cap, float* __restrict__ val, HgEp st) {
-  const int ep = blockIdx.y;
+                                           int n_cap, float* __restrict__ val, HgEp st, HgGrid gr) {
+  HG_SYSBLK(gr);
   HG_WS(row_ptr); HG_WS(col); HG_WS(dinv); HG_AT(n_dev, st.desc); HG_WS(val);
   const int n = min(*n_dev, n_cap);
-  const int i = blockIdx.x * 4 + (threadIdx.x >> 6);
+  const int i = blk * 4 + (threadIdx.x >> 6);
   const int lane = threadIdx.x & 63;
   if (i >= n) return;
   const float di = dinv[i];
@@ -307,12 +332,11 @@
 #define HG_SEED_PITCH 257
 __global__ __launch_bounds__(256) void r3d_cg_aggregate_kernel(const float* __restrict__ nodes, long ldn, int D,
                                                                const int* __restrict__ n_dev, const int* __restrict__ n_proto_dev,
-                                                               int n_cap, int rows_per_wave, int* __restrict__ agg, HgEp st) {
+                                                               int n_cap, int rows_per_wave, int* __restrict__ agg, HgEp st,
+                                                               HgGrid gr) {
   extern __shared__ float smem[];
-  {
-    const int ep = blockIdx.y;
-    nodes += (long)ep * st.nodes * ldn; HG_AT(n_dev, st.desc); HG_AT(n_proto_dev, st.desc); HG_WS(agg);
-  }
+  HG_SYSBLK(gr);
+  nodes += (long)ep * st.nodes * ldn; HG_AT(n_dev, st.desc); HG_AT(n_proto_dev, st.desc); HG_WS(agg);
   const int pitch = D | 1;
   float* seeds = smem;
   float* xrow = smem + HG_M * pitch + (threadIdx.x >> 6) * D;
@@ -338,7 +362,7 @@
       }
     }
   }
-  const int row0 = (blockIdx.x * 4 + w) * rows_per_wave;
+  const int row0 = (blk * 4 + w) * rows_per_wave;
   float xr[4][4];
 #pragma unroll
   for (int k = 0; k < 4; ++k)
@@ -378,15 +402,14 @@
 __global__ __launch_bounds__(256) void r3d_cg_mw_kernel(const int* __restrict__ row_ptr, const hg_col_t* __restrict__ col,
                                                         const float* __restrict__ val, const float* __restrict__ dinv,
                                                         const int* __restrict__ agg, const int* __restrict__ n_dev, int n_cap,
-                                                        float alpha_lp, int rows_per_wave, float* __restrict__ MW, HgEp st) {
+                                                        float alpha_lp, int rows_per_wave, float* __restrict__ MW, HgEp st,
+                                                        HgGrid gr) {
   __shared__ float2 pairs[4][256];
-  {
-    const int ep = blockIdx.y;
-    HG_WS(row_ptr); HG_WS(col); HG_WS(val); HG_WS(dinv); HG_WS(agg); HG_AT(n_dev, st.desc); HG_WS(MW);
-  }
+  HG_SYSBLK(gr);
+  HG_WS(row_ptr); HG_WS(col); HG_WS(val); HG_WS(dinv); HG_WS(agg); HG_AT(n_dev, st.desc); HG_WS(MW);
   const int n = min(*n_dev, n_cap);
   const int lane = threadIdx.x & 63, w = threadIdx.x >> 6;
-  const int row0 = (blockIdx.x * 4 + w) * rows_per_wave;
+  const int row0 = (blk * 4 + w) * rows_per_wave;
   for (int k = 0; k < rows_per_wave; ++k) {
     const int i = row0 + k;
     if (i >= n_cap) break;
@@ -1180,9 +1203,9 @@
     float* base = scratch + (long)e * per;
     int32_t* wse = ws + (long)e * ws_stride;
     const LpWs Le = lp_carve(wse, n_cap, kp1);
-    hipLaunchKernelGGL(r3d_graph_weights_kernel, dim3(n_cap, 1), dim3(256), 0, st, nodes + (long)e * n_cap * ldn, ldn, D, Le.outb,
+    hipLaunchKernelGGL(r3d_graph_weights_kernel, dim3(n_cap), dim3(256), 0, st, nodes + (long)e * n_cap * ldn, ldn, D, Le.outb,
                        (int)Le.words, n_dev + (long)e * desc_stride, n_cap, Le.row_ptr, Le.col, sigma, base + 2 * nnz_cap,
-                       base + 3 * nnz_cap, base, one);
+                       base + 3 * nnz_cap, base, one, HgGrid{n_cap, 1, 0});
   }
   HgEp ep{};
   ep.desc = desc_stride; ep.ws = ws_stride;
@@ -1207,10 +1230,11 @@
     hipFuncSetAttribute((const void*)r3d_cg_aggregate_kernel, hipFuncAttributeMaxDynamicSharedMemorySize, 96 * 1024);
     lds_opt_in = true;
   }
-  hipLaunchKernelGGL(r3d_cg_aggregate_kernel, dim3(r3d_cdiv(n_cap, 4 * agg_rpw), n_ep), dim3(256), agg_lds, st, nodes, ldn, D,
-                     n_dev, n_proto_dev, n_cap, agg_rpw, L.agg, ep);
-  hipLaunchKernelGGL(r3d_cg_mw_kernel, dim3(r3d_cdiv(n_cap, 4), n_ep), dim3(256), 0, st, L.row_ptr, L.col, L.val, L.dinv, L.agg,
-                     n_dev, n_cap, alpha, 1, L.MW, ep);
+  const HgGrid ga = hg_grid(r3d_cdiv(n_cap, 4 * agg_rpw), n_ep), g4 = hg_grid(r3d_cdiv(n_cap, 4), n_ep);
+  hipLaunchKernelGGL(r3d_cg_aggregate_kernel, hg_dim(ga), dim3(256), agg_lds, st, nodes, ldn, D, n_dev, n_proto_dev, n_cap,
+                     agg_rpw, L.agg, ep, ga);
+  hipLaunchKernelGGL(r3d_cg_mw_kernel, hg_dim(g4), dim3(256), 0, st, L.row_ptr, L.col, L.val, L.dinv, L.agg, n_dev, n_cap, alpha,
+                     1, L.MW, ep, g4);
   hipLaunchKernelGGL(r3d_cg_epart_kernel, dim3(HG_EBLOCKS, n_ep), dim3(128), 0, st, L.MW, L.dinv, L.agg, n_dev, n_cap, L.Epart,
                      ep);
   hipLaunchKernelGGL(r3d_cg_einv_kernel, dim3(n_ep), dim3(1024), 0, st, L.Epart, L.Einv, ep);
@@ -1290,12 +1314,13 @@
   hipLaunchKernelGGL(r3d_graph_rowlen_kernel, dim3(r3d_cdiv(n_cap, 4), n_ep), dim3(256), 0, st, L.sym, L.outb, (int)words,
                      n_dev, n_cap, L.row_len, ep);
   hipLaunchKernelGGL(r3d_scan_kernel, dim3(n_ep), dim3(1024), 0, st, L.row_len, n_cap, L.row_ptr, ep);
-  hipLaunchKernelGGL(r3d_graph_cols_kernel, dim3(r3d_cdiv(n_cap, 4), n_ep), dim3(256), 0, st, L.sym, (int)words, n_dev,
-                     n_cap, L.row_ptr, L.col, ep);
-  hipLaunchKernelGGL(r3d_graph_weights_kernel, dim3(n_cap, n_ep), dim3(256), 0, st, nodes, ldn, D, L.outb,
-                     (int)words, n_dev, n_cap, L.row_ptr, L.col, sigma, L.val, L.dinv, L.wdir, ep);
-  hipLaunchKernelGGL(r3d_graph_normalize_kernel, dim3(r3d_cdiv(n_cap, 4), n_ep), dim3(256), 0, st, L.row_ptr, L.col, L.dinv,
-                     n_dev, n_cap, L.val, ep);
+  const HgGrid g1 = hg_grid(n_cap, n_ep), g4 = hg_grid(r3d_cdiv(n_cap, 4), n_ep);
+  hipLaunchKernelGGL(r3d_graph_cols_kernel, hg_dim(g4), dim3(256), 0, st, L.sym, (int)words, n_dev, n_cap, L.row_ptr, L.col, ep,
+                     g4);
+  hipLaunchKernelGGL(r3d_graph_weights_kernel, hg_dim(g1), dim3(256), 0, st, nodes, ldn, D, L.outb,
+                     (int)words, n_dev, n_cap, L.row_ptr, L.col, sigma, L.val, L.dinv, L.wdir, ep, g1);
+  hipLaunchKernelGGL(r3d_graph_normalize_kernel, hg_dim(g4), dim3(256), 0, st, L.row_ptr, L.col, L.dinv, n_dev, n_cap, L.val,
+                     ep, g4);
   int rc = lp_coarse_space(L, nodes, ldn, D, n_dev, n_proto_dev, n_cap, alpha, n_ep, ep, st);
   if (rc) return rc;
   rc = lp_solve(L, Y, ep.y, n_dev, n_cap, alpha, max_iter, tol, Z, ep.z, stats_out, n_ep, ep, st);
@@ -1351,11 +1376,11 @@
                                                             const float* __restrict__ val, const float* __restrict__ dinv,
                                                             const int* __restrict__ n_dev, int n_cap, float alpha,
                                                             const float4* __restrict__ lam, const float4* __restrict__ Z,
-                                                            float* __restrict__ dD, HgEp st) {
-  const int ep = blockIdx.y;
+                                                            float* __restrict__ dD, HgEp st, HgGrid gr) {
+  HG_SYSBLK(gr);
   HG_WS(row_ptr); HG_WS(col); HG_WS(val); HG_WS(dinv); HG_AT(n_dev, st.desc); HG_AT(lam, st.lam); HG_AT(Z, st.z); HG_WS(dD);
   const int n = min(*n_dev, n_cap);
-  const int i = blockIdx.x * 4 + (threadIdx.x >> 6);
+  const int i = blk * 4 + (threadIdx.x >> 6);
   const int lane = threadIdx.x & 63;
   if (i >= n) return;
   const float4 li = lam[i], zi = Z[i];
@@ -1374,17 +1399,15 @@
     const float* __restrict__ nodes, long ldn, int D, const float* __restrict__ wdir,
     const int* __restrict__ row_ptr, const hg_col_t* __restrict__ col, const float* __restrict__ dinv,
     const int* __restrict__ n_dev, int n_cap, float sigma, float alpha, const float4* __restrict__ lam,
-    const float4* __restrict__ Z, const float* __restrict__ dD, float* __restrict__ dnodes, long ldd, HgEp st) {
-  {
-    const int ep = blockIdx.y;
-    nodes += (long)ep * st.nodes * ldn; HG_WS(wdir); HG_WS(row_ptr); HG_WS(col); HG_WS(dinv); HG_AT(n_dev, st.desc);
-    HG_AT(lam, st.lam); HG_AT(Z, st.z); HG_WS(dD); dnodes += (long)ep * st.dn * ldd;
-  }
+    const float4* __restrict__ Z, const float* __restrict__ dD, float* __restrict__ dnodes, long ldd, HgEp st, HgGrid gr) {
+  HG_SYSBLK(gr);
+  nodes += (long)ep * st.nodes * ldn; HG_WS(wdir); HG_WS(row_ptr); HG_WS(col); HG_WS(dinv); HG_AT(n_dev, st.desc);
+  HG_AT(lam, st.lam); HG_AT(Z, st.z); HG_WS(dD); dnodes += (long)ep * st.dn * ldd;
   __shared__ float acc_s[4][256];
   __shared__ float uv_s[4][2];
   const int n = min(*n_dev, n_cap);
   const int w = threadIdx.x >> 6;
-  const int i = blockIdx.x;
+  const int i = blk;
   const int lane = threadIdx.x & 63;
   if (i >= n) return;
   const float* xi = nodes + (long)i * ldn;
@@ -1494,11 +1517,12 @@
   int rc = lp_solve(L, G, ep.g, n_dev, n_cap, alpha, max_iter, tol, lam, ep.lam, stats_out, n_ep, ep, st);
   if (rc) return rc;
   float* dD = (float*)L.q;
-  hipLaunchKernelGGL(r3d_lp_bwd_dd_kernel, dim3(r3d_cdiv(n_cap, 4), n_ep), dim3(256), 0, st, L.row_ptr, L.col, L.val, L.dinv, n_dev,
-                     n_cap, alpha, (const float4*)lam, (const float4*)Z, dD, ep);
-  hipLaunchKernelGGL(r3d_lp_bwd_dx_kernel, dim3(n_cap, n_ep), dim3(256), 0, st, nodes, ldn, D, L.wdir,
+  const HgGrid g1 = hg_grid(n_cap, n_ep), g4 = hg_grid(r3d_cdiv(n_cap, 4), n_ep);
+  hipLaunchKernelGGL(r3d_lp_bwd_dd_kernel, hg_dim(g4), dim3(256), 0, st, L.row_ptr, L.col, L.val, L.dinv, n_dev, n_cap, alpha,
+                     (const float4*)lam, (const float4*)Z, dD, ep, g4);
+  hipLaunchKernelGGL(r3d_lp_bwd_dx_kernel, hg_dim(g1), dim3(256), 0, st, nodes, ldn, D, L.wdir,
                      L.row_ptr, L.col, L.dinv, n_dev, n_cap, sigma, alpha, (const float4*)lam, (const float4*)Z, dD, dnodes,
-                     ldd, ep);
+                     ldd, ep, g1);
   R3D_LAUNCH_CHECK("r3d_label_propagate_bwd");
   return R3D_OK;
 }
diff --git a/r3dfsseg_amd/train_ops.py b/r3dfsseg_amd/train_ops.py
--- a/r3dfsseg_amd/train_ops.py
+++ b/r3dfsseg_amd/train_ops.py
@@ -57,8 +57,18 @@
         return False
 
 
+poison_unfilled = None
+
+
+def _unfilled(*shape, dev):
+    t = torch.empty(*shape, device=dev, dtype=torch.float32)
+    if poison_unfilled is not None:
+        t.fill_(poison_unfilled)
+    return t
+
+
 def _f(n, dev):
-    return torch.empty(n, device=dev, dtype=torch.float32)
+    return _unfilled(n, dev=dev)
 
 
 class BNVec:
@@ -151,7 +161,9 @@
     return out
 
 
-def conv_acc(X, W, out):
+def conv_acc(X, W, out, first=False):
+    if first:
+        return ops.pointwise_conv(X, W, out=out)
     M, ldx = _rows(X)
     with _timed("pointwise_conv"):
         _lib.check(_lib.load().r3d_pointwise_conv_acc(_p(X), ldx, _p(W), M, X.shape[1], W.shape[0], None, None, 0, _p(out),
@@ -188,7 +200,7 @@
     return y, (X, W2d, z, bn, act, seg)
 
 
-def conv_bn_bwd(saved, dY, want_dx=True, dx_acc=None):
+def conv_bn_bwd(saved, dY, want_dx=True, dx_acc=None, dx_first=False):
     X, W2d, z, bn, act, seg = saved
     C = W2d.shape[0]
     M = z.shape[0]
@@ -201,13 +213,13 @@
     if want_dx:
         Wt = W2d.t().contiguous()
         if dx_acc is not None:
-            conv_acc(dz, Wt, dx_acc)
+            conv_acc(dz, Wt, dx_acc, first=dx_first)
         else:
             dX = ops.pointwise_conv(dz, Wt)
     return dW, tot[1], tot[0], dbias, dX
 
 
-def edgeconv_train_fwd(inp, idx, ec, B, N, out, seg=None):
+def edgeconv_train_fwd(inp, idx, ec, B, N, out, seg=None, out2=None):
     lib = _lib.load()
     dev = inp.device
     seg = SegLayout(1, B, 0, N) if seg is None else seg
@@ -239,8 +251,9 @@
     bn2 = bn_fold(sums2, counts, ec.layer[4])
     sc2, sh2, _, _ = bn2.ptrs()
     with _timed("edgeconv"):
-        _lib.check(lib.r3d_edge_select(_p(zmax), _p(zmin), _p(argmax), _p(argmin), sc2, sh2, bn2.stride, M, seg.rows_a,
-                                       seg.rows_b, _p(out), out.stride(0), _st()))
+        _lib.check(lib.r3d_edge_select2(_p(zmax), _p(zmin), _p(argmax), _p(argmin), sc2, sh2, bn2.stride, M, seg.rows_a,
+                                        seg.rows_b, _p(out), out.stride(0), _p(out2), out2.stride(0) if out2 is not None else 0,
+                                        _st()))
     return (inp, idx3, Wpq, PQ, W2, bn1, bn2, argmax, zmax, C, seg, esum)
 
 
@@ -289,13 +302,14 @@
         assert seg.B == B and seg.N == N
         x_pm, x_cm = ops.input_layouts(x)
         cat = torch.empty(M, 64 * enc.n_edgeconv, device=dev, dtype=torch.float32)
+        feat = torch.empty(M, model.feat_dim, device=dev, dtype=torch.float32)
         inp, ec_saved = x_pm, []
         for l in range(enc.n_edgeconv):
             idx = ops.knn(inp, B, N, enc.k, x_cm=x_cm if l == 0 else None)
             if enc.idx_patch is not None:
                 idx = enc.idx_patch(l, idx.view(B, N, enc.k)).view(idx.shape)
             out = cat[:, 64 * l:64 * (l + 1)]
-            ec_saved.append(edgeconv_train_fwd(inp, idx, enc.edge_convs[l], B, N, out, seg))
+            ec_saved.append(edgeconv_train_fwd(inp, idx, enc.edge_convs[l], B, N, out, seg, out2=feat[:, :64] if l == 0 else None))
             inp = out
         h, mlp_saved = cat, []
         for jn in range(len(enc.conv.layer_dims)):
@@ -303,9 +317,7 @@
             h, sv = conv_bn_fwd(h, W.reshape(W.shape[0], -1).contiguous(), enc.conv.layer[3 * jn + 1], ops.ACT_LRELU, seg=seg)
             mlp_saved.append(sv)
         level2 = h
-        feat = torch.empty(M, model.feat_dim, device=dev, dtype=torch.float32)
         od = att.out_channel
-        ops.copy_cols(cat[:, :64], feat[:, :64])
         hb, base_saved = level2, []
         for i, seq in enumerate(base.convs):
             last = i == base.num_convs - 1
@@ -348,12 +360,12 @@
             def __setitem__(self, k, v):
                 dict.__setitem__(self, id(k), v)
         g = _G()
-        dlevel2 = torch.zeros(M, level2.shape[1], device=dev, dtype=torch.float32)
+        dlevel2 = _unfilled(M, level2.shape[1], dev=dev)
         od = att.out_channel
         d = dfeat[:, 64 + od:]
         for i in reversed(range(base.num_convs)):
             seq = base.convs[i]
-            dW, dg, db, dbias, dX = conv_bn_bwd(base_saved[i], d, want_dx=True, dx_acc=dlevel2 if i == 0 else None)
+            dW, dg, db, dbias, dX = conv_bn_bwd(base_saved[i], d, want_dx=True, dx_acc=dlevel2 if i == 0 else None, dx_first=True)
             g[seq[0].weight] = dW.view_as(seq[0].weight)
             g[seq[0].bias] = dbias
             g[seq[1].weight], g[seq[1].bias] = dg, db
@@ -369,15 +381,15 @@
             g[m.weight] = dWqkv[od * k:od * (k + 1)].reshape(m.weight.shape)
         Wraw = torch.cat([m.weight.reshape(od, -1) for m in (att.q_map, att.k_map, att.v_map)], 0)
         conv_acc(dqkv, Wraw.t().contiguous(), dlevel2)
-        dcat = torch.zeros(M, cat.shape[1], device=dev, dtype=torch.float32)
-        add_cols(dfeat[:, :64], dcat[:, :64])
+        dcat = _unfilled(M, cat.shape[1], dev=dev)
         d = dlevel2
         for jn in reversed(range(len(mlp_saved))):
             conv, bnm = enc.conv.layer[3 * jn], enc.conv.layer[3 * jn + 1]
-            dW, dg, db, _, dX = conv_bn_bwd(mlp_saved[jn], d, want_dx=True, dx_acc=dcat if jn == 0 else None)
+            dW, dg, db, _, dX = conv_bn_bwd(mlp_saved[jn], d, want_dx=True, dx_acc=dcat if jn == 0 else None, dx_first=True)
             g[conv.weight] = dW.view_as(conv.weight)
             g[bnm.weight], g[bnm.bias] = dg, db
             d = dX
+        add_cols(dfeat[:, :64], dcat[:, :64])
         for l in reversed(range(enc.n_edgeconv)):
             ec = enc.edge_convs[l]
             dx_acc = dcat[:, 64 * (l - 1):64 * l] if l > 0 else None
```
